# arielmission-space/PAOS

Hardware: AMD Instinct MI355X
Metric: wavefronts/sec (4096^2 c128, 20-surface chain) + achieved HBM GB/s (higher is better)
Workload: dtype c128 (f64); 1 GPU; SYN20 20-surface chain (SURVEY 8d: 43 2-D FFTs per wavefront as the reference runs it), 4096x4096 fp64, walked 512-wavelength sweep, 32 wavefronts/GPU/step, PSFs stay in HBM; separable pass programs + ptp identities ([24] passes/wavefront, parity 1e-15..2e-14 vs oracle); grid=4096, batch_per_gpu=32, parallelism=wavefront-sharded x1, transport=none (single process), ranks_seen=1, launcher=none

## Files before the change

include/paos_hip.h:

```cpp
#ifndef PAOS_HIP_H
#define PAOS_HIP_H

#ifdef __cplusplus
extern "C" {
#endif

typedef struct paos_ctx paos_ctx;

enum { PAOS_OK = 0, PAOS_EINVAL = 1, PAOS_EHIP = 2, PAOS_EUNSUPPORTED = 3 };
enum { PAOS_F64 = 0, PAOS_F32 = 1 };
enum { PAOS_SHAPE_ELLIPSE = 0, PAOS_SHAPE_RECT = 1 };
enum { PAOS_KERNEL_PASS_ROWS = 0, PAOS_KERNEL_PASS_COLS = 1, PAOS_KERNEL_PASS_ANY = 2 };
enum { PAOS_PW_SIGN = 1, PAOS_PW_QPHASE_CENTRED = 2, PAOS_PW_QPHASE_NATURAL = 3, PAOS_PW_SCALE = 4,
       PAOS_PW_MASK = 5 };
enum { PAOS_PWF_MUL2PI = 1,
       PAOS_PWF_X_ONLY = 2, PAOS_PWF_Y_ONLY = 4 };
enum { PAOS_MAX_PW = 6 };
enum { PAOS_NORM_SLOTS = 64 };
enum { PAOS_WHAT_FIELD = 0, PAOS_WHAT_AMPLITUDE = 1, PAOS_WHAT_PHASE = 2, PAOS_WHAT_INTENSITY = 3 };

enum { PAOS_PHASE_STRIDE = 5 };
enum { PAOS_APERTURE_STRIDE = 8 };
enum { PAOS_ZERNIKE_HEAD = 8 };

typedef struct { int kind, flags, block; } paos_pw_op;
typedef struct {
  int axis;
  int fft1, fft2;
  int n_pre, n_mid, n_post;
  paos_pw_op pre[PAOS_MAX_PW], mid[PAOS_MAX_PW], post[PAOS_MAX_PW];
} paos_pass;

typedef struct {
  const double* live_rows;
  int rows_stale;
  int final_intensity;
  int* power_ticket;
  const double* live_cols;
} paos_program_opts;

int paos_ctx_create(int device, int n, int batch, int precision, paos_ctx** out);
int paos_ctx_destroy(paos_ctx* ctx);
const char* paos_last_error(const paos_ctx* ctx);
int paos_sync(paos_ctx* ctx);
const char* paos_build_info(void);
const char* paos_source_hash(void);
void* paos_stream(paos_ctx* ctx);

int paos_profile_begin(paos_ctx* ctx, int kernel_kind, int max_launches);
int paos_profile_end(paos_ctx* ctx, int* launches, double* total_ms);
int paos_profile_end_split(paos_ctx* ctx, int* launches, double* total_ms, int* pruned_launches, double* pruned_ms);
int paos_profile_end_launches(paos_ctx* ctx, int capacity, double* ms_out, int* tag_out, int* count);
int paos_profile_planned_bytes(paos_ctx* ctx, int capacity, double* bytes_out, int* count);
int paos_profile_line_transforms(paos_ctx* ctx, int capacity, double* lines_out, int* count);

int paos_fill(paos_ctx* ctx, double re, double im);
int paos_start(paos_ctx* ctx, double re, double im, int shape, const double* aperture, const double* stop);
int paos_start_rows(paos_ctx* ctx, double re, double im, int shape, const double* aperture, const double* stop,
                    const double* write_rows);
int paos_zero_outside_rows(paos_ctx* ctx, const double* live_rows);
int paos_start_box(paos_ctx* ctx, double re, double im, int shape, const double* aperture, const double* stop,
                   const double* write_rows, const double* write_cols);
int paos_start_zernike_box(paos_ctx* ctx, double re, double im, int shape, const double* aperture, const double* stop,
                           const double* write_rows, const double* write_cols, int nmax, int kdim, const double* table,
                           const double* params, int param_stride, int* power_ticket);
int paos_zero_outside_box(paos_ctx* ctx, const double* live_rows, const double* live_cols);
int paos_import(paos_ctx* ctx, int item, const void* host_c128);
int paos_export(paos_ctx* ctx, int item, int what, void* host_out);

int paos_psf_keep(paos_ctx* ctx);
int paos_psf_keep_power(paos_ctx* ctx, int* ticket);
int paos_psf_fetch(paos_ctx* ctx, int item, double* host_out);
int paos_host_alloc(unsigned long long bytes, void** out);
int paos_host_free(void* p);
int paos_export_pinned(paos_ctx* ctx, int item, int what, void* pinned_out);

int paos_aperture(paos_ctx* ctx, int shape, const double* params);
int paos_aperture_render(paos_ctx* ctx, int shape, const double* params1, double* host_mask);
int paos_make_stop(paos_ctx* ctx, const double* enable);
int paos_stop_scale_last_power(paos_ctx* ctx, const double* enable);
int paos_stop_defer_last_power(paos_ctx* ctx, const double* enable);
int paos_norm2(paos_ctx* ctx, double* host_out);
int paos_norm2_enqueue(paos_ctx* ctx, int* ticket);
int paos_norm2_enqueue_rows(paos_ctx* ctx, const double* live_rows, int* ticket);
int paos_norm2_enqueue_rows_like(paos_ctx* ctx, const double* live_rows, const double* same_as, int* ticket);
int paos_norm2_enqueue_box(paos_ctx* ctx, const double* live_rows, const double* live_cols, const double* same_as, int* ticket);
int paos_norm2_fetch(paos_ctx* ctx, int ticket, double* host_out);
int paos_norm2_release(paos_ctx* ctx, int ticket);
int paos_psf_metrics(paos_ctx* ctx, int nr, const double* radii_px, double cx_px, double cy_px,
                     double* host_out);
int paos_phase(paos_ctx* ctx, const double* params, int mul2pi);
int paos_phase_map(paos_ctx* ctx, int item, const double* host_wfe, double wl);
int paos_phase_map_items(paos_ctx* ctx, const double* host_wfe, unsigned long long key, int n_items, const double* items,
                         const double* wl);
int paos_psd_screen(paos_ctx* ctx, const double* host_noise, const double* host_rough, const double* params,
                    unsigned long long key, double* host_out);
int paos_ptp(paos_ctx* ctx, const double* params);
int paos_stw(paos_ctx* ctx, const double* params, int inverse);
int paos_wts(paos_ctx* ctx, const double* params, int inverse);
int paos_focus_begin(paos_ctx* ctx);
int paos_focus_plane(paos_ctx* ctx, const double* params);
int paos_focus_end(paos_ctx* ctx);
enum { PAOS_OTF_MTF = 0, PAOS_OTF_COMPLEX = 1 };
int paos_otf_compute(paos_ctx* ctx);
int paos_otf_fetch(paos_ctx* ctx, int item, int what, void* host_out);
int paos_otf_cuts(paos_ctx* ctx, double* host_out);
int paos_blur_table(int n, double d, double sigma, double pixel, double* t);
enum { PAOS_BLUR_ITEM = 6 };
int paos_blur_apply(paos_ctx* ctx, const double* per_item);
enum { PAOS_EE_GIVEN = 0, PAOS_EE_CENTROID = 1, PAOS_EE_PEAK = 2 };
enum { PAOS_EE_ITEM = 4 };
enum { PAOS_EE_SUMMARY = 9 };
int paos_ee_compute(paos_ctx* ctx, int bins, int square, int centre_mode, const double* per_item);
int paos_ee_fetch(paos_ctx* ctx, double* summary, double* curves);
int paos_zoom_weights(int n, int s, double frac, double* w, int* carry);
enum { PAOS_ZOOM_PSF = 0, PAOS_ZOOM_FIELD = 1 };
int paos_zoom_compute(paos_ctx* ctx, int m, int s, const double* centres, int want_field);
int paos_zoom_tiles(int n, int batch, int m, int* pt_y, int* pt_x);
int paos_zoom_fetch(paos_ctx* ctx, int item, int what, void* host_out);
int paos_run_passes(paos_ctx* ctx, const paos_pass* passes, int n_passes, const double* blocks,
                    int n_blocks);
int paos_copy_yardstick(paos_ctx* ctx, int reps, double* ms_per_launch, double* bytes_per_launch);
int paos_record_set_stats(paos_ctx* ctx, unsigned long long* found, unsigned long long* rendered);
int paos_central_half_stats(paos_ctx* ctx, unsigned long long* central, unsigned long long* plain);
int paos_frugal_built(int precision, int n, const int* record);
int paos_pass_builds(paos_ctx* ctx, int* records, int capacity, int* count);
int paos_deferred_stop_stats(paos_ctx* ctx, unsigned long long* rode, unsigned long long* settled);
int paos_ctx_set_pruning(paos_ctx* ctx, int on);
int paos_run_passes_live(paos_ctx* ctx, const paos_pass* passes, int n_passes, const double* blocks,
                         int n_blocks, const double* live_rows);
int paos_run_program(paos_ctx* ctx, const paos_pass* passes, int n_passes, const double* blocks, int n_blocks,
                     const paos_program_opts* opts);
int paos_zernike(paos_ctx* ctx, int nmax, int kdim, const double* table, const double* params,
                 int param_stride, double* host_wfe);
int paos_zernike_like(paos_ctx* ctx, int nmax, int kdim, const double* table, const double* params,
                      int param_stride, const double* same_as, double* host_wfe);


int paos_pupil_aperture(paos_ctx* ctx, int shape, const double* params);
int paos_pupil_upload(paos_ctx* ctx, int item, const double* host_weights);
int paos_zernike_gram(paos_ctx* ctx, int nmax, int kdim, const double* table, const double* params,
                      int param_stride, int K, const double* poly, int use_pupil, double* host_out);
int paos_zernike_pupil(paos_ctx* ctx, int nmax, int kdim, const double* table, const double* params,
                       int param_stride, double* host_wfe);

enum { PAOS_WF_UNIFORM = 0, PAOS_WF_INTENSITY = 1 };
enum { PAOS_WF_SUMMARY = 10 };
int paos_wavefront_fit(paos_ctx* ctx, int nmax, int kdim, const double* table, const double* params, int param_stride,
                       int K, const double* poly, int weight_mode, int use_pupil, const double* min_intensity);
int paos_wavefront_fetch(paos_ctx* ctx, double* summary, double* sums);

enum { PAOS_DETECTOR_GEOM = 6 };
enum { PAOS_DETECTOR_ITEM = 3 };
enum { PAOS_DETECTOR_SCRATCH_MIB = 512 };
int paos_detector_begin(paos_ctx* ctx, const double* geom);
int paos_detector_add(paos_ctx* ctx, const double* per_item);
int paos_detector_images(paos_ctx* ctx, const double* per_item, double* host_out);
int paos_detector_fetch(paos_ctx* ctx, double* host_out);
enum { PAOS_DETECTOR_PLACED_ITEM = 5 };
int paos_detector_add_placed(paos_ctx* ctx, const double* per_item);
int paos_detector_images_placed(paos_ctx* ctx, const double* per_item, double* host_out);

#ifdef __cplusplus
}
#endif
#endif
```

paos_amd/_lib.py:

```python
import ctypes
import os
import threading
import weakref

import numpy as np

_HERE = os.path.dirname(os.path.abspath(__file__))
LIB_PATH = os.environ.get("PAOS_LIB") or os.path.join(_HERE, "libpaoship.so")

PAOS_F64, PAOS_F32 = 0, 1
SHAPE_ELLIPSE, SHAPE_RECT = 0, 1
WHAT_FIELD, WHAT_AMPLITUDE, WHAT_PHASE, WHAT_INTENSITY = 0, 1, 2, 3
KERNEL_PASS_ROWS, KERNEL_PASS_COLS, KERNEL_PASS_ANY = 0, 1, 2
PW_SIGN, PW_QPHASE_CENTRED, PW_QPHASE_NATURAL, PW_SCALE, PW_MASK = 1, 2, 3, 4, 5
PWF_MUL2PI = 1
PWF_X_ONLY, PWF_Y_ONLY = 2, 4
MAX_PW = 6
OTF_MTF, OTF_COMPLEX = 0, 1
EE_GIVEN, EE_CENTROID, EE_PEAK = 0, 1, 2
EE_ITEM, EE_SUMMARY, EE_MAX_BINS = 4, 9, 1024
WF_UNIFORM, WF_INTENSITY = 0, 1
WF_SUMMARY, WF_MAX_TERMS = 10, 63
ZOOM_PSF, ZOOM_FIELD = 0, 1
ZOOM_MAX_TABLES = 256
NORM_SLOTS = 64


class PwOp(ctypes.Structure):
    _fields_ = [("kind", ctypes.c_int), ("flags", ctypes.c_int), ("block", ctypes.c_int)]


class ProgramOpts(ctypes.Structure):
    _fields_ = [("live_rows", ctypes.POINTER(ctypes.c_double)), ("rows_stale", ctypes.c_int),
                ("final_intensity", ctypes.c_int), ("power_ticket", ctypes.POINTER(ctypes.c_int)),
                ("live_cols", ctypes.POINTER(ctypes.c_double))]


class Pass(ctypes.Structure):
    _fields_ = [("axis", ctypes.c_int), ("fft1", ctypes.c_int), ("fft2", ctypes.c_int),
                ("n_pre", ctypes.c_int), ("n_mid", ctypes.c_int), ("n_post", ctypes.c_int),
                ("pre", PwOp * MAX_PW), ("mid", PwOp * MAX_PW), ("post", PwOp * MAX_PW)]

PHASE_STRIDE = 5
APERTURE_STRIDE = 8
ZERNIKE_HEAD = 8

_c_ctx = ctypes.c_void_p
_dbl_p = ctypes.POINTER(ctypes.c_double)
SYMBOLS = {
    "paos_ctx_create": (ctypes.c_int, [ctypes.c_int, ctypes.c_int, ctypes.c_int, ctypes.c_int, ctypes.POINTER(_c_ctx)]),
    "paos_ctx_destroy": (ctypes.c_int, [_c_ctx]),
    "paos_last_error": (ctypes.c_char_p, [_c_ctx]),
    "paos_sync": (ctypes.c_int, [_c_ctx]),
    "paos_build_info": (ctypes.c_char_p, []),
    "paos_stream": (ctypes.c_void_p, [_c_ctx]),
    "paos_profile_begin": (ctypes.c_int, [_c_ctx, ctypes.c_int, ctypes.c_int]),
    "paos_profile_end": (ctypes.c_int, [_c_ctx, ctypes.POINTER(ctypes.c_int), _dbl_p]),
    "paos_profile_end_split": (ctypes.c_int, [_c_ctx, ctypes.POINTER(ctypes.c_int), _dbl_p, ctypes.POINTER(ctypes.c_int), _dbl_p]),
    "paos_source_hash": (ctypes.c_char_p, []),
    "paos_profile_planned_bytes": (ctypes.c_int, [_c_ctx, ctypes.c_int, _dbl_p, ctypes.POINTER(ctypes.c_int)]),
    "paos_profile_line_transforms": (ctypes.c_int, [_c_ctx, ctypes.c_int, _dbl_p, ctypes.POINTER(ctypes.c_int)]),
    "paos_profile_end_launches": (ctypes.c_int, [_c_ctx, ctypes.c_int, _dbl_p, ctypes.POINTER(ctypes.c_int),
                                                 ctypes.POINTER(ctypes.c_int)]),
    "paos_fill": (ctypes.c_int, [_c_ctx, ctypes.c_double, ctypes.c_double]),
    "paos_import": (ctypes.c_int, [_c_ctx, ctypes.c_int, ctypes.c_void_p]),
    "paos_export": (ctypes.c_int, [_c_ctx, ctypes.c_int, ctypes.c_int, ctypes.c_void_p]),
    "paos_aperture": (ctypes.c_int, [_c_ctx, ctypes.c_int, _dbl_p]),
    "paos_aperture_render": (ctypes.c_int, [_c_ctx, ctypes.c_int, _dbl_p, _dbl_p]),
    "paos_make_stop": (ctypes.c_int, [_c_ctx, _dbl_p]),
    "paos_stop_scale_last_power": (ctypes.c_int, [_c_ctx, _dbl_p]),
    "paos_stop_defer_last_power": (ctypes.c_int, [_c_ctx, _dbl_p]),
    "paos_norm2": (ctypes.c_int, [_c_ctx, _dbl_p]),
    "paos_norm2_enqueue": (ctypes.c_int, [_c_ctx, ctypes.POINTER(ctypes.c_int)]),
    "paos_norm2_fetch": (ctypes.c_int, [_c_ctx, ctypes.c_int, _dbl_p]),
    "paos_norm2_release": (ctypes.c_int, [_c_ctx, ctypes.c_int]),
    "paos_psf_metrics": (ctypes.c_int, [_c_ctx, ctypes.c_int, _dbl_p, ctypes.c_double, ctypes.c_double, _dbl_p]),
    "paos_phase": (ctypes.c_int, [_c_ctx, _dbl_p, ctypes.c_int]),
    "paos_phase_map": (ctypes.c_int, [_c_ctx, ctypes.c_int, _dbl_p, ctypes.c_double]),
    "paos_ptp": (ctypes.c_int, [_c_ctx, _dbl_p]),
    "paos_stw": (ctypes.c_int, [_c_ctx, _dbl_p, ctypes.c_int]),
    "paos_wts": (ctypes.c_int, [_c_ctx, _dbl_p, ctypes.c_int]),
    "paos_focus_begin": (ctypes.c_int, [_c_ctx]),
    "paos_focus_plane": (ctypes.c_int, [_c_ctx, _dbl_p]),
    "paos_focus_end": (ctypes.c_int, [_c_ctx]),
    "paos_otf_compute": (ctypes.c_int, [_c_ctx]),
    "paos_otf_fetch": (ctypes.c_int, [_c_ctx, ctypes.c_int, ctypes.c_int, ctypes.c_void_p]),
    "paos_otf_cuts": (ctypes.c_int, [_c_ctx, _dbl_p]),
    "paos_blur_table": (ctypes.c_int, [ctypes.c_int, ctypes.c_double, ctypes.c_double, ctypes.c_double, _dbl_p]),
    "paos_blur_apply": (ctypes.c_int, [_c_ctx, _dbl_p]),
    "paos_ee_compute": (ctypes.c_int, [_c_ctx, ctypes.c_int, ctypes.c_int, ctypes.c_int, _dbl_p]),
    "paos_ee_fetch": (ctypes.c_int, [_c_ctx, _dbl_p, _dbl_p]),
    "paos_wavefront_fit": (ctypes.c_int, [_c_ctx, ctypes.c_int, ctypes.c_int, _dbl_p, _dbl_p, ctypes.c_int, ctypes.c_int, _dbl_p,
                                          ctypes.c_int, ctypes.c_int, _dbl_p]),
    "paos_wavefront_fetch": (ctypes.c_int, [_c_ctx, _dbl_p, _dbl_p]),
    "paos_zoom_weights": (ctypes.c_int, [ctypes.c_int, ctypes.c_int, ctypes.c_double, _dbl_p, ctypes.POINTER(ctypes.c_int)]),
    "paos_zoom_compute": (ctypes.c_int, [_c_ctx, ctypes.c_int, ctypes.c_int, _dbl_p, ctypes.c_int]),
    "paos_zoom_fetch": (ctypes.c_int, [_c_ctx, ctypes.c_int, ctypes.c_int, ctypes.c_void_p]),
    "paos_zoom_tiles": (ctypes.c_int, [ctypes.c_int, ctypes.c_int, ctypes.c_int, ctypes.POINTER(ctypes.c_int),
                                       ctypes.POINTER(ctypes.c_int)]),
    "paos_run_passes": (ctypes.c_int, [_c_ctx, ctypes.POINTER(Pass), ctypes.c_int, _dbl_p, ctypes.c_int]),
    "paos_copy_yardstick": (ctypes.c_int, [_c_ctx, ctypes.c_int, _dbl_p, _dbl_p]),
    "paos_record_set_stats": (ctypes.c_int, [_c_ctx, ctypes.POINTER(ctypes.c_ulonglong), ctypes.POINTER(ctypes.c_ulonglong)]),
    "paos_central_half_stats": (ctypes.c_int, [_c_ctx, ctypes.POINTER(ctypes.c_ulonglong), ctypes.POINTER(ctypes.c_ulonglong)]),
    "paos_frugal_built": (ctypes.c_int, [ctypes.c_int, ctypes.c_int, ctypes.POINTER(ctypes.c_int)]),
    "paos_pass_builds": (ctypes.c_int, [_c_ctx, ctypes.POINTER(ctypes.c_int), ctypes.c_int, ctypes.POINTER(ctypes.c_int)]),
    "paos_deferred_stop_stats": (ctypes.c_int, [_c_ctx, ctypes.POINTER(ctypes.c_ulonglong), ctypes.POINTER(ctypes.c_ulonglong)]),
    "paos_ctx_set_pruning": (ctypes.c_int, [_c_ctx, ctypes.c_int]),
    "paos_run_passes_live": (ctypes.c_int, [_c_ctx, ctypes.POINTER(Pass), ctypes.c_int, _dbl_p, ctypes.c_int, _dbl_p]),
    "paos_zernike": (ctypes.c_int, [_c_ctx, ctypes.c_int, ctypes.c_int, _dbl_p, _dbl_p, ctypes.c_int, _dbl_p]),
    "paos_psf_keep": (ctypes.c_int, [_c_ctx]),
    "paos_psf_keep_power": (ctypes.c_int, [_c_ctx, ctypes.POINTER(ctypes.c_int)]),
    "paos_psf_fetch": (ctypes.c_int, [_c_ctx, ctypes.c_int, _dbl_p]),
    "paos_host_alloc": (ctypes.c_int, [ctypes.c_ulonglong, ctypes.POINTER(ctypes.c_void_p)]),
    "paos_host_free": (ctypes.c_int, [ctypes.c_void_p]),
    "paos_export_pinned": (ctypes.c_int, [_c_ctx, ctypes.c_int, ctypes.c_int, ctypes.c_void_p]),
    "paos_start": (ctypes.c_int, [_c_ctx, ctypes.c_double, ctypes.c_double, ctypes.c_int, _dbl_p, _dbl_p]),
    "paos_pupil_aperture": (ctypes.c_int, [_c_ctx, ctypes.c_int, _dbl_p]),
    "paos_pupil_upload": (ctypes.c_int, [_c_ctx, ctypes.c_int, _dbl_p]),
    "paos_zernike_like": (ctypes.c_int, [_c_ctx, ctypes.c_int, ctypes.c_int, _dbl_p, _dbl_p, ctypes.c_int, _dbl_p, _dbl_p]),
    "paos_zernike_gram": (ctypes.c_int, [_c_ctx, ctypes.c_int, ctypes.c_int, _dbl_p, _dbl_p, ctypes.c_int,
                                         ctypes.c_int, _dbl_p, ctypes.c_int, _dbl_p]),
    "paos_zernike_pupil": (ctypes.c_int, [_c_ctx, ctypes.c_int, ctypes.c_int, _dbl_p, _dbl_p, ctypes.c_int, _dbl_p]),
    "paos_start_rows": (ctypes.c_int, [_c_ctx, ctypes.c_double, ctypes.c_double, ctypes.c_int, _dbl_p, _dbl_p, _dbl_p]),
    "paos_zero_outside_rows": (ctypes.c_int, [_c_ctx, _dbl_p]),
    "paos_phase_map_items": (ctypes.c_int, [_c_ctx, _dbl_p, ctypes.c_ulonglong, ctypes.c_int, _dbl_p, _dbl_p]),
    "paos_psd_screen": (ctypes.c_int, [_c_ctx, _dbl_p, _dbl_p, _dbl_p, ctypes.c_ulonglong, _dbl_p]),
    "paos_start_box": (ctypes.c_int, [_c_ctx, ctypes.c_double, ctypes.c_double, ctypes.c_int, _dbl_p, _dbl_p, _dbl_p, _dbl_p]),
    "paos_start_zernike_box": (ctypes.c_int, [_c_ctx, ctypes.c_double, ctypes.c_double, ctypes.c_int, _dbl_p, _dbl_p, _dbl_p, _dbl_p,
                                              ctypes.c_int, ctypes.c_int, _dbl_p, _dbl_p, ctypes.c_int, ctypes.POINTER(ctypes.c_int)]),
    "paos_zero_outside_box": (ctypes.c_int, [_c_ctx, _dbl_p, _dbl_p]),
    "paos_norm2_enqueue_box": (ctypes.c_int, [_c_ctx, _dbl_p, _dbl_p, _dbl_p, ctypes.POINTER(ctypes.c_int)]),
    "paos_norm2_enqueue_rows": (ctypes.c_int, [_c_ctx, _dbl_p, ctypes.POINTER(ctypes.c_int)]),
    "paos_norm2_enqueue_rows_like": (ctypes.c_int, [_c_ctx, _dbl_p, _dbl_p, ctypes.POINTER(ctypes.c_int)]),
    "paos_run_program": (ctypes.c_int, [_c_ctx, ctypes.POINTER(Pass), ctypes.c_int, _dbl_p, ctypes.c_int,
                                        ctypes.POINTER(ProgramOpts)]),
    "paos_detector_begin": (ctypes.c_int, [_c_ctx, _dbl_p]),
    "paos_detector_add": (ctypes.c_int, [_c_ctx, _dbl_p]),
    "paos_detector_images": (ctypes.c_int, [_c_ctx, _dbl_p, _dbl_p]),
    "paos_detector_fetch": (ctypes.c_int, [_c_ctx, _dbl_p]),
    "paos_detector_add_placed": (ctypes.c_int, [_c_ctx, _dbl_p]),
    "paos_detector_images_placed": (ctypes.c_int, [_c_ctx, _dbl_p, _dbl_p]),
}

_lib = None


class PaosHipError(RuntimeError):
    pass


def load():
    global _lib
    if _lib is not None:
        return _lib
    if not os.path.exists(LIB_PATH):
        raise PaosHipError(
            f"{LIB_PATH} not found: build it with `make` or "
            "`python -c 'import __graft_entry__ as g; g.build()'` (there is no CPU fallback)"
        )
    lib = ctypes.CDLL(LIB_PATH)
    if os.environ.get("PAOS_LIB"):
        import sys

        print(f"paos_amd: using the library variant {LIB_PATH} (PAOS_LIB)", file=sys.stderr)
    for name, (res, args) in SYMBOLS.items():
        fn = getattr(lib, name)
        fn.restype = res
        fn.argtypes = args
    _lib = lib
    return lib


def _dptr(arr):
    return arr.ctypes.data_as(_dbl_p)


def as_blocks(blocks, batch, stride):
    arr = np.ascontiguousarray(blocks, dtype=np.float64)
    if arr.shape != (batch, stride):
        raise ValueError(f"expected parameter blocks of shape {(batch, stride)}, got {arr.shape}")
    return arr


BUILD_FIELDS = ("axis", "kpre", "kmid", "nfft", "store", "tab", "fuse", "one_line", "central")


def frugal_built(precision, n, record):
    if len(record) != len(BUILD_FIELDS):
        raise ValueError("a build record has nine fields")
    rec = (ctypes.c_int * 9)(*[int(v) for v in record])
    code = {"fp64": PAOS_F64, "fp32": PAOS_F32}.get(precision, -1)
    rc = load().paos_frugal_built(code, int(n), rec)
    if rc < 0:
        raise ValueError(f"no family of pass-kernel builds for {precision} at n = {n}")
    return bool(rc)


def zoom_check(size, oversample, n):
    if isinstance(size, bool) or not isinstance(size, (int, np.integer)) or size < 16 or size > 1024 or size % 16:
        raise ValueError(f"a zoomed window's size must be an integer multiple of 16 in 16 .. 1024, got {size!r}")
    if isinstance(oversample, bool) or not isinstance(oversample, (int, np.integer)) or not 1 <= oversample <= 64:
        raise ValueError(f"a zoomed window's oversampling must be an integer in 1 .. 64, got {oversample!r}")
    if size > oversample * n:
        raise ValueError(f"a zoomed window of {size} samples at oversampling {oversample} is wider than the {n}-pixel grid")


def zoom_tiles(n, batch, size):
    pty, ptx = ctypes.c_int(0), ctypes.c_int(0)
    if load().paos_zoom_tiles(int(n), int(batch), int(size), ctypes.byref(pty), ctypes.byref(ptx)) != 0:
        raise ValueError(f"paos_zoom_tiles refused n={n!r}, batch={batch!r}, size={size!r}")
    return pty.value, ptx.value


def blur_table(n, d, sigma, pixel=0.0):
    if isinstance(n, bool) or not isinstance(n, (int, np.integer)) or n < 2:
        raise ValueError(f"paos_blur_table refused n={n!r}")
    out = np.empty(int(n) // 2 + 1, dtype=np.float64)
    if load().paos_blur_table(int(n), float(d), float(sigma), float(pixel), _dptr(out)) != 0:
        raise ValueError(f"paos_blur_table refused n={n!r}, d={d!r}, sigma={sigma!r}, pixel={pixel!r}")
    return out


def zoom_centres(centres, batch, n):
    try:
        ctr = np.ascontiguousarray(centres, dtype=np.float64)
    except (TypeError, ValueError):
        raise ValueError("zoomed-window centres must be a (batch, 2) array of pixel positions (x, y)") from None
    if ctr.shape != (batch, 2):
        raise ValueError(f"zoomed-window centres must have shape ({batch}, 2), got {ctr.shape}")
    if not np.all(np.isfinite(ctr)) or np.any(ctr < 0.0) or np.any(ctr >= n):
        raise ValueError(f"zoomed-window centres must be finite and lie in [0, {n})")
    if np.unique(ctr - np.floor(ctr)).size > ZOOM_MAX_TABLES:
        raise ValueError(f"the centres of one call may have at most {ZOOM_MAX_TABLES} distinct fractional parts")
    return ctr


PINNED_MIN_BYTES = 4 << 20
PINNED_MAX_BYTES = 32 << 20
PINNED_LIVE_BYTES = int(os.environ.get("PAOS_PINNED_BYTES", 8 << 30))
PINNED_POOL_BYTES = 2 << 30
_pin_lock = threading.Lock()
_pin_free = {}
_pin_live = 0
_pin_pooled = 0


def _pin_release(address, nbytes):
    global _pin_live, _pin_pooled
    with _pin_lock:
        _pin_live -= nbytes
        if _pin_pooled + nbytes <= PINNED_POOL_BYTES:
            _pin_free.setdefault(nbytes, []).append(address)
            _pin_pooled += nbytes
            return
    try:
        load().paos_host_free(ctypes.c_void_p(address))
    except Exception:
        pass


def pinned_empty(shape, dtype):
    global _pin_live, _pin_pooled
    nbytes = int(np.prod(shape)) * np.dtype(dtype).itemsize
    if nbytes <= PINNED_MIN_BYTES:
        return None
    address = None
    with _pin_lock:
        if _pin_live + nbytes > PINNED_LIVE_BYTES:
            return None
        stack = _pin_free.get(nbytes)
        if stack:
            address = stack.pop()
            _pin_pooled -= nbytes
        elif nbytes > PINNED_MAX_BYTES:
            return None
        _pin_live += nbytes
    if address is None:
        ptr = ctypes.c_void_p()
        if load().paos_host_alloc(nbytes, ctypes.byref(ptr)) != 0 or not ptr.value:
            with _pin_lock:
                _pin_live -= nbytes
            return None
        address = ptr.value
    buf = (ctypes.c_char * nbytes).from_address(address)
    weakref.finalize(buf, _pin_release, address, nbytes)
    return np.frombuffer(buf, dtype=dtype).reshape(shape)


def release_pinned_pool():
    global _pin_pooled
    with _pin_lock:
        items = [(a, n) for n, lst in _pin_free.items() for a in lst]
        _pin_free.clear()
        _pin_pooled = 0
    for address, _ in items:
        load().paos_host_free(ctypes.c_void_p(address))


_HIP_TOUCHED = [False]


def hip_initialised():
    return _HIP_TOUCHED[0]


class DeviceFields:

    def __init__(self, n, batch=1, precision="fp64", device=0):
        self._lib = load()
        _HIP_TOUCHED[0] = True
        self._ctx = _c_ctx()
        self.detector = None
        self.n, self.batch = int(n), int(batch)
        if precision not in ("fp64", "fp32"):
            raise ValueError("precision must be 'fp64' or 'fp32'")
        self.precision = precision
        rc = self._lib.paos_ctx_create(int(device), self.n, self.batch,
                                       PAOS_F64 if precision == "fp64" else PAOS_F32,
                                       ctypes.byref(self._ctx))
        if rc != 0:
            msg = self._lib.paos_last_error(None).decode()
            self._ctx = _c_ctx()
            raise PaosHipError(f"paos_ctx_create failed ({rc}): {msg}")

    def _check(self, rc, what):
        if rc != 0:
            raise PaosHipError(f"{what} failed ({rc}): {self._lib.paos_last_error(self._ctx).decode()}")

    def close(self):
        if getattr(self, "_ctx", None) and self._ctx.value:
            self._lib.paos_ctx_destroy(self._ctx)
            self._ctx = _c_ctx()

    def __del__(self):
        try:
            self.close()
        except Exception:
            pass

    def sync(self):
        self._check(self._lib.paos_sync(self._ctx), "paos_sync")

    @property
    def stream(self):
        return self._lib.paos_stream(self._ctx)

    def build_info(self):
        return self._lib.paos_build_info().decode()

    def profile_begin(self, kernel_kind, max_launches=4096):
        self._check(self._lib.paos_profile_begin(self._ctx, int(kernel_kind), int(max_launches)),
                    "paos_profile_begin")

    def profile_end(self):
        n, ms = ctypes.c_int(0), ctypes.c_double(0.0)
        self._check(self._lib.paos_profile_end(self._ctx, ctypes.byref(n), ctypes.byref(ms)),
                    "paos_profile_end")
        return n.value, ms.value

    def profile_end_split(self):
        n, ms, pn, pms = ctypes.c_int(0), ctypes.c_double(0.0), ctypes.c_int(0), ctypes.c_double(0.0)
        self._check(self._lib.paos_profile_end_split(self._ctx, ctypes.byref(n), ctypes.byref(ms), ctypes.byref(pn),
                                                     ctypes.byref(pms)), "paos_profile_end_split")
        return n.value, ms.value, pn.value, pms.value

    def profile_planned_bytes(self, capacity=1 << 16):
        out = np.empty(capacity, dtype=np.float64)
        n = ctypes.c_int(0)
        self._check(self._lib.paos_profile_planned_bytes(self._ctx, int(capacity), _dptr(out), ctypes.byref(n)),
                    "paos_profile_planned_bytes")
        return out[:n.value].copy()

    def profile_line_transforms(self, capacity=1 << 16):
        out = np.empty(capacity, dtype=np.float64)
        n = ctypes.c_int(0)
        self._check(self._lib.paos_profile_line_transforms(self._ctx, int(capacity), _dptr(out), ctypes.byref(n)),
                    "paos_profile_line_transforms")
        return out[:n.value].copy()

    def profile_end_launches(self, capacity=1 << 16):
        ms = np.empty(capacity, dtype=np.float64)
        tags = np.empty(capacity, dtype=np.int32)
        n = ctypes.c_int(0)
        self._check(self._lib.paos_profile_end_launches(self._ctx, int(capacity), _dptr(ms),
                                                        tags.ctypes.data_as(ctypes.POINTER(ctypes.c_int)), ctypes.byref(n)),
                    "paos_profile_end_launches")
        return ms[:n.value].copy(), tags[:n.value].copy()

    def fill(self, value=1.0 + 0.0j):
        value = complex(value)
        self._check(self._lib.paos_fill(self._ctx, value.real, value.imag), "paos_fill")

    def upload(self, item, field):
        arr = np.ascontiguousarray(field, dtype=np.complex128)
        if arr.shape != (self.n, self.n):
            raise ValueError(f"field must have shape {(self.n, self.n)}")
        self._check(self._lib.paos_import(self._ctx, int(item), arr.ctypes.data_as(ctypes.c_void_p)),
                    "paos_import")

    def download(self, item=0, what=WHAT_FIELD):
        dtype = np.complex128 if what == WHAT_FIELD else np.float64
        out = pinned_empty((self.n, self.n), dtype)
        if out is not None:
            self._check(self._lib.paos_export_pinned(self._ctx, int(item), int(what),
                                                     out.ctypes.data_as(ctypes.c_void_p)), "paos_export_pinned")
            return out
# ... 457 lines not shown
```

paos_amd/csrc/context.hip:

```cpp
#include "host.h"

#include <cmath>
#include <complex>
#include <cstdio>
#include <cstring>
#include <mutex>
#include <set>
#include <utility>

namespace {

thread_local std::string g_err;

}

int fail(paos_ctx* c, int code, const std::string& msg) {
  if (c) c->err = msg;
  g_err = msg;
  return code;
}

namespace {

bool dump_arena() {
  static const bool dump = env_is("PAOS_DUMP_PASSES", '1');
  return dump;
}

int arena_commit(paos_ctx* c) {
  Arena& a = c->arena;
  size_t first = 0, count = 0;
  if (!a.lay.take(&first, &count)) return PAOS_OK;
  const size_t at = (size_t)a.cur * a.lay.cap + first;
  HIPCHK(c, hipMemcpyAsync(a.dev + at, a.host + at, count * sizeof(double), hipMemcpyHostToDevice, c->stream));
  return PAOS_OK;
}

int arena_switch(paos_ctx* c) {
  Arena& a = c->arena;
  if (int rc = arena_commit(c)) return rc;
  if (a.left >= 0) {
    HIPCHK(c, hipEventRecord(a.fence[a.left], c->stream));
    a.fenced[a.left] = true;
  }
  a.left = a.cur;
  const int next = (a.cur + 1) % kArenaSlabs;
  if (a.used[next]) {
    if (a.fenced[next]) HIPCHK(c, hipEventSynchronize(a.fence[next]));
    else HIPCHK(c, hipStreamSynchronize(c->stream));
  }
  a.fenced[next] = false;
  a.used[next] = true;
  a.cur = next;
  a.lay.rewind();
  if (dump_arena()) std::fprintf(stderr, "arena switch to slab %d\n", next);
  return PAOS_OK;
}

}

int launch_failed(paos_ctx* c, const char* call, hipError_t e, const char* file, int line) {
  return fail(c, PAOS_EHIP, std::string(call) + ": " + hipGetErrorString(e) + " (" + file + ":" + std::to_string(line) + ")");
}

int arena_reserve(paos_ctx* c, size_t total) {
  Arena& a = c->arena;
  switch (a.lay.room(total)) {
    case ARENA_FITS: return PAOS_OK;
    case ARENA_SWITCH: return arena_switch(c);
    case ARENA_GROW: break;
  }
  if (int rc = arena_commit(c)) return rc;
  HIPCHK(c, hipStreamSynchronize(c->stream));
  const size_t cap = a.lay.grown(total);
  double *h = nullptr, *d = nullptr;
  HIPCHK(c, hipHostMalloc(&h, kArenaSlabs * cap * sizeof(double)));
  if (hipMalloc(&d, kArenaSlabs * cap * sizeof(double)) != hipSuccess) {
    (void)hipHostFree(h);
    return fail(c, PAOS_EHIP, "hipMalloc(arena growth)");
  }
  (void)hipHostFree(a.host);
  (void)hipFree(a.dev);
  if (dump_arena()) std::fprintf(stderr, "arena grow to %zu doubles per slab\n", cap);
  a.host = h; a.dev = d; a.lay.cap = cap; a.lay.rewind(); a.cur = 0; a.left = -1;
  for (int k = 0; k < kArenaSlabs; ++k) a.fenced[k] = a.used[k] = false;
  a.used[0] = true;
  return PAOS_OK;
}

int ArenaBatch::begin(size_t total) {
  if (st_.closed || st_.reserved) return fail(c_, PAOS_EINVAL, "a parameter batch is begun once, before its first block");
  const int rc = arena_reserve(c_, total);
  if (rc == PAOS_OK) st_.reserved = true;
  return rc;
}

int ArenaBatch::add(const double* src, size_t count, const double** dev) {
  Arena& a = c_->arena;
  if (!st_.may_add()) return fail(c_, PAOS_EINVAL, "parameter block added to a batch that has been committed");
  if (count > a.lay.cap) return fail(c_, PAOS_EINVAL, "parameter block larger than the arena");
  if (!a.lay.fits(count)) {
    if (!st_.may_switch()) return fail(c_, PAOS_EINVAL, "a parameter batch outgrew the room it reserved");
    if (int rc = arena_switch(c_)) return rc;
  }
  const size_t at = (size_t)a.cur * a.lay.cap + a.lay.place(count);
  std::memcpy(a.host + at, src, count * sizeof(double));
  *dev = a.dev + at;
  return PAOS_OK;
}

int ArenaBatch::commit() {
  st_.closed = true;
  return arena_commit(c_);
}

int arena_push(paos_ctx* c, const double* src, size_t count, const double** dev) {
  ArenaBatch one(c);
  if (int rc = one.add(src, count, dev)) return rc;
  return one.commit();
}

int arena_settled(paos_ctx* c, int rc) {
  if (!c) return rc;
  const bool pending = c->arena.lay.pending();
  c->arena.lay.drop();
  if (rc == PAOS_OK && pending)
    return fail(c, PAOS_EHIP, "parameter blocks were added but never copied to the device: the call's launches read stale parameters");
  return rc;
}

constexpr size_t kBounceBytes = size_t(4) << 20;
int copy_to_host(paos_ctx* c, void* host, const void* dev, size_t bytes) {
  if (bytes > kBounceBytes) {
    HIPCHK(c, hipMemcpyAsync(host, dev, bytes, hipMemcpyDeviceToHost, c->stream));
    HIPCHK(c, hipStreamSynchronize(c->stream));
    return PAOS_OK;
  }
  for (int i = 0; i < 2; ++i)
    if (!c->bounce[i]) {
      HIPCHK(c, hipHostMalloc(&c->bounce[i], kBounceBytes));
      HIPCHK(c, hipEventCreateWithFlags(&c->bounce_ev[i], hipEventDisableTiming));
    }
  const size_t chunks = (bytes + kBounceBytes - 1) / kBounceBytes;
  auto len = [&](size_t k) { return k + 1 < chunks ? kBounceBytes : bytes - k * kBounceBytes; };
  for (size_t k = 0; k <= chunks; ++k) {
    if (k < chunks) {
      HIPCHK(c, hipMemcpyAsync(c->bounce[k & 1], (const char*)dev + k * kBounceBytes, len(k), hipMemcpyDeviceToHost, c->stream));
      HIPCHK(c, hipEventRecord(c->bounce_ev[k & 1], c->stream));
    }
    if (k > 0) {
      HIPCHK(c, hipEventSynchronize(c->bounce_ev[(k - 1) & 1]));
      std::memcpy((char*)host + (k - 1) * kBounceBytes, c->bounce[(k - 1) & 1], len(k - 1));
    }
  }
  HIPCHK(c, hipStreamSynchronize(c->stream));
  return PAOS_OK;
}

bool timed_launch_begin(paos_ctx* c, int kind) {
  const bool timed = (c->prof_kind == kind || c->prof_kind == PAOS_KERNEL_PASS_ANY) && (c->prof_used + 2 <= c->prof_events.size());
  return timed && hipEventRecord(c->prof_events[c->prof_used], c->stream) == hipSuccess;
}
hipError_t timed_launch_end(paos_ctx* c, int tag) {
  const hipError_t e = hipEventRecord(c->prof_events[c->prof_used + 1], c->stream);
  if (e != hipSuccess) return e;
  c->prof_tags.resize(c->prof_used / 2, 0);
  c->prof_tags.push_back(tag);
  c->prof_bytes.resize(c->prof_tags.size() - 1, 0.0);
  c->prof_bytes.push_back(c->prof_next_bytes);
  c->prof_lines.resize(c->prof_tags.size() - 1, 0.0);
  c->prof_lines.push_back(c->prof_next_lines);
  c->prof_used += 2;
  return hipSuccess;
}

int next_norm_slot(paos_ctx* c) {
  for (int k = 0; k < kNormSlots; ++k) {
    const int slot = (c->norm_slot + k) % kNormSlots;
    if (!c->norm_busy[slot]) { c->norm_slot = slot; return slot; }
  }
  return c->norm_slot;
}

int opt_in_lds(paos_ctx* c, const void* kern, size_t lds) {
  static std::mutex mu;
  static std::set<std::pair<int, const void*>> configured;
  std::lock_guard<std::mutex> lock(mu);
  const std::pair<int, const void*> key(c->device, kern);
  if (configured.count(key)) return PAOS_OK;
  HIPCHK(c, hipFuncSetAttribute(kern, hipFuncAttributeMaxDynamicSharedMemorySize, (int)lds));
  configured.insert(key);
  return PAOS_OK;
}

int check_mask_overflow(paos_ctx* c) {
  if (!c->mask_overflow) return PAOS_OK;
  int n = 0;
  HIPCHK(c, hipMemcpy(&n, c->mask_overflow, sizeof(int), hipMemcpyDeviceToHost));
  if (n != 0) {
    (void)hipMemset(c->mask_overflow, 0, sizeof(int));
    for (auto& ms : c->mask_sets) ms.key.clear();
    return fail(c, PAOS_EUNSUPPORTED, "aperture line records overflowed (partial run longer than kMaskW): results are invalid");
  }
  return PAOS_OK;
}

int check_rows(paos_ctx* c, const double* rows) {
  for (int i = 0; i < c->batch; ++i)
    if (!(rows[2 * i] >= 0.0) || !(rows[2 * i + 1] <= (double)c->n) || !(rows[2 * i] <= rows[2 * i + 1]))
      return fail(c, PAOS_EINVAL, "row range must satisfy 0 <= lo <= hi <= n");
  return PAOS_OK;
}

std::vector<double> rounded_cols(const paos_ctx* c, const double* cols) {
  std::vector<double> out((size_t)2 * c->batch);
  for (int i = 0; i < c->batch; ++i) {
    int l = (int)cols[2 * i], h = (int)cols[2 * i + 1];
    l = l < 0 ? 0 : (l / c->br) * c->br;
    h = ((h + c->br - 1) / c->br) * c->br;
    if (h > c->n) h = c->n;
    out[2 * i] = l; out[2 * i + 1] = h;
  }
  return out;
}

namespace {

template <typename T>
std::vector<std::complex<T>> twiddles(int n) {
  std::vector<std::complex<T>> tw(n);
  const long double two_pi = 6.283185307179586476925286766559005768L;
  for (int m = 0; m < n; ++m) {
    const long double a = two_pi * (long double)m / (long double)n;
    tw[m] = std::complex<T>((T)cosl(a), (T)-sinl(a));
  }
  return tw;
}


int profile_end(paos_ctx* c, int* launches, double* total_ms, int* pruned_launches, double* pruned_ms) {
  if (c) (void)hipSetDevice(c->device);
  if (!c || !launches || !total_ms) return fail(c, PAOS_EINVAL, "null argument");
  HIPCHK(c, hipStreamSynchronize(c->stream));
  double sum = 0.0, psum = 0.0;
  int pcount = 0;
  for (size_t i = 0; i + 1 < c->prof_used; i += 2) {
    float ms = 0.f;
    HIPCHK(c, hipEventElapsedTime(&ms, c->prof_events[i], c->prof_events[i + 1]));
    sum += ms;
    if (i / 2 < c->prof_tags.size() && c->prof_tags[i / 2]) { psum += ms; ++pcount; }
  }
  *launches = (int)(c->prof_used / 2);
  *total_ms = sum;
  if (pruned_launches) *pruned_launches = pcount;
  if (pruned_ms) *pruned_ms = psum;
  c->prof_kind = -1;
  c->prof_used = 0;
  return PAOS_OK;
}

}

extern "C" {

const char* paos_last_error(const paos_ctx* ctx) { return ctx ? ctx->err.c_str() : g_err.c_str(); }

const char* paos_build_info(void) {
  static const std::string info = std::string("libpaoship gfx950 layout=") + std::to_string(BR) + "(c64 at N>=2048: " + std::to_string(PAOS_F32_BR) + ")x(" +
                                  std::to_string(Lay<double>::BC) + "|" + std::to_string(Lay<float>::BC) +
                                  ") pad_blocks=" + std::to_string(PAOS_PAD_BLOCKS);
  return info.c_str();
}

void* paos_stream(paos_ctx* ctx) { return ctx ? (void*)ctx->stream : nullptr; }

int paos_ctx_create(int device, int n, int batch, int precision, paos_ctx** out) {
  if (!out) return fail(nullptr, PAOS_EINVAL, "out is null");
  *out = nullptr;
  if (n < 64 || n > 4096 || (n & (n - 1))) return fail(nullptr, PAOS_EUNSUPPORTED, "grid size must be a power of two in 64..4096");
  if (batch < 1) return fail(nullptr, PAOS_EINVAL, "batch must be >= 1");
  if (precision != PAOS_F64 && precision != PAOS_F32) return fail(nullptr, PAOS_EINVAL, "precision must be PAOS_F64 or PAOS_F32");
  int ndev = 0;
  if (hipGetDeviceCount(&ndev) != hipSuccess || ndev == 0)
    return fail(nullptr, PAOS_EHIP, "no HIP device available: libpaoship has no CPU fallback");
  if (device < 0 || device >= ndev) return fail(nullptr, PAOS_EINVAL, "device index out of range");
  paos_ctx* c = new paos_ctx();
  c->device = device; c->n = n; c->batch = batch; c->precision = precision;
  const int bc = precision == PAOS_F64 ? Lay<double>::BC : Lay<float>::BC;
  c->br = (precision == PAOS_F32 && n >= 2048) ? PAOS_F32_BR : PAOS_BR;
  c->pitch = (unsigned)n * c->br + (unsigned)PAOS_PAD_BLOCKS * c->br * bc;
  c->item_stride = c->pitch * (unsigned)(n / c->br);
  const size_t eb = elem_bytes(c);
  auto bail = [&](hipError_t e, const char* what) {
    std::string msg = std::string(what) + ": " + hipGetErrorString(e);
    paos_ctx_destroy(c);
    return fail(nullptr, PAOS_EHIP, msg);
  };
  hipError_t e;
  if ((e = hipSetDevice(device)) != hipSuccess) return bail(e, "hipSetDevice");
  if ((e = hipStreamCreateWithFlags(&c->stream, hipStreamNonBlocking)) != hipSuccess) return bail(e, "hipStreamCreate");
  if (const char* pad = getenv("PAOS_LDS_PAD")) c->lds_pad = (size_t)std::max(0, std::atoi(pad));
  if (env_is("PAOS_CENTRAL_HALF", '0')) c->central_half = false;
  if (env_is("PAOS_CENTRAL_HALF", '1')) c->central_half = true;
  if ((e = hipMalloc(&c->dyn_scale, (size_t)batch * sizeof(double))) != hipSuccess) return bail(e, "hipMalloc(dyn_scale)");
  {
    std::vector<double> ones((size_t)batch, 1.0);
    if ((e = hipMemcpy(c->dyn_scale, ones.data(), ones.size() * sizeof(double), hipMemcpyHostToDevice)) != hipSuccess) return bail(e, "hipMemcpy(dyn_scale)");
  }
  if ((e = hipMalloc(&c->field, (size_t)c->item_stride * batch * eb)) != hipSuccess) return bail(e, "hipMalloc(field)");
  if ((e = hipMemsetAsync(c->field, 0, (size_t)c->item_stride * batch * eb, c->stream)) != hipSuccess) return bail(e, "hipMemset(field)");
  if ((e = hipMalloc(&c->tw, (size_t)n * eb)) != hipSuccess) return bail(e, "hipMalloc(tw)");
  if ((e = hipMalloc(&c->staging, (size_t)n * n * 16)) != hipSuccess) return bail(e, "hipMalloc(staging)");
  c->nparts = 1024;
  if ((e = hipMalloc(&c->partial, (size_t)batch * c->nparts * sizeof(double))) != hipSuccess) return bail(e, "hipMalloc(partial)");
  if ((e = hipMalloc(&c->norm2, (size_t)batch * sizeof(double))) != hipSuccess) return bail(e, "hipMalloc(norm2)");
  if ((e = hipHostMalloc(&c->norm2_host, (size_t)kNormSlots * batch * sizeof(double))) != hipSuccess) return bail(e, "hipHostMalloc(norm2)");
  c->arena.lay.cap = (size_t)1 << 18;
  if (c->arena.lay.cap < (size_t)batch * 2048) c->arena.lay.cap = (size_t)batch * 2048;
  if (const char* cap = getenv("PAOS_ARENA_DOUBLES")) c->arena.lay.cap = arena_rounded((size_t)std::max(1LL, std::atoll(cap)));
  if ((e = hipHostMalloc(&c->arena.host, kArenaSlabs * c->arena.lay.cap * sizeof(double))) != hipSuccess) return bail(e, "hipHostMalloc(arena)");
  if ((e = hipMalloc(&c->arena.dev, kArenaSlabs * c->arena.lay.cap * sizeof(double))) != hipSuccess) return bail(e, "hipMalloc(arena)");
  for (int k = 0; k < kArenaSlabs; ++k)
    if ((e = hipEventCreateWithFlags(&c->arena.fence[k], hipEventDisableTiming)) != hipSuccess) return bail(e, "hipEventCreate(arena fence)");
  c->arena.used[0] = true;
  e = dispatch_layout(c, [&](auto t, auto) {
    auto tw = twiddles<decltype(t)>(n);
    return hipMemcpy(c->tw, tw.data(), (size_t)n * eb, hipMemcpyHostToDevice);
  });
  if (e != hipSuccess) return bail(e, "hipMemcpy(tw)");
  *out = c;
  return PAOS_OK;
}

int paos_profile_begin(paos_ctx* c, int kernel_kind, int max_launches) {
  if (c) (void)hipSetDevice(c->device);
  if (!c || max_launches < 0) return fail(c, PAOS_EINVAL, "bad profile request");
  HIPCHK(c, hipStreamSynchronize(c->stream));
  while (c->prof_events.size() < (size_t)2 * max_launches) {
    hipEvent_t e;
    HIPCHK(c, hipEventCreate(&e));
    c->prof_events.push_back(e);
  }
  c->prof_kind = kernel_kind;
  c->prof_used = 0;
  c->prof_tags.clear();
  c->prof_bytes.clear();
  c->prof_lines.clear();
  return PAOS_OK;
}

int paos_profile_end_launches(paos_ctx* c, int capacity, double* ms_out, int* tag_out, int* count) {
  if (c) (void)hipSetDevice(c->device);
  if (!c || !ms_out || !tag_out || !count || capacity < 0) return fail(c, PAOS_EINVAL, "null argument");
  HIPCHK(c, hipStreamSynchronize(c->stream));
  const int n = (int)(c->prof_used / 2);
  if (n > capacity) return fail(c, PAOS_EINVAL, "more launches were timed than the caller's arrays hold");
  for (int i = 0; i < n; ++i) {
    float ms = 0.f;
    HIPCHK(c, hipEventElapsedTime(&ms, c->prof_events[2 * i], c->prof_events[2 * i + 1]));
    ms_out[i] = ms;
    tag_out[i] = (size_t)i < c->prof_tags.size() ? c->prof_tags[i] : 0;
  }
  *count = n;
  c->prof_kind = -1;
  c->prof_used = 0;
  return PAOS_OK;
}

int paos_profile_planned_bytes(paos_ctx* c, int capacity, double* bytes_out, int* count) {
  if (!c || !bytes_out || !count || capacity < 0) return fail(c, PAOS_EINVAL, "null argument");
  const int n = (int)(c->prof_used / 2);
  if (n > capacity) return fail(c, PAOS_EINVAL, "more launches were timed than the caller's array holds");
  for (int i = 0; i < n; ++i) bytes_out[i] = (size_t)i < c->prof_bytes.size() ? c->prof_bytes[i] : 0.0;
  *count = n;
  return PAOS_OK;
}

int paos_profile_line_transforms(paos_ctx* c, int capacity, double* lines_out, int* count) {
  if (!c || !lines_out || !count || capacity < 0) return fail(c, PAOS_EINVAL, "bad profile request");
  const int n = (int)(c->prof_used / 2);
  if (n > capacity) return fail(c, PAOS_EINVAL, "profile buffer too small");
  for (int i = 0; i < n; ++i) lines_out[i] = (size_t)i < c->prof_lines.size() ? c->prof_lines[i] : 0.0;
  *count = n;
  return PAOS_OK;
}

int paos_profile_end(paos_ctx* c, int* launches, double* total_ms) {
  return profile_end(c, launches, total_ms, nullptr, nullptr);
}

int paos_profile_end_split(paos_ctx* c, int* launches, double* total_ms, int* pruned_launches, double* pruned_ms) {
  if (!pruned_launches || !pruned_ms) return fail(c, PAOS_EINVAL, "null argument");
  return profile_end(c, launches, total_ms, pruned_launches, pruned_ms);
}

int paos_ctx_destroy(paos_ctx* c) {
  if (!c) return PAOS_OK;
  (void)hipSetDevice(c->device);
  if (c->stream) (void)hipStreamSynchronize(c->stream);
  for (hipEvent_t e : c->prof_events) (void)hipEventDestroy(e);
  if (c->field) (void)hipFree(c->field);
  if (c->tw) (void)hipFree(c->tw);
  if (c->staging) (void)hipFree(c->staging);
  if (c->tables) (void)hipFree(c->tables);
  if (c->mask) (void)hipFree(c->mask);
  if (c->metric_partial) (void)hipFree(c->metric_partial);
  if (c->metric_out) (void)hipFree(c->metric_out);
  if (c->metric_host) (void)hipHostFree(c->metric_host);
  for (auto& ms : c->mask_sets) {
    if (ms.lines) (void)hipFree(ms.lines);
    if (ms.vals) (void)hipFree(ms.vals);
  }
  if (c->mask_overflow) (void)hipFree(c->mask_overflow);
  if (c->partial) (void)hipFree(c->partial);
  if (c->norm2) (void)hipFree(c->norm2);
  if (c->norm2_host) (void)hipHostFree(c->norm2_host);
  if (c->psf) (void)hipFree(c->psf);
  if (c->focus_spec) (void)hipFree(c->focus_spec);
  if (c->otf_spec) (void)hipFree(c->otf_spec);
  if (c->otf_cuts) (void)hipFree(c->otf_cuts);
  if (c->zoom_t) (void)hipFree(c->zoom_t);
  if (c->zoom_psf) (void)hipFree(c->zoom_psf);
  if (c->zoom_field) (void)hipFree(c->zoom_field);
  if (c->zoom_tabs) (void)hipFree(c->zoom_tabs);
  if (c->map_dev) (void)hipFree(c->map_dev);
  if (c->psd_scratch) (void)hipFree(c->psd_scratch);
  if (c->start_norm2) (void)hipFree(c->start_norm2);
  if (c->start_partial) (void)hipFree(c->start_partial);
  if (c->psd_bad) (void)hipFree(c->psd_bad);
  if (c->pow_partial) (void)hipFree(c->pow_partial);
  if (c->dyn_scale) (void)hipFree(c->dyn_scale);
  if (c->ptab) (void)hipFree(c->ptab);
  if (c->psf_partial) (void)hipFree(c->psf_partial);
  if (c->det_img) (void)hipFree(c->det_img);
  if (c->det_rows) (void)hipFree(c->det_rows);
  if (c->det_out) (void)hipFree(c->det_out);
  if (c->ee_buf) (void)hipFree(c->ee_buf);
  if (c->wf_buf) (void)hipFree(c->wf_buf);
  for (int i = 0; i < 2; ++i) {
    if (c->bounce[i]) (void)hipHostFree(c->bounce[i]);
    if (c->bounce_ev[i]) (void)hipEventDestroy(c->bounce_ev[i]);
  }
  if (c->arena.host) (void)hipHostFree(c->arena.host);
  if (c->arena.dev) (void)hipFree(c->arena.dev);
  for (int k = 0; k < kArenaSlabs; ++k)
    if (c->arena.fence[k]) (void)hipEventDestroy(c->arena.fence[k]);
  if (c->stream) (void)hipStreamDestroy(c->stream);
  delete c;
  return PAOS_OK;
}

int paos_sync(paos_ctx* c) {
  if (c) (void)hipSetDevice(c->device);
  if (!c) return fail(c, PAOS_EINVAL, "null context");
  HIPCHK(c, hipStreamSynchronize(c->stream));
  return check_mask_overflow(c);
}

int paos_host_alloc(unsigned long long bytes, void** out) {
  if (!out || bytes == 0) return fail(nullptr, PAOS_EINVAL, "null argument");
  *out = nullptr;
  const hipError_t e = hipHostMalloc(out, (size_t)bytes);
  if (e != hipSuccess) {
    *out = nullptr;
    return fail(nullptr, PAOS_EHIP, std::string("hipHostMalloc: ") + hipGetErrorString(e));
  }
  return PAOS_OK;
}

int paos_host_free(void* p) {
  if (!p) return PAOS_OK;
  const hipError_t e = hipHostFree(p);
  if (e != hipSuccess) return fail(nullptr, PAOS_EHIP, std::string("hipHostFree: ") + hipGetErrorString(e));
  return PAOS_OK;
}

int paos_norm2_fetch(paos_ctx* c, int ticket, double* host_out) {
  if (c) (void)hipSetDevice(c->device);
  if (!c || !host_out || ticket < 0 || ticket >= kNormSlots) return fail(c, PAOS_EINVAL, "bad ticket");
  if (!c->norm_busy[ticket]) return fail(c, PAOS_EINVAL, "ticket is not outstanding (already fetched, or never issued)");
  HIPCHK(c, hipStreamSynchronize(c->stream));
  c->norm_busy[ticket] = false;
  std::memcpy(host_out, c->norm2_host + (size_t)ticket * c->batch, (size_t)c->batch * sizeof(double));
  return check_mask_overflow(c);
}

int paos_norm2_release(paos_ctx* c, int ticket) {
  if (!c || ticket < 0 || ticket >= kNormSlots) return fail(c, PAOS_EINVAL, "bad ticket");
  c->norm_busy[ticket] = false;
  return PAOS_OK;
}

int paos_record_set_stats(paos_ctx* c, unsigned long long* found, unsigned long long* rendered) {
  if (!c || !found || !rendered) return fail(c, PAOS_EINVAL, "bad record-set request");
  *found = c->mask_hits;
  *rendered = c->mask_rendered;
  return PAOS_OK;
}

int paos_central_half_stats(paos_ctx* c, unsigned long long* central, unsigned long long* plain) {
  if (!c || !central || !plain) return fail(c, PAOS_EINVAL, "bad central-half request");
  *central = c->central_launches;
  *plain = c->plain_launches;
  return PAOS_OK;
}

int paos_deferred_stop_stats(paos_ctx* c, unsigned long long* rode, unsigned long long* settled) {
  if (!c || !rode || !settled) return fail(c, PAOS_EINVAL, "bad deferred-stop request");
  *rode = c->deferred_rode;
  *settled = c->deferred_settled;
  return PAOS_OK;
}

int paos_ctx_set_pruning(paos_ctx* c, int on) {
  if (!c) return fail(c, PAOS_EINVAL, "null context");
  c->prune = on != 0;
  return PAOS_OK;
}

}
```

paos_amd/csrc/fft_core.h:

```cpp
#pragma once
#include <hip/hip_runtime.h>

namespace paos {

template <typename T>
struct cx {
  T x, y;
};

template <typename T>
__device__ __forceinline__ cx<T> cadd(cx<T> a, cx<T> b) { return {a.x + b.x, a.y + b.y}; }
template <typename T>
__device__ __forceinline__ cx<T> csub(cx<T> a, cx<T> b) { return {a.x - b.x, a.y - b.y}; }
template <typename T>
__device__ __forceinline__ cx<T> cmul(cx<T> a, cx<T> b) {
  return {fma(a.x, b.x, -(a.y * b.y)), fma(a.x, b.y, a.y * b.x)};
}
template <typename T>
__device__ __forceinline__ cx<T> cconj(cx<T> a) { return {a.x, -a.y}; }
template <typename T>
__device__ __forceinline__ cx<T> sub_ib(cx<T> a, cx<T> b) { return {a.x + b.y, a.y - b.x}; }
template <typename T>
__device__ __forceinline__ cx<T> add_ib(cx<T> a, cx<T> b) { return {a.x - b.y, a.y + b.x}; }
template <typename T>
__device__ __forceinline__ cx<T> fma_real(T c, cx<T> b, cx<T> a) { return {fma(c, b.x, a.x), fma(c, b.y, a.y)}; }
template <typename T>
__device__ __forceinline__ cx<T> rot_tau(cx<T> b, T tau) { return {fma(-tau, b.y, b.x), fma(tau, b.x, b.y)}; }
template <typename T>
__device__ __forceinline__ cx<T> fma_mic(T c, cx<T> b, cx<T> a) { return {fma(c, b.y, a.x), fma(-c, b.x, a.y)}; }
template <typename T>
__device__ __forceinline__ cx<T> fma_pic(T c, cx<T> b, cx<T> a) { return {fma(-c, b.y, a.x), fma(c, b.x, a.y)}; }
template <typename T>
__device__ __forceinline__ cx<T> cmul_const(cx<T> v, T c, T s) { return {fma(v.x, c, -(v.y * s)), fma(v.x, s, v.y * c)}; }
template <typename T>
__device__ __forceinline__ cx<T> scale2(cx<T> v, T p, T q) { return {v.x * p, v.y * q}; }

typedef float f2 __attribute__((ext_vector_type(2)));
__device__ __forceinline__ f2 pk(cx<float> a) { return f2{a.x, a.y}; }
__device__ __forceinline__ cx<float> unpk(f2 v) { return {v.x, v.y}; }
__device__ __forceinline__ cx<float> cadd(cx<float> a, cx<float> b) { return unpk(pk(a) + pk(b)); }
__device__ __forceinline__ cx<float> csub(cx<float> a, cx<float> b) { return unpk(pk(a) - pk(b)); }
__device__ __forceinline__ cx<float> cmul(cx<float> a, cx<float> b) {
  f2 t, r;
  const f2 av = pk(a), bv = pk(b);
  asm("v_pk_mul_f32 %0, %1, %2 op_sel_hi:[0,1]" : "=v"(t) : "v"(av), "v"(bv));
  asm("v_pk_fma_f32 %0, %1, %2, %3 op_sel:[1,1,0] op_sel_hi:[1,0,1] neg_lo:[1,0,0]"
      : "=v"(r) : "v"(av), "v"(bv), "v"(t));
  return unpk(r);
}
__device__ __forceinline__ cx<float> cmul_after_trans(cx<float> a, cx<float> b) {
  f2 t, r;
  const f2 av = pk(a), bv = pk(b);
  asm("s_nop 0\n\tv_pk_mul_f32 %0, %1, %2 op_sel_hi:[0,1]" : "=v"(t) : "v"(av), "v"(bv));
  asm("v_pk_fma_f32 %0, %1, %2, %3 op_sel:[1,1,0] op_sel_hi:[1,0,1] neg_lo:[1,0,0]" : "=v"(r) : "v"(av), "v"(bv), "v"(t));
  return unpk(r);
}
__device__ __forceinline__ cx<float> sub_ib(cx<float> a, cx<float> b) {
  f2 r;
  asm("v_pk_add_f32 %0, %1, %2 op_sel:[0,1] op_sel_hi:[1,0] neg_hi:[0,1]" : "=v"(r) : "v"(pk(a)), "v"(pk(b)));
  return unpk(r);
}
__device__ __forceinline__ cx<float> add_ib(cx<float> a, cx<float> b) {
  f2 r;
  asm("v_pk_add_f32 %0, %1, %2 op_sel:[0,1] op_sel_hi:[1,0] neg_lo:[0,1]" : "=v"(r) : "v"(pk(a)), "v"(pk(b)));
  return unpk(r);
}
__device__ __forceinline__ cx<float> fma_real(float c, cx<float> b, cx<float> a) {
  return unpk(__builtin_elementwise_fma(f2{c, c}, pk(b), pk(a)));
}
__device__ __forceinline__ cx<float> rot_tau(cx<float> b, float tau) {
  const f2 bv = pk(b);
  return unpk(__builtin_elementwise_fma(bv.yx, f2{-tau, tau}, bv));
}
__device__ __forceinline__ cx<float> fma_mic(float c, cx<float> b, cx<float> a) {
  return unpk(__builtin_elementwise_fma(pk(b).yx, f2{c, -c}, pk(a)));
}
__device__ __forceinline__ cx<float> fma_pic(float c, cx<float> b, cx<float> a) {
  return unpk(__builtin_elementwise_fma(pk(b).yx, f2{-c, c}, pk(a)));
}
__device__ __forceinline__ cx<float> cmul_const(cx<float> v, float c, float s) {
  const f2 vv = pk(v);
  return unpk(__builtin_elementwise_fma(vv.yy, f2{-s, c}, vv.xx * f2{c, s}));
}
__device__ __forceinline__ cx<float> scale2(cx<float> v, float p, float q) { return unpk(pk(v) * f2{p, q}); }

__device__ __forceinline__ void sincos_fast(double a, double* sn, double* cs) {
  const double kMagic = 6755399441055744.0;
  const double nb = fma(a, 0.63661977236758134308, kMagic);
  const unsigned q = (unsigned)__double2loint(nb);
  const double n = nb - kMagic;
  double r = fma(-n, 1.57079632673412561417e+00, a);
  r = fma(-n, 6.07710050630396597660e-11, r);
  r = fma(-n, 2.02226624879595063154e-21, r);
  const double z = r * r;
  double ps = fma(z, 1.58969099521155010221e-10, -2.50507602534068634195e-08);
  ps = fma(z, ps, 2.75573137070700676789e-06);
  ps = fma(z, ps, -1.98412698298579493134e-04);
  ps = fma(z, ps, 8.33333333332248946124e-03);
  ps = fma(z, ps, -1.66666666666666324348e-01);
  const double s = fma(r * z, ps, r);
  double pc = fma(z, -1.13596475577881948265e-11, 2.08757232129817482790e-09);
  pc = fma(z, pc, -2.75573143513906633035e-07);
  pc = fma(z, pc, 2.48015872894767294178e-05);
  pc = fma(z, pc, -1.38888888888741095749e-03);
  pc = fma(z, pc, 4.16666666666666019037e-02);
  const double c = fma(z * z, pc, fma(z, -0.5, 1.0));
  const bool odd = (q & 1u) != 0;
  const double s1 = odd ? c : s;
  const double c1 = odd ? s : c;
  const int sflip = (int)((q & 2u) << 30), cflip = (int)(((q + 1u) & 2u) << 30);
  *sn = __hiloint2double(__double2hiint(s1) ^ sflip, __double2loint(s1));
  *cs = __hiloint2double(__double2hiint(c1) ^ cflip, __double2loint(c1));
}

__device__ constexpr double kCos32[9] = {
    1.0,
    0.98078528040323044913,
    0.92387953251128675613,
    0.83146961230254523708,
    0.70710678118654752440,
    0.55557023301960222474,
    0.38268343236508977173,
    0.19509032201612826785,
    0.0};

__host__ __device__ constexpr double cos32(int m) {
  m &= 31;
  if (m > 16) m = 32 - m;
  return (m > 8) ? -kCos32[16 - m] : kCos32[m];
}
__host__ __device__ constexpr double sin32(int m) { return cos32(m - 8); }

template <int R, int DIR, typename T>
__device__ __forceinline__ cx<T> mulw(cx<T> v, int m) {
  const int m32 = (m * (32 / R)) & 31;
  if (m32 == 0) return v;
  if (m32 == 16) return {-v.x, -v.y};
  if (m32 == 8) return (DIR > 0) ? cx<T>{v.y, -v.x} : cx<T>{-v.y, v.x};
  if (m32 == 24) return (DIR > 0) ? cx<T>{-v.y, v.x} : cx<T>{v.y, -v.x};
  const T c = (T)cos32(m32);
  const T s = (T)((DIR > 0) ? -sin32(m32) : sin32(m32));
  return cmul_const(v, c, s);
}

template <int M16, int DIR>
struct W16 {
  static constexpr int m32 = (M16 * 2) & 31;
  static constexpr bool quarter = m32 == 8 || m32 == 24;
  static constexpr bool times_minus_i = (m32 == 8) == (DIR > 0);
  static constexpr double c = cos32(m32);
  static constexpr double s = (DIR > 0) ? -sin32(m32) : sin32(m32);
  static constexpr double tau = quarter ? 0.0 : s / c;
};
template <typename T>
__device__ __forceinline__ cx<T> lf_u(cx<T> b, double tau) { return rot_tau(b, (T)tau); }
template <int K1, int DIR, typename T>
__device__ __forceinline__ void lf_twiddled_dft4(const cx<T>* b, cx<T>* out) {
  using W1 = W16<K1, DIR>;
  using W2 = W16<2 * K1, DIR>;
  using W3 = W16<3 * K1, DIR>;
  static_assert(!W1::quarter && !W3::quarter, "K1 and 3 K1 are never multiples of 4 here");
  cx<T> t0, t1;
  if constexpr (W2::quarter) {
    const cx<T> wb = W2::times_minus_i ? cx<T>{b[2].y, -b[2].x} : cx<T>{-b[2].y, b[2].x};
    t0 = cadd(b[0], wb);
    t1 = csub(b[0], wb);
  } else {
    const cx<T> u2 = lf_u(b[2], W2::tau);
    t0 = fma_real((T)W2::c, u2, b[0]);
    t1 = fma_real((T)-W2::c, u2, b[0]);
  }
  const cx<T> u1 = lf_u(b[1], W1::tau), u3 = lf_u(b[3], W3::tau);
  constexpr double rho = W3::c / W1::c;
  const cx<T> t2 = fma_real((T)rho, u3, u1);
  const cx<T> t3 = fma_real((T)-rho, u3, u1);
  constexpr T c1 = (T)W1::c;
  out[0] = fma_real(c1, t2, t0);
  out[2] = fma_real(-c1, t2, t0);
  if constexpr (DIR > 0) {
    out[1] = fma_mic(c1, t3, t1);
    out[3] = fma_pic(c1, t3, t1);
  } else {
    out[1] = fma_pic(c1, t3, t1);
    out[3] = fma_mic(c1, t3, t1);
  }
}

template <int R, int DIR, typename T>
__device__ __forceinline__ void dft(cx<T>* v);

template <int DIR, typename T>
__device__ __forceinline__ void dft16_lf(cx<T>* v) {
  cx<T> y[16];
#pragma unroll
  for (int n2 = 0; n2 < 4; ++n2) {
    cx<T> a[4] = {v[n2], v[4 + n2], v[8 + n2], v[12 + n2]};
    dft<4, DIR>(a);
#pragma unroll
    for (int k1 = 0; k1 < 4; ++k1) y[k1 * 4 + n2] = a[k1];
  }
  cx<T> o[4];
  {
    cx<T> b[4] = {y[0], y[1], y[2], y[3]};
    dft<4, DIR>(b);
#pragma unroll
    for (int k2 = 0; k2 < 4; ++k2) v[4 * k2] = b[k2];
  }
  lf_twiddled_dft4<1, DIR>(y + 4, o);
#pragma unroll
  for (int k2 = 0; k2 < 4; ++k2) v[1 + 4 * k2] = o[k2];
  lf_twiddled_dft4<2, DIR>(y + 8, o);
#pragma unroll
  for (int k2 = 0; k2 < 4; ++k2) v[2 + 4 * k2] = o[k2];
  lf_twiddled_dft4<3, DIR>(y + 12, o);
#pragma unroll
  for (int k2 = 0; k2 < 4; ++k2) v[3 + 4 * k2] = o[k2];
}

template <int DIR, typename T>
__device__ __forceinline__ void dft16_lf_central(cx<T>* v) {
  static_assert(DIR > 0, "the pass kernel runs forward transforms only");
  cx<T> y[16];
#pragma unroll
  for (int n2 = 0; n2 < 4; ++n2) {
    const cx<T> a = v[4 + n2], b = v[8 + n2];
    const cx<T> nb = {-b.x, -b.y};
    y[0 * 4 + n2] = cadd(b, a);
    y[1 * 4 + n2] = sub_ib(nb, a);
    y[2 * 4 + n2] = csub(b, a);
    y[3 * 4 + n2] = add_ib(nb, a);
  }
  cx<T> o[4];
  {
    cx<T> b[4] = {y[0], y[1], y[2], y[3]};
    dft<4, DIR>(b);
#pragma unroll
    for (int k2 = 0; k2 < 4; ++k2) v[4 * k2] = b[k2];
  }
  lf_twiddled_dft4<1, DIR>(y + 4, o);
#pragma unroll
  for (int k2 = 0; k2 < 4; ++k2) v[1 + 4 * k2] = o[k2];
  lf_twiddled_dft4<2, DIR>(y + 8, o);
#pragma unroll
  for (int k2 = 0; k2 < 4; ++k2) v[2 + 4 * k2] = o[k2];
  lf_twiddled_dft4<3, DIR>(y + 12, o);
#pragma unroll
  for (int k2 = 0; k2 < 4; ++k2) v[3 + 4 * k2] = o[k2];
}

template <int R, int DIR, typename T>
__device__ __forceinline__ void dft(cx<T>* v) {
  if constexpr (R == 16) {
    dft16_lf<DIR>(v);
  } else if constexpr (R == 2) {
    cx<T> a = v[0], b = v[1];
    v[0] = cadd(a, b);
    v[1] = csub(a, b);
  } else if constexpr (R == 4) {
    cx<T> t0 = cadd(v[0], v[2]), t1 = csub(v[0], v[2]);
    cx<T> t2 = cadd(v[1], v[3]), t3 = csub(v[1], v[3]);
    v[0] = cadd(t0, t2);
    v[2] = csub(t0, t2);
    if constexpr (DIR > 0) {
      v[1] = sub_ib(t1, t3);
      v[3] = add_ib(t1, t3);
    } else {
      v[1] = add_ib(t1, t3);
      v[3] = sub_ib(t1, t3);
    }
  } else if constexpr (R > 4) {
    constexpr int A = 4, B = R / 4;
    cx<T> y[R];
#pragma unroll
    for (int n2 = 0; n2 < B; ++n2) {
      cx<T> a[A];
#pragma unroll
      for (int n1 = 0; n1 < A; ++n1) a[n1] = v[B * n1 + n2];
      dft<A, DIR>(a);
#pragma unroll
      for (int k1 = 0; k1 < A; ++k1) y[k1 * B + n2] = mulw<R, DIR>(a[k1], n2 * k1);
    }
#pragma unroll
    for (int k1 = 0; k1 < A; ++k1) {
      cx<T> b[B];
#pragma unroll
      for (int n2 = 0; n2 < B; ++n2) b[n2] = y[k1 * B + n2];
      dft<B, DIR>(b);
#pragma unroll
      for (int k2 = 0; k2 < B; ++k2) v[k1 + A * k2] = b[k2];
    }
  }
}

__device__ __forceinline__ constexpr int lds_pad(int i) { return i + (i >> 4); }
template <int N>
constexpr int lds_line_slots() { return N + (N >> 4); }

template <int N, int E, int NS>
struct StageInfo {
  static constexpr int REM = N / NS;
  static constexpr int R = (REM >= E) ? E : REM;
  static constexpr int TPT = E / R;
  static constexpr bool LAST = (NS * R == N);
};

template <int N, int E, int NS = 1>
constexpr int last_radix() {
  if constexpr (StageInfo<N, E, NS>::LAST) return StageInfo<N, E, NS>::R;
  else return last_radix<N, E, NS * StageInfo<N, E, NS>::R>();
}

template <int N, int E>
__device__ __forceinline__ constexpr int outslot(int k) {
  constexpr int RL = last_radix<N, E>();
  constexpr int TPTL = E / RL;
  return (k / RL) + (k % RL) * TPTL;
}

template <int R, typename T>
__device__ __forceinline__ void apply_twiddle_powers(cx<T>* v, cx<T> w1) {
  v[1] = cmul(v[1], w1);
  if constexpr (R > 2) {
    const cx<T> w2 = cmul(w1, w1);
    const cx<T> w3 = cmul(w2, w1);
    v[2] = cmul(v[2], w2);
    v[3] = cmul(v[3], w3);
    if constexpr (R > 4) {
      const cx<T> w4 = cmul(w2, w2);
      cx<T> base = w4;
#pragma unroll
      for (int a = 1; a < R / 4; ++a) {
        v[4 * a] = cmul(v[4 * a], base);
        v[4 * a + 1] = cmul(v[4 * a + 1], cmul(base, w1));
        v[4 * a + 2] = cmul(v[4 * a + 2], cmul(base, w2));
        v[4 * a + 3] = cmul(v[4 * a + 3], cmul(base, w3));
        if (a + 1 < R / 4) base = cmul(base, w4);
      }
    }
  }
}

template <int R, typename T>
__device__ __forceinline__ void apply_twiddle_chain(cx<T>* v, cx<T> w1) {
  cx<T> w = w1;
#pragma unroll
  for (int r = 1; r < R; ++r) {
    v[r] = cmul(v[r], w);
    if (r + 1 < R) w = cmul(w, w1);
  }
}

#define PAOS_FENCE() do { if constexpr (FR != 0) __builtin_amdgcn_sched_barrier(0); } while (0)
template <typename T, int N, int E, int DIR, bool SPLIT, int NS = 1, int FR = 0, int CH = 0>
__device__ __forceinline__ void fft_stages(cx<T>* v, void* lds, int t,
                                           const cx<T>* __restrict__ tw, const cx<double>* circle = nullptr,
                                           const cx<T>* w1_last = nullptr) {
  using S = StageInfo<N, E, NS>;
  constexpr int TL = N / E;
  constexpr int R = S::R;
  constexpr int TPT = S::TPT;

#pragma unroll
  for (int s = 0; s < TPT; ++s) {
    if constexpr (NS > 1) {
      const int j = t + s * TL;
      const int k = j & (NS - 1);
      if constexpr (FR != 0 && sizeof(T) == 8 && NS * R == 256) {
        cx<double> wa = circle[k], wb = circle[2 * k];
#pragma unroll
        for (int r = 1; r < R; ++r) {
          const cx<double> w = wa;
          wa = wb;
          if (r + 2 < R) wb = circle[k * (r + 2)];
          v[s * R + r] = cmul(v[s * R + r], cx<T>{(T)w.x, (T)(DIR > 0 ? -w.y : w.y)});
          PAOS_FENCE();
        }
      } else {
        cx<T> w1 = (w1_last != nullptr && NS * R == N) ? w1_last[s] : tw[k * (N / (NS * R))];
        if constexpr (DIR < 0) w1.y = -w1.y;
        if constexpr (FR != 0) apply_twiddle_chain<R>(v + s * R, w1);
        else apply_twiddle_powers<R>(v + s * R, w1);
      }
      PAOS_FENCE();
    }
    if constexpr (CH != 0 && NS == 1) {
      static_assert(R == 16 && TPT == 1, "central-half first stage: one 16-point butterfly per thread");
      dft16_lf_central<DIR>(v);
    } else {
      dft<R, DIR>(v + s * R);
    }
    PAOS_FENCE();
  }

  if constexpr (!S::LAST) {
    using SN = StageInfo<N, E, NS * R>;
    constexpr int R2 = SN::R;
    constexpr int TPT2 = SN::TPT;
    constexpr bool LIN_R = (TL % 16 == 0) && ((N / R2) % 16 == 0);
    int wb[TPT];
#pragma unroll
    for (int s = 0; s < TPT; ++s) {
      const int j = t + s * TL;
      wb[s] = lds_pad((j / NS) * (NS * R) + (j & (NS - 1)));
    }
    const int rb = lds_pad(t);
    auto ridx = [&](int s, int r) -> int {
      const int off = s * TL + r * (N / R2);
      return LIN_R ? rb + lds_pad(off) : lds_pad(t + off);
    };
    if constexpr (!SPLIT) {
      cx<T>* l = reinterpret_cast<cx<T>*>(lds);
#pragma unroll
      for (int s = 0; s < TPT; ++s)
#pragma unroll
        for (int r = 0; r < R; ++r) l[wb[s] + lds_pad(r * NS)] = v[s * R + r];
      __syncthreads();
#pragma unroll
      for (int s = 0; s < TPT2; ++s)
#pragma unroll
        for (int r = 0; r < R2; ++r) v[s * R2 + r] = l[ridx(s, r)];
      if constexpr (!SN::LAST) __syncthreads();
    } else {
      T* l = reinterpret_cast<T*>(lds);
#pragma unroll
      for (int part = 0; part < 2; ++part) {
#pragma unroll
        for (int s = 0; s < TPT; ++s)
#pragma unroll
          for (int r = 0; r < R; ++r) l[wb[s] + lds_pad(r * NS)] = part ? v[s * R + r].y : v[s * R + r].x;
        __syncthreads();
#pragma unroll
        for (int s = 0; s < TPT2; ++s)
#pragma unroll
          for (int r = 0; r < R2; ++r) {
            const T val = l[ridx(s, r)];
            if (part) v[s * R2 + r].y = val; else v[s * R2 + r].x = val;
          }
        if (part == 0 || !SN::LAST) __syncthreads();
      }
    }
    PAOS_FENCE();
    fft_stages<T, N, E, DIR, SPLIT, NS * R, FR, 0>(v, lds, t, tw, circle, w1_last);
  }
}

template <int N, int E, typename T>
__device__ __forceinline__ void unpermute_slots(cx<T>* v) {
  cx<T> tmp[E];
#pragma unroll
  for (int k = 0; k < E; ++k) tmp[outslot<N, E>(k)] = v[k];
#pragma unroll
  for (int k = 0; k < E; ++k) v[k] = tmp[k];
}

template <int BR, int BC>
__device__ __host__ __forceinline__ constexpr size_t layout_index(int row, int col, size_t pitch) {
  return (size_t)(row / BR) * pitch + (size_t)(col / BC) * (BR * BC) + (row % BR) * BC + (col % BC);
}

}
```

paos_amd/csrc/frugal_d1024.hip:

```cpp
#include "frugal_launch.h"

template <>
int frugal_family<double, 1024>(paos_ctx* c, const FrugalBuild& b, const FrugalArgs& a) { return frugal_dispatch<double, 1024>(c, b, a); }
```

paos_amd/csrc/frugal_d2048.hip:

```cpp
#include "frugal_launch.h"

template <>
int frugal_family<double, 2048>(paos_ctx* c, const FrugalBuild& b, const FrugalArgs& a) { return frugal_dispatch<double, 2048>(c, b, a); }
```

paos_amd/csrc/frugal_d4096.hip:

```cpp
#include "frugal_launch.h"

template <>
int frugal_family<double, 4096>(paos_ctx* c, const FrugalBuild& b, const FrugalArgs& a) { return frugal_dispatch<double, 4096>(c, b, a); }
```

paos_amd/csrc/frugal_f2048.hip:

```cpp
#include "frugal_launch.h"

template <>
int frugal_family<float, 2048>(paos_ctx* c, const FrugalBuild& b, const FrugalArgs& a) { return frugal_dispatch<float, 2048>(c, b, a); }
```

paos_amd/csrc/frugal_f4096.hip:

```cpp
#include "frugal_launch.h"

template <>
int frugal_family<float, 4096>(paos_ctx* c, const FrugalBuild& b, const FrugalArgs& a) { return frugal_dispatch<float, 4096>(c, b, a); }
```

paos_amd/csrc/frugal_launch.h:

```cpp
#pragma once
#include "host.h"
#include "pass_records.h"


inline int frugal_not_built(paos_ctx* c, const FrugalBuild& b) {
  if (b.tab && b.fuse) {
    if (b.kpre != 1 || b.kmid != 1) return fail(c, PAOS_EINVAL, "no fused build of this pass shape");
    if (b.nfft < 2) return fail(c, PAOS_EINVAL, "a fused chain starts with a two-transform pass");
    if (b.fuse > 4) return fail(c, PAOS_EINVAL, "a launch runs at most three passes");
  }
  if (b.tab && !(b.kpre <= 1 && b.kmid <= 1 && b.kpre + b.kmid > 0)) return fail(c, PAOS_EINVAL, "no table build of this pass shape");
  if (b.store == 1 && !b.tab) return fail(c, PAOS_EUNSUPPORTED, "no PSF-storing build of this pass shape");
  if (b.store == 2 && !b.tab) return fail(c, PAOS_EUNSUPPORTED, "no power-summing build of this pass shape");
  return fail(c, PAOS_EINVAL, "no build of this pass shape");
}

template <typename T, int N, int AXIS, int KPRE, int KMID, int STORE = 0, int LONG = 0, int ONE = 0, int LINES_ = 0, int TILES_ = 0>
struct FrugalGeometry {
  using C = FftCfg<T, N>;
  static constexpr bool kLatencyBound = PAOS_LONG_ONE_LINE != 0 && (LONG != 0 || ONE != 0) && STORE == 0 && sizeof(T) == 8;
  static constexpr bool kOneLine = kLatencyBound && N == 4096;
  static constexpr int OCC = (kLatencyBound && N == 2048) ? 1 : 0;
  static constexpr int LINES = LINES_ != 0 ? LINES_ : (kOneLine ? 1 : (AXIS == 0 ? C::FR_ROW_LINES : C::COL_LINES));
  static constexpr int TILES = TILES_ != 0 ? TILES_ : (AXIS == 0 ? C::ROW_TILES : C::COL_TILES);
  static constexpr bool SPLIT = sizeof(T) == 8 || LINES > 2;
  static constexpr int GROUPS = N / LINES / TILES, THREADS = TILES * LINES * N / C::E;
  static constexpr size_t LDS = frugal_lds_bytes<T, N, LINES, TILES, SPLIT, KPRE, KMID, C::E, STORE, OCC>();
  static constexpr unsigned ALIGN = (LINES == 1 && AXIS == 0) ? 32 : 16;
};

namespace {

template <typename T, int N, int AXIS, int KPRE, int KMID, int NFFT, int STORE, int TAB, int LONG, int ONE, int CH>
int frugal_launch(paos_ctx* c, const FrugalArgs& args) {
  using C = FftCfg<T, N>;
  using G = FrugalGeometry<T, N, AXIS, KPRE, KMID, STORE, LONG, ONE>;
  FrugalArgs a = args;
  unsigned groups = G::GROUPS;
  a.wg0 = 0;
  static_assert(G::GROUPS % G::ALIGN == 0, "TileMap renumbers tiles inside aligned groups of workgroups");
  if (a.live_hi > a.live_lo) {
    const unsigned per = G::LINES * G::TILES;
    a.wg0 = (a.live_lo / per) / G::ALIGN * G::ALIGN;
    unsigned end = ((a.live_hi + per - 1) / per + G::ALIGN - 1) / G::ALIGN * G::ALIGN;
    if (end > groups) end = groups;
    groups = end - a.wg0;
  }
  const dim3 grid(groups, c->batch), block(G::THREADS);
  constexpr size_t kMaxPad = 8192;
  const size_t lds = G::LDS + (c->lds_pad < kMaxPad ? c->lds_pad : kMaxPad);
  auto kern = frugal_pass_kernel<T, N, C::E, G::LINES, G::TILES, AXIS, C::BR, C::BC, G::SPLIT, KPRE, KMID, NFFT, STORE, TAB, LONG, G::OCC, CH>;
  ++(CH != 0 ? c->central_launches : c->plain_launches);
  return TIMED_LAUNCH(c, kern, grid, block, lds, G::LDS + kMaxPad, AXIS == 0 ? PAOS_KERNEL_PASS_ROWS : PAOS_KERNEL_PASS_COLS,
                      c->prof_next_tag, PAOS_FRUGAL_PASS(a));
}

constexpr int kFrugalFieldMax[] = {1, kFrugalMaxPre, kFrugalMaxMid, 2, 2, 1, 4, 1, 1};
template <typename T, int N, int X, int... V>
int frugal_unfold(paos_ctx* c, const FrugalBuild& b, const FrugalArgs& a) {
  constexpr int I = sizeof...(V), kFields = sizeof(kFrugalFieldMax) / sizeof(int);
  static_assert(kFields == kBuildFields, "one maximum per field");
  int field[kBuildFields];
  build_to_ints(b, field);
  if (field[I] != X) {
    if constexpr (X < kFrugalFieldMax[I]) return frugal_unfold<T, N, X + 1, V...>(c, b, a);
    else return frugal_not_built(c, b);
  } else if constexpr (I + 1 < kFields) {
    return frugal_unfold<T, N, 0, V..., X>(c, b, a);
  } else if constexpr (frugal_built<T, N>(FrugalBuild{V..., X})) {
    return frugal_launch<T, N, V..., X>(c, a);
  } else {
    return frugal_not_built(c, b);
  }
}
template <typename T, int N>
int frugal_dispatch(paos_ctx* c, const FrugalBuild& b, const FrugalArgs& a) {
  return frugal_unfold<T, N, 0>(c, b, a);
}

}
```

paos_amd/csrc/frugal_pass.h:

```cpp
#pragma once
#include "fft_kernels.h"
#include "pass_records.h"

#ifndef PAOS_FENCE_EVERY
#define PAOS_FENCE_EVERY 2
#endif

namespace paos {


template <int N, int E>
constexpr int twiddle_lds_entries() { return E <= 16 ? 256 : (N / 4 < 1024 ? N / 4 : 1024); }

#ifndef PAOS_STAMPS
#define PAOS_STAMPS 0
#endif
constexpr int kStampSlots = 12;

struct FrugalArgs {
  void* field;
  const void* tw;
  const FrugalItem* items;
  unsigned pitch, item_stride;
  double* psf;
  double* psf_partial;
  double* pow_partial;
  const double* dyn_scale;
#if PAOS_STAMPS
  unsigned long long* stamps;
#endif
  unsigned live_lo = 0, live_hi = 0, wg0 = 0;
};
#if PAOS_STAMPS
#define PAOS_STAMP(i)                                                                              \
  do {                                                                                             \
    if (threadIdx.x == 0)                                                                          \
      a.stamps[((size_t)blockIdx.y * gridDim.x + blockIdx.x) * kStampSlots + (i)] = __builtin_amdgcn_s_memtime(); \
  } while (0)
#define PAOS_STAMP_WAIT_VM() asm volatile("s_waitcnt vmcnt(0)" ::: "memory")
#else
#define PAOS_STAMP(i) do { } while (0)
#define PAOS_STAMP_WAIT_VM() do { } while (0)
#endif

constexpr int kCircleLds = 256;
template <bool TAIL = false>
__device__ __forceinline__ void sincos_tab(double a, const cx<double>* circle, double* sn, double* cs, double tail = 0.0) {
  const double kMagic = 6755399441055744.0;
  const double nb = fma(a, 40.743665431525205956834243423363677, kMagic);
  const unsigned j = (unsigned)__double2loint(nb) & (unsigned)(kCircleLds - 1);
  const double n = nb - kMagic;
  double r = fma(-n, 2.45436926061702596754894014318e-02, a);
  r = fma(-n, 9.56755311833869697380e-19, r);
  if constexpr (TAIL) r = __dadd_rn(r, tail);
  const cx<double> c = circle[j];
  const double z = r * r;
  const double ps = fma(z, 8.33333333333333333333e-03, -1.66666666666666666667e-01);
  const double s1 = fma(r * z, ps, r);
  double pc = fma(z, -1.38888888888888888889e-03, 4.16666666666666666667e-02);
  pc = fma(z, pc, -0.5);
  const double c1 = fma(z, pc, 1.0);
  *cs = fma(c.x, c1, -(c.y * s1));
  *sn = fma(c.y, c1, c.x * s1);
}

template <typename T>
__device__ __forceinline__ T flip_sign(T x, unsigned mask_hi) {
  if constexpr (sizeof(T) == 8)
    return __hiloint2double(__double2hiint(x) ^ (int)mask_hi, __double2loint(x));
  else
    return __uint_as_float(__float_as_uint(x) ^ mask_hi);
}

#ifndef PAOS_ROW_PRE
#define PAOS_ROW_PRE 2
#endif
#ifndef PAOS_COL_PRE
#define PAOS_COL_PRE 2
#endif
#ifndef PAOS_TABLE_FENCE
#define PAOS_TABLE_FENCE 8
#endif

__device__ __forceinline__ void lds_barrier() { asm volatile("s_waitcnt lgkmcnt(0)\n\ts_barrier" ::: "memory"); }

template <int K>
__device__ __forceinline__ cx<double> slot_factor(const double* g, const double* step, const double* across2,
                                                  const double* coefq, const double* m2, const cx<double>* circle) {
  cx<double> p = {1.0, 0.0};
  if constexpr (K == 2) {
    const double x0 = __dmul_rn(g[0], step[0]);
    const double q0 = __dmul_rn(m2[0], __dmul_rn(coefq[0], __dadd_rn(__dmul_rn(x0, x0), across2[0])));
    const double x1 = __dmul_rn(g[1], step[1]);
    const double q1 = __dmul_rn(m2[1], __dmul_rn(coefq[1], __dadd_rn(__dmul_rn(x1, x1), across2[1])));
    const double a = __dadd_rn(q0, q1);
    const double bb = __dsub_rn(a, q0);
    const double e = __dadd_rn(__dsub_rn(q0, __dsub_rn(a, bb)), __dsub_rn(q1, bb));
    double sn, cs;
    sincos_tab<true>(a, circle, &sn, &cs, e);
    return cx<double>{cs, sn};
  }
#pragma unroll
  for (int j = 0; j < K; ++j) {
    const double x = __dmul_rn(g[j], step[j]);
    const double s = __dadd_rn(__dmul_rn(x, x), across2[j]);
    const double q = __dmul_rn(m2[j], __dmul_rn(coefq[j], s));
    double sn, cs;
    sincos_tab(q, circle, &sn, &cs);
    p = j == 0 ? cx<double>{cs, sn} : cx<double>{fma(p.x, cs, -(p.y * sn)), fma(p.x, sn, p.y * cs)};
  }
  return p;
}

__device__ __forceinline__ float turn_fraction(double q) {
  const double k = rint(q * 0.15915494309189535);
  double r = fma(-k, 6.283185307179586, q);
  r = fma(-k, 2.4492935982947064e-16, r);
  return (float)(r * 0.15915494309189535);
}
template <int K>
__device__ __forceinline__ cx<float> slot_factor32(const double* g, const double* step, const double* across2,
                                                   const double* coefq, const double* m2) {
  cx<float> p = {1.0f, 0.0f};
  if constexpr (K == 2) {
    const double x0 = __dmul_rn(g[0], step[0]);
    const double q0 = __dmul_rn(m2[0], __dmul_rn(coefq[0], __dadd_rn(__dmul_rn(x0, x0), across2[0])));
    const double x1 = __dmul_rn(g[1], step[1]);
    const double q1 = __dmul_rn(m2[1], __dmul_rn(coefq[1], __dadd_rn(__dmul_rn(x1, x1), across2[1])));
    const double a = __dadd_rn(q0, q1);
    const double bb = __dsub_rn(a, q0);
    const double e = __dadd_rn(__dsub_rn(q0, __dsub_rn(a, bb)), __dsub_rn(q1, bb));
    const float frac = turn_fraction(a) + (float)(e * 0.15915494309189535);
    return cx<float>{__builtin_amdgcn_cosf(frac), __builtin_amdgcn_sinf(frac)};
  }
#pragma unroll
  for (int j = 0; j < K; ++j) {
    const double x = __dmul_rn(g[j], step[j]);
    const double q = __dmul_rn(m2[j], __dmul_rn(coefq[j], __dadd_rn(__dmul_rn(x, x), across2[j])));
    const float frac = turn_fraction(q);
    const float snf = __builtin_amdgcn_sinf(frac), csf = __builtin_amdgcn_cosf(frac);
    p = j == 0 ? cx<float>{csf, snf} : cmul_after_trans(p, cx<float>{csf, snf});
  }
  return p;
}

template <typename T, int N, int E, int K, typename Map, int PLAIN = 0, bool SHARE = false, int RECS = 0, int TAB = 0, int CH = 0>
__device__ __forceinline__ void frugal_slot(cx<T>* v, const FrugalSlot& sl, const FrugalPhase* ph,
                                            const Map& m, const cx<double>* circle, bool conj_in, bool conj_out, int tpos,
                                            void* area = nullptr, bool area_busy = false, const MaskLine* recs = nullptr,
                                            int lbase = 0, double extra_scale = 1.0) {
  if constexpr (PLAIN == 1) {
    static_assert(K == 0, "a plain slot has no phases");
    const unsigned mask = (conj_out != conj_in) ? 0x80000000u : 0u;
#pragma unroll
    for (int k = 0; k < E; ++k) v[k].y = flip_sign(v[k].y, mask);
    return;
  }
  if constexpr (PLAIN == 2) {
    static_assert(K == 0, "a plain slot has no phases");
    const unsigned mask = (conj_out != conj_in) ? 0x80000000u : 0u;
    const unsigned none = (sl.sign_on != 0.0) ? 0x80000000u : 0u;
#pragma unroll
    for (int k = 0; k < E; ++k) {
      v[k].x = flip_sign(v[k].x, none);
      v[k].y = flip_sign(v[k].y, mask);
      if ((k + 1) % PAOS_FENCE_EVERY == 0) __builtin_amdgcn_sched_barrier(0);
    }
    return;
  }
  constexpr int TL = N / E;
  static_assert(TL % 2 == 0, "the checkerboard sign is constant along a thread's elements");
  static_assert(CH == 0 || (K > 0 && TAB != 0 && sizeof(T) == 8 && E % 4 == 0), "central-half slots: complex128 table slots");
  constexpr int kFirst = CH != 0 ? E / 4 : 0, kEnd = CH != 0 ? 3 * E / 4 : E;
  const double sc = __dmul_rn(sl.scale, extra_scale);
  const int line = Map::kAxis == 0 ? m.row(0) : m.col(0);
  if (sl.mask_on != 0.0) {
    MaskLine ml;
    if constexpr (RECS > 0) {
      ml = recs[0];
#pragma unroll
      for (int j = 1; j < RECS; ++j)
        if (line - lbase == j) ml = recs[j];
    } else if constexpr (RECS < 0) {
      ml = recs[line - lbase];
    } else {
      ml = sl.lines[line];
    }
    constexpr int R = (kMaskW + TL - 1) / TL;
    const char* vb = reinterpret_cast<const char*>(sl.vals);
    const unsigned vlo = (unsigned)line * (unsigned)(2 * kMaskW * sizeof(double));
    auto val = [&](int idx) { return *reinterpret_cast<const double*>(vb + (vlo + (unsigned)idx * (unsigned)sizeof(double))); };
    const int ka = (int)((unsigned)(ml.p0 - tpos + TL - 1) / (unsigned)TL);
    const int kb = (int)((unsigned)(ml.p2 - tpos + TL - 1) / (unsigned)TL);
    double wa[R], wb[R];
    int sel_a[R], sel_b[R];
#pragma unroll
    for (int j = 0; j < R; ++j) {
      const int pa = tpos + (ka + j) * TL, pb = tpos + (kb + j) * TL;
      const bool hit_a = ka + j < E && pa < ml.p1, hit_b = kb + j < E && pb < ml.p3;
      wa[j] = val(hit_a ? pa - ml.p0 : 0);
      wb[j] = val(hit_b ? kMaskW + pb - ml.p2 : kMaskW);
      sel_a[j] = hit_a ? ka + j : -1;
      sel_b[j] = hit_b ? kb + j : -1;
    }
    const double w_in = __dmul_rn(sl.w_in, ml.lm), w_out = __dmul_rn(sl.w_out, ml.lm);
#pragma unroll
    for (int j = 0; j < R; ++j) { wa[j] = __dmul_rn(wa[j], ml.lm); wb[j] = __dmul_rn(wb[j], ml.lm); }
#pragma unroll
    for (int k = kFirst; k < kEnd; ++k) {
      const int pos = tpos + k * TL;
      double w = (pos >= ml.p1 && pos < ml.p2) ? w_in : w_out;
#pragma unroll
      for (int j = 0; j < R; ++j) {
        w = (k == sel_a[j]) ? wa[j] : w;
        w = (k == sel_b[j]) ? wb[j] : w;
      }
      if constexpr (sizeof(T) == 4) {
        const float wf = (float)w;
        v[k] = {(T)(v[k].x * wf), (T)(v[k].y * wf)};
      } else {
        v[k] = {(T)__dmul_rn((double)v[k].x, w), (T)__dmul_rn((double)v[k].y, w)};
      }
      if ((k + 1) % PAOS_FENCE_EVERY == 0) __builtin_amdgcn_sched_barrier(0);
    }
    __builtin_amdgcn_sched_barrier(0);
  }
  const int parity = sl.sign_on == 1.0 ? line + tpos : (sl.sign_on == 2.0 ? tpos : line);
  const double f = (sl.sign_on != 0.0 && (parity & 1)) ? -sc : sc;
  const double fy = (conj_out != conj_in) ? -f : f;
  const int qflip = conj_in ? (int)0x80000000 : 0;
  constexpr int KK = K > 0 ? K : 1;
  double across2[KK], step[KK], g_lo[KK], g_hi[KK], coefq[KK];
#pragma unroll
  for (int j = 0; j < K; ++j) {
    coefq[j] = __hiloint2double(__double2hiint(ph[j].coef) ^ qflip, __double2loint(ph[j].coef));
    const bool nat = ph[j].natural != 0.0;
    const int ga = nat ? ((line < N / 2) ? line : line - N) : line - N / 2;
    const double a = (double)ga * (Map::kAxis == 0 ? ph[j].sy : ph[j].sx);
    across2[j] = __dmul_rn(a, a);
    step[j] = Map::kAxis == 0 ? ph[j].sx : ph[j].sy;
    g_lo[j] = (double)(nat ? tpos : tpos - N / 2);
    g_hi[j] = (double)(nat ? tpos - N : tpos - N / 2);
  }
  const int mt = tpos == 0 ? 0 : TL - tpos;
  const int mbase = (tpos == 0 ? TL : 0) + mt;
  if constexpr (sizeof(T) == 4) {
    double m2s32[KK];
#pragma unroll
    for (int j = 0; j < K; ++j) m2s32[j] = ph[j].m2;
    const float ff = (float)f, ffy = (float)fy;
    auto factor32 = [&](int k) __attribute__((always_inline)) {
      double gk[KK];
#pragma unroll
      for (int j = 0; j < K; ++j) gk[j] = (k < E / 2 ? g_lo[j] : g_hi[j]) + (double)(k * TL);
      return slot_factor32<K>(gk, step, across2, coefq, m2s32);
    };
    if constexpr (K > 0 && TAB != 0) {
      static_assert(!SHARE, "a table slot does not stand for a barrier");
      const cx<float>* tb = reinterpret_cast<const cx<float>*>(sl.table) + tpos;
#pragma unroll
      for (int k = 0; k < E; ++k) {
        const cx<float> zs = scale2(cmul(cx<float>{(float)v[k].x, (float)v[k].y}, tb[k * TL]), ff, ffy);
        v[k] = {(T)zs.x, (T)zs.y};
        if ((k + 1) % PAOS_TABLE_FENCE == 0) __builtin_amdgcn_sched_barrier(0);
      }
      return;
    }
    if constexpr (SHARE && K > 0) {
      cx<float>* fac = reinterpret_cast<cx<float>*>(area);
      if (area_busy) lds_barrier();
#pragma unroll
      for (int k = 0; k < E / 2; ++k) {
        const cx<float> p = factor32(k);
        fac[k * TL + tpos] = p;
        constexpr bool kFresh = K <= 2;
        const cx<float> zs = scale2(kFresh ? cmul_after_trans(cx<float>{(float)v[k].x, (float)v[k].y}, p)
                                           : cmul(cx<float>{(float)v[k].x, (float)v[k].y}, p), ff, ffy);
        v[k] = {(T)zs.x, (T)zs.y};
        if ((k + 1) % PAOS_FENCE_EVERY == 0) __builtin_amdgcn_sched_barrier(0);
      }
      if (tpos == 0) fac[(E / 2) * TL] = factor32(E / 2);
      lds_barrier();
#pragma unroll
      for (int k = E / 2; k < E; ++k) {
        const cx<float> p = fac[(E - 1 - k) * TL + mbase];
        const cx<float> zs = scale2(cmul(cx<float>{(float)v[k].x, (float)v[k].y}, p), ff, ffy);
        v[k] = {(T)zs.x, (T)zs.y};
      }
      lds_barrier();
      return;
    }
#pragma unroll
    for (int k = 0; k < E; ++k) {
      cx<float> z = {(float)v[k].x, (float)v[k].y};
      if constexpr (K > 0) z = cmul_after_trans(z, factor32(k));
      const cx<float> zs = scale2(z, ff, ffy);
      v[k] = {(T)zs.x, (T)zs.y};
      if ((k + 1) % PAOS_FENCE_EVERY == 0) __builtin_amdgcn_sched_barrier(0);
    }
    return;
  }
  double m2s[KK];
#pragma unroll
  for (int j = 0; j < K; ++j) m2s[j] = ph[j].m2;
  auto factor = [&](int k) __attribute__((always_inline)) {
    double gk[KK];
#pragma unroll
    for (int j = 0; j < K; ++j) gk[j] = (k < E / 2 ? g_lo[j] : g_hi[j]) + (double)(k * TL);
    return slot_factor<K>(gk, step, across2, coefq, m2s, circle);
  };
  auto apply = [&](int k, cx<double> p) __attribute__((always_inline)) {
    const cx<double> vd = {(double)v[k].x, (double)v[k].y};
    v[k] = {(T)(fma(vd.x, p.x, -(vd.y * p.y)) * f), (T)(fma(vd.x, p.y, vd.y * p.x) * fy)};
  };
  if constexpr (K > 0 && TAB != 0) {
    static_assert(!SHARE, "a table slot does not stand for a barrier");
    const cx<double>* tb = sl.table + tpos;
    constexpr int kFence = Map::kLinesPerWorkgroup == 1 ? 4 : PAOS_TABLE_FENCE;
#pragma unroll
    for (int k = kFirst; k < kEnd; ++k) {
      apply(k, tb[k * TL]);
      if ((k - kFirst + 1) % kFence == 0) __builtin_amdgcn_sched_barrier(0);
    }
    return;
  }
  if constexpr (SHARE && K > 0) {
    cx<double>* fac = reinterpret_cast<cx<double>*>(area);
    if (area_busy) lds_barrier();
#pragma unroll
    for (int k = 0; k < E / 2; ++k) {
      const cx<double> p = factor(k);
      fac[k * TL + tpos] = p;
      apply(k, p);
      if ((k + 1) % PAOS_FENCE_EVERY == 0) __builtin_amdgcn_sched_barrier(0);
    }
    if (tpos == 0) fac[(E / 2) * TL] = factor(E / 2);
    lds_barrier();
#pragma unroll
    for (int k = E / 2; k < E; ++k) {
      apply(k, fac[(E - 1 - k) * TL + mbase]);
      if ((k + 1) % PAOS_FENCE_EVERY == 0) __builtin_amdgcn_sched_barrier(0);
    }
    lds_barrier();
    return;
  }
#pragma unroll
  for (int k = 0; k < E; ++k) {
    if constexpr (K > 0) apply(k, factor(k));
    else v[k] = {(T)((double)v[k].x * f), (T)((double)v[k].y * fy)};
    if ((k + 1) % PAOS_FENCE_EVERY == 0) __builtin_amdgcn_sched_barrier(0);
  }
}

struct PhaseTableArgs {
  const FrugalItem* items;
  const cx<double>* tw;
  const PhaseSlotDesc* desc;
  int n;
  int f32;
};
template <int UNIT = 0>
__global__ void __launch_bounds__(256) phase_table_kernel(PhaseTableArgs a) {
  __shared__ cx<double> circle[kCircleLds];
  if (!a.f32) {
    const cx<double> w = a.tw[threadIdx.x * (a.n / kCircleLds)];
    circle[threadIdx.x] = {w.x, -w.y};
  }
  __syncthreads();
  const PhaseSlotDesc d = a.desc[blockIdx.z];
  const FrugalItem& it = a.items[d.item_base + blockIdx.y];
  const bool mid = d.mid != 0;
  const FrugalSlot& sl = mid ? it.mid : it.pre;
  if (it.active == 0.0 || sl.table == nullptr) return;
  const FrugalPhase* ph = mid ? it.mid_ph : it.pre_ph;
  const int K = d.k;
  const int qflip = (mid && it.fft1_on != 0.0 && it.fft1_inv != 0.0) ? (int)0x80000000 : 0;
  const int pos = blockIdx.x * blockDim.x + threadIdx.x;
  double g[kFrugalMaxMid], step[kFrugalMaxMid], across2[kFrugalMaxMid], coefq[kFrugalMaxMid], m2[kFrugalMaxMid];
#pragma unroll
  for (int j = 0; j < kFrugalMaxMid; ++j) {
    const FrugalPhase& q = ph[j < K ? j : 0];
    g[j] = (double)(q.natural != 0.0 ? (pos < a.n / 2 ? pos : pos - a.n) : pos - a.n / 2);
    step[j] = d.axis == 0 ? q.sx : q.sy;
    across2[j] = 0.0;
    coefq[j] = __hiloint2double(__double2hiint(q.coef) ^ qflip, __double2loint(q.coef));
    m2[j] = q.m2;
  }
  if (a.f32) {
    cx<float> pf = {1.0f, 0.0f};
    if (K <= 0) {}
    else if (K == 1) pf = slot_factor32<1>(g, step, across2, coefq, m2);
    else if (K == 2) pf = slot_factor32<2>(g, step, across2, coefq, m2);
    else pf = slot_factor32<3>(g, step, across2, coefq, m2);
    reinterpret_cast<cx<float>*>(const_cast<cx<double>*>(sl.table))[pos] = pf;
    return;
  }
  cx<double> p = {1.0, 0.0};
  if (K <= 0) {}
  else if (K == 1) p = slot_factor<1>(g, step, across2, coefq, m2, circle);
  else if (K == 2) p = slot_factor<2>(g, step, across2, coefq, m2, circle);
  else p = slot_factor<3>(g, step, across2, coefq, m2, circle);
  const_cast<cx<double>*>(sl.table)[pos] = p;
}

template <bool NT, typename T>
__device__ __forceinline__ cx<T> stream_load(const cx<T>* p) {
  typedef T vec2 __attribute__((ext_vector_type(2)));
  if constexpr (NT) {
    const vec2 t = __builtin_nontemporal_load(reinterpret_cast<const vec2*>(p));
    return {t.x, t.y};
  } else {
    return *p;
  }
}
template <bool NT, typename T>
__device__ __forceinline__ void stream_store(cx<T>* p, cx<T> v) {
  typedef T vec2 __attribute__((ext_vector_type(2)));
  if constexpr (NT) __builtin_nontemporal_store(vec2{v.x, v.y}, reinterpret_cast<vec2*>(p));
  else *p = v;
}

template <typename T, int N, int E, bool SPLIT, bool FLIP = true, int CH = 0>
__device__ __forceinline__ void frugal_fft(cx<T>* v, void* lds, int t, const cx<T>* tw, const cx<double>* circle,
                                           double inv, const cx<T>* w1_last = nullptr) {
  fft_stages<T, N, E, +1, SPLIT, 1, 1, CH>(v, lds, t, tw, circle, w1_last);
  unpermute_slots<N, E>(v);
  if constexpr (FLIP) {
    const unsigned mask = inv != 0.0 ? 0x80000000u : 0u;
#pragma unroll
    for (int k = 0; k < E; ++k) v[k].y = flip_sign(v[k].y, mask);
  }
  __builtin_amdgcn_sched_barrier(0);
}

constexpr size_t kStoreScratch = 16 * sizeof(double);
template <int LINES, int TILES, int KPRE>
constexpr int frugal_record_mode() {
  return (TILES * LINES == 2 && KPRE == 0) ? 2 : (TILES * LINES <= 16 ? 1 : 0);
}
template <typename T, int N, int E, int LINES, int TILES, int OCC = 0>
constexpr bool frugal_tw_in_regs() {
  return sizeof(T) == 8 && E == 16 && ((N == 4096 && TILES * LINES == 1) || (N == 2048 && OCC != 0 && TILES * LINES == 2) ||
                                       (N == 1024 && OCC != 0 && TILES * LINES == 4));
}
template <typename T, int N, int LINES, int TILES, bool SPLIT, int KPRE, int KMID, int E = 16, int STORE = 0, int OCC = 0>
constexpr size_t frugal_lds_bytes() {
  return (size_t)TILES * LINES * line_lds_bytes<T, N, SPLIT, LINES>() +
         (frugal_tw_in_regs<T, N, E, LINES, TILES, OCC>() ? 0 : twiddle_lds_entries<N, E>() * sizeof(cx<T>)) +
         (sizeof(T) == 8 ? kCircleLds * sizeof(cx<double>) : 0) + kStoreScratch +
         (frugal_record_mode<LINES, TILES, KPRE>() == 1 ? (size_t)TILES * LINES * sizeof(MaskLine) : 0);
}

#ifndef PAOS_MINW_SMALL
#define PAOS_MINW_SMALL 3
#endif
#ifndef PAOS_F32_MINW
#define PAOS_F32_MINW 4
#endif
template <typename T, int N, int THREADS, int OCC = 0>
constexpr int frugal_min_waves() {
  if (OCC != 0) return 4;
  if (sizeof(T) == 4 && THREADS >= 1024) return 8;
  if (sizeof(T) == 4 && THREADS >= 512) return PAOS_F32_MINW;
  if (sizeof(T) == 8 && N == 4096 && THREADS == 256) return 4;
  return THREADS >= 512 ? 4 : PAOS_MINW_SMALL;
}

template <int THREADS>
__device__ __forceinline__ void tile_power_out(double acc, double* scratch, double* out) {
#pragma unroll
  for (int off = 32; off > 0; off >>= 1) acc += __shfl_down(acc, off, 64);
  if ((threadIdx.x & 63) == 0) scratch[threadIdx.x >> 6] = acc;
  __syncthreads();
  if (threadIdx.x == 0) {
    double s = 0.0;
#pragma unroll
    for (int w = 0; w < THREADS / 64; ++w) s += scratch[w];
    *out = s;
  }
}

#if PAOS_STAMPS
#define PAOS_FRUGAL_PARAMS const FrugalItem *k_items, void *k_field, unsigned k_pitch, unsigned k_item_stride, unsigned k_wg0, \
                           const void *k_tw, double *k_psf, double *k_psf_partial, double *k_pow_partial, const double *k_dyn_scale, \
                           unsigned long long *k_stamps
#define PAOS_FRUGAL_PASS(a) (a).items, (a).field, (a).pitch, (a).item_stride, (a).wg0, (a).tw, (a).psf, (a).psf_partial, (a).pow_partial, (a).dyn_scale, (a).stamps
#else
#define PAOS_FRUGAL_PARAMS const FrugalItem *k_items, void *k_field, unsigned k_pitch, unsigned k_item_stride, unsigned k_wg0, \
                           const void *k_tw, double *k_psf, double *k_psf_partial, double *k_pow_partial, const double *k_dyn_scale
#define PAOS_FRUGAL_PASS(a) (a).items, (a).field, (a).pitch, (a).item_stride, (a).wg0, (a).tw, (a).psf, (a).psf_partial, (a).pow_partial, (a).dyn_scale
#endif
template <typename T, int N, int E, int LINES, int TILES, int AXIS, int BR, int BC, bool SPLIT,
          int KPRE, int KMID, int NFFT, int STORE = 0, int TAB = 0, int LONG = 0, int OCC = 0, int CH = 0>
__global__ void __launch_bounds__(TILES* LINES* N / E, (frugal_min_waves<T, N, TILES * LINES * N / E, OCC>()))
    frugal_pass_kernel(PAOS_FRUGAL_PARAMS) {
  static_assert(LONG == 0 || (TAB != 0 && NFFT == 2 && KPRE == 1 && KMID == 1), "LONG builds: see above");
  static_assert(CH == 0 || (sizeof(T) == 8 && N == 4096 && E == 16 && TAB != 0 && KPRE == 1 && NFFT <= 2), "CH builds: see above");
  FrugalArgs a;
  a.items = k_items; a.field = k_field; a.pitch = k_pitch; a.item_stride = k_item_stride; a.wg0 = k_wg0;
  a.tw = k_tw; a.psf = k_psf; a.psf_partial = k_psf_partial; a.pow_partial = k_pow_partial; a.dyn_scale = k_dyn_scale; a.live_lo = a.live_hi = 0;
#if PAOS_STAMPS
  a.stamps = k_stamps;
#endif
  const int item = blockIdx.y;
  typedef const __attribute__((address_space(4))) FrugalItem* ConstItemPtr;
  const FrugalItem& it = *(const FrugalItem*)((ConstItemPtr)a.items + item);
  constexpr int kThreads = TILES * LINES * N / E;
  constexpr int kTwiddleLds = twiddle_lds_entries<N, E>();
  constexpr int kTwIt = (kTwiddleLds + kThreads - 1) / kThreads;
  constexpr int kClIt = sizeof(T) == 8 ? (kCircleLds + kThreads - 1) / kThreads : 1;
  constexpr int kExtra = (LONG + 1) / 2;
  const FrugalItem& it_last = LONG == 0 ? it : *(const FrugalItem*)((ConstItemPtr)a.items + item + kExtra * gridDim.y);
  const double h_active = it.active, h_line_lo = it.line_lo, h_line_hi = it.line_hi, h_line_fill = it_last.line_fill,
               h_pos_lo = it.pos_lo, h_pos_hi = it.pos_hi, h_spos_lo = it_last.spos_lo, h_spos_hi = it_last.spos_hi;
  const double h_mask_on = it.mid.mask_on;
  const MaskLine* const h_lines = it.mid.lines;
  const double h_dyn = *((const __attribute__((address_space(4))) double*)a.dyn_scale + item);
  if constexpr (frugal_record_mode<LINES, TILES, KPRE>() != 0)
    asm volatile("" ::"s"(h_active), "s"(h_line_lo), "s"(h_line_hi), "s"(h_line_fill), "s"(h_pos_lo), "s"(h_pos_hi), "s"(h_spos_lo),
                 "s"(h_spos_hi), "s"(h_mask_on), "s"(h_lines), "s"(h_dyn));
  else
    asm volatile("" ::"s"(h_active), "s"(h_line_lo), "s"(h_line_hi), "s"(h_line_fill), "s"(h_pos_lo), "s"(h_pos_hi), "s"(h_spos_lo),
                 "s"(h_spos_hi), "s"(h_dyn));
  if (h_active == 0.0) return;
  extern __shared__ __attribute__((aligned(16))) unsigned char smem[];
  constexpr bool kBlockIsLine = BR * BC * sizeof(cx<T>) >= 128;
  constexpr int COLSIB = (kBlockIsLine ? 1 : (int)(128 / (BR * BC * sizeof(cx<T>)))) * (AXIS == 1 && LINES < BC ? BC / LINES : 1);
  const unsigned wg = blockIdx.x + a.wg0;
  const TileMap<N, E, LINES, TILES, AXIS, BR, BC, 1, COLSIB> m(wg, threadIdx.x, a.pitch);
  cx<T>* f = reinterpret_cast<cx<T>*>(a.field) + (size_t)item * a.item_stride;
  constexpr bool NT = kBlockIsLine && ((AXIS == 1 && LINES >= BC) || (AXIS == 0 && LINES == BR));
  const int l0 = TILES == 1 ? (AXIS == 0 ? m.row0 : m.col0) : (int)wg * (TILES * LINES);
  {
    if (l0 + TILES * LINES <= (int)h_line_lo || l0 >= (int)h_line_hi) {
      if constexpr (STORE == 1) {
        if (h_line_fill == 0.0) return;
        if (l0 + TILES * LINES <= (int)h_spos_lo || l0 >= (int)h_spos_hi) return;
        double* ps = a.psf + (size_t)item * a.item_stride;
#pragma unroll
        for (int k = 0; k < E; ++k) ps[m.base + (unsigned)k * m.stride] = 0.0;
        if (threadIdx.x == 0) a.psf_partial[(size_t)item * (N / LINES / TILES) + wg] = 0.0;
        return;
      }
      if (h_line_fill != 0.0) {
#pragma unroll
        for (int k = 0; k < E; ++k)
          stream_store<NT>(reinterpret_cast<cx<T>*>(reinterpret_cast<char*>(f) + (m.base + (unsigned)k * m.stride) * (unsigned)sizeof(cx<T>)),
                           cx<T>{(T)0, (T)0});
      }
      return;
    }
  }
  void* lds = smem + (size_t)m.lds_line * line_lds_bytes<T, N, SPLIT, LINES>();
  cx<T>* tw_lds = reinterpret_cast<cx<T>*>(smem + (size_t)TILES * LINES * line_lds_bytes<T, N, SPLIT, LINES>());
  constexpr bool kTwRegs = frugal_tw_in_regs<T, N, E, LINES, TILES, OCC>();
  const cx<T>* tw = kTwRegs ? reinterpret_cast<const cx<T>*>(a.tw) : tw_lds;
  cx<double>* cl = reinterpret_cast<cx<double>*>(tw_lds + (kTwRegs ? 0 : kTwiddleLds));
  const cx<double>* circle = sizeof(T) == 8 ? cl : nullptr;
#if PAOS_STAMPS
  if (threadIdx.x == 0) {
    unsigned long long* st = a.stamps + ((size_t)blockIdx.y * gridDim.x + blockIdx.x) * kStampSlots;
    st[8] = __builtin_amdgcn_s_memrealtime();
    st[9] = ((unsigned long long)__builtin_amdgcn_s_getreg((31 << 11) | 20) << 32) | __builtin_amdgcn_s_getreg((31 << 11) | 4);
  }
#endif
  PAOS_STAMP(0);

  const char* fb = reinterpret_cast<const char*>(f);
  const unsigned boff = m.base * (unsigned)sizeof(cx<T>);
  const size_t bstride = (size_t)(m.stride * (unsigned)sizeof(cx<T>));
  auto at = [&](int k) {
    const unsigned long long u = (unsigned long long)(fb + (size_t)k * bstride);
    const unsigned lo = (unsigned)__builtin_amdgcn_readfirstlane((int)(unsigned)u);
    const unsigned hi = (unsigned)__builtin_amdgcn_readfirstlane((int)(unsigned)(u >> 32));
    typedef __attribute__((address_space(1))) char* GlobalBytes;
    unsigned bo = boff;
    asm volatile("" : "+v"(bo));
    return (cx<T>*)((GlobalBytes)(((unsigned long long)hi << 32) | lo) + bo);
  };
  constexpr int kRecMode = frugal_record_mode<LINES, TILES, KPRE>();
  constexpr int kRecs = kRecMode == 2 ? 2 : 0;
  MaskLine mrec[kRecs > 0 ? kRecs : 1] = {};
  const int lbase = __builtin_amdgcn_readfirstlane(l0);
  if constexpr (kRecs > 0) {
    if (h_mask_on != 0.0) {
#pragma unroll
      for (int j = 0; j < kRecs; ++j) mrec[j] = h_lines[lbase + j];
    }
  }
  constexpr int kPlainPre = KPRE != 0 ? 0 : (AXIS == 1 ? PAOS_COL_PRE : PAOS_ROW_PRE);
  cx<T> v[E];
  const int plo = (int)h_pos_lo, phi = (int)h_pos_hi;
  if constexpr (CH != 0) {
#pragma unroll
    for (int k = 0; k < E; ++k) v[k] = cx<T>{(T)0, (T)0};
#pragma unroll
    for (int k = E / 4; k < 3 * E / 4; ++k) {
      const int pos = m.t + k * (N / E);
      if (pos >= plo && pos < phi) v[k] = stream_load<NT>(at(k));
    }
  } else if (plo <= 0 && phi >= N) {
#pragma unroll
    for (int k = 0; k < E; ++k) v[k] = stream_load<NT>(at(k));
  } else {
#pragma unroll
    for (int k = 0; k < E; ++k) {
      const int pos = m.t + k * (N / E);
      v[k] = cx<T>{(T)0, (T)0};
      if (pos >= plo && pos < phi) v[k] = stream_load<NT>(at(k));
    }
  }
  __builtin_amdgcn_sched_barrier(0);
  cx<T> tw_fetch[kTwIt], cl_fetch[kClIt];
  constexpr int kRecDwords = kRecMode == 1 ? TILES * LINES * (int)(sizeof(MaskLine) / 4) : 0;
  static_assert(kRecDwords <= 128, "the record area is filled by the first 128 threads");
  const bool stage_recs = kRecMode == 1 && h_mask_on != 0.0;
  unsigned rec_fetch = 0;
  if constexpr (kRecMode == 1) {
    if (stage_recs && (int)threadIdx.x < kRecDwords) rec_fetch = reinterpret_cast<const unsigned*>(h_lines + lbase)[threadIdx.x];
  }
  constexpr int kLastTpt = E / last_radix<N, E>();
  cx<T> w1_keep[kLastTpt];
#pragma unroll
  for (int q = 0; q < kLastTpt; ++q) w1_keep[q] = cx<T>{(T)1, (T)0};
  if constexpr (kTwRegs) {
#pragma unroll
    for (int q = 0; q < kLastTpt; ++q) w1_keep[q] = reinterpret_cast<const cx<T>*>(a.tw)[m.t + q * (N / E)];
  }
  const cx<T>* const w1_last = kTwRegs ? w1_keep : nullptr;
#pragma unroll
  for (int j = 0; j < kTwIt; ++j) {
    const int i = (int)threadIdx.x + j * kThreads;
    tw_fetch[j] = cx<T>{(T)0, (T)0};
    if (!kTwRegs && i < kTwiddleLds) tw_fetch[j] = reinterpret_cast<const cx<T>*>(a.tw)[i];
  }
  if constexpr (sizeof(T) == 8) {
#pragma unroll
    for (int j = 0; j < kClIt; ++j) {
      const int i = (int)threadIdx.x + j * kThreads;
      cl_fetch[j] = cx<T>{(T)0, (T)0};
      if (i < kCircleLds) cl_fetch[j] = reinterpret_cast<const cx<T>*>(a.tw)[i * (N / kCircleLds)];
    }
  }
#pragma unroll
  for (int j = 0; j < kTwIt; ++j) {
    const int i = (int)threadIdx.x + j * kThreads;
    if (!kTwRegs && i < kTwiddleLds) tw_lds[i] = tw_fetch[j];
  }
  if constexpr (sizeof(T) == 8) {
#pragma unroll
    for (int j = 0; j < kClIt; ++j) {
      const int i = (int)threadIdx.x + j * kThreads;
      if (i < kCircleLds) cl[i] = {(double)cl_fetch[j].x, -(double)cl_fetch[j].y};
    }
  }
  MaskLine* rec_lds = reinterpret_cast<MaskLine*>(smem + frugal_lds_bytes<T, N, LINES, TILES, SPLIT, KPRE, KMID, E, 0, OCC>() -
                                                  (kRecMode == 1 ? (size_t)TILES * LINES * sizeof(MaskLine) : 0));
  if constexpr (kRecMode == 1) {
    if (stage_recs && (int)threadIdx.x < kRecDwords) reinterpret_cast<unsigned*>(rec_lds)[threadIdx.x] = rec_fetch;
  }
  asm volatile("s_waitcnt lgkmcnt(0)\n\ts_barrier" ::: "memory");
  PAOS_STAMP_WAIT_VM();
  PAOS_STAMP(1);

  const bool ran1 = it.fft1_on != 0.0;
  const bool ran2 = NFFT == 2 && it.fft2_on != 0.0;
  const bool inv1 = ran1 && it.fft1_inv != 0.0;
  constexpr bool kShare = TAB == 0;
  frugal_slot<T, N, E, KPRE, decltype(m), kPlainPre, kShare && KMID == 0, 0, TAB, CH>(v, it.pre, it.pre_ph, m, circle, false, inv1, m.t, lds, false);
  PAOS_STAMP(2);
  if (ran1) frugal_fft<T, N, E, SPLIT, false, CH>(v, lds, m.t, tw, circle, it.fft1_inv, w1_last);
  PAOS_STAMP(3);
  constexpr bool kShareMid = kShare && KPRE == 0 && KMID < 3;
  frugal_slot<T, N, E, KMID, decltype(m), 0, kShareMid, (kRecMode == 1 ? -1 : kRecs), TAB>(
      v, it.mid, it.mid_ph, m, circle, inv1, ran2 && it.fft2_inv != 0.0, m.t, lds, ran1, kRecMode == 1 ? rec_lds : mrec, lbase, h_dyn);
  PAOS_STAMP(4);
  if constexpr (NFFT == 2) {
    if (ran2) {
      if (ran1 && !(kShareMid && KMID > 0)) __syncthreads();
      frugal_fft<T, N, E, SPLIT>(v, lds, m.t, tw, circle, it.fft2_inv, w1_last);
    }
  }
  if constexpr (LONG != 0) {
    bool busy = ran1 || ran2;
#define PAOS_EXTRA_PASS(ix, kTwo)                                                                                                    \
  {                                                                                                                                  \
    const bool ran3 = (ix).fft1_on != 0.0;                                                                                           \
    const bool ran4 = (kTwo) && (ix).fft2_on != 0.0;                                                                                 \
    const bool inv3 = ran3 && (ix).fft1_inv != 0.0;                                                                                  \
    frugal_slot<T, N, E, 1, decltype(m), 0, false, 0, TAB>(v, (ix).pre, (ix).pre_ph, m, circle, false, inv3, m.t, lds, false);       \
    if (ran3) {                                                                                                                      \
      if (busy) __syncthreads();                                                                                                     \
      frugal_fft<T, N, E, SPLIT, false>(v, lds, m.t, tw, circle, (ix).fft1_inv, w1_last);                                            \
      busy = true;                                                                                                                   \
    }                                                                                                                                \
    frugal_slot<T, N, E, 1, decltype(m), 0, false, 0, TAB>(v, (ix).mid, (ix).mid_ph, m, circle, inv3, ran4 && (ix).fft2_inv != 0.0,  \
                                                           m.t, lds, ran3);                                                          \
    if constexpr (kTwo) {                                                                                                            \
      if (ran4) {                                                                                                                    \
        if (busy) __syncthreads();                                                                                                   \
        frugal_fft<T, N, E, SPLIT>(v, lds, m.t, tw, circle, (ix).fft2_inv, w1_last);                                                 \
        busy = true;                                                                                                                 \
      }                                                                                                                              \
    }                                                                                                                                \
  }
    const FrugalItem& it2 = *(const FrugalItem*)((ConstItemPtr)a.items + item + gridDim.y);
    if constexpr (LONG == 1) PAOS_EXTRA_PASS(it2, false)
    else PAOS_EXTRA_PASS(it2, true)
    if constexpr (LONG == 3) PAOS_EXTRA_PASS(it_last, false)
    if constexpr (LONG == 4) PAOS_EXTRA_PASS(it_last, true)
#undef PAOS_EXTRA_PASS
  }
  PAOS_STAMP(5);
  [[maybe_unused]] double* const scratch = reinterpret_cast<double*>(
      smem + frugal_lds_bytes<T, N, LINES, TILES, SPLIT, KPRE, KMID, E, 0, OCC>() - kStoreScratch - (kRecMode == 1 ? (size_t)TILES * LINES * sizeof(MaskLine) : 0));
  if constexpr (STORE == 1) {
    double* ps = a.psf + (size_t)item * a.item_stride;
    double acc = 0.0;
#pragma unroll
    for (int k = 0; k < E; ++k) {
      const double x = (double)v[k].x, y = (double)v[k].y;
      const double w = __dadd_rn(__dmul_rn(x, x), __dmul_rn(y, y));
      ps[m.base + (unsigned)k * m.stride] = w;
      acc += w;
    }
    tile_power_out<TILES * LINES * N / E>(acc, scratch, a.psf_partial + (size_t)item * (N / LINES / TILES) + wg);
    return;
  }
  const int slo = (int)h_spos_lo, shi = (int)h_spos_hi;
  if (slo <= 0 && shi >= N) {
#pragma unroll
    for (int k = 0; k < E; ++k) stream_store<NT>(at(k), v[k]);
  } else {
#pragma unroll
    for (int k = 0; k < E; ++k) {
      const int pos = m.t + k * (N / E);
      if (pos >= slo && pos < shi) stream_store<NT>(at(k), v[k]);
    }
  }
  if constexpr (STORE == 2) {
    double acc = 0.0;
#pragma unroll
    for (int k = 0; k < E; ++k) {
      const double x = (double)v[k].x, y = (double)v[k].y;
      acc += __dadd_rn(__dmul_rn(x, x), __dmul_rn(y, y));
    }
    tile_power_out<TILES * LINES * N / E>(acc, scratch, a.pow_partial + (size_t)item * (N / LINES / TILES) + wg);
  }
  PAOS_STAMP(6);
  PAOS_STAMP_WAIT_VM();
  PAOS_STAMP(7);
#if PAOS_STAMPS
  if (threadIdx.x == 0)
    a.stamps[((size_t)blockIdx.y * gridDim.x + blockIdx.x) * kStampSlots + 10] = __builtin_amdgcn_s_memrealtime();
#endif
}

}
```

paos_amd/csrc/host.h:

```cpp
#pragma once
#include "../../include/paos_hip.h"

#include <hip/hip_runtime.h>

#include <cstdlib>
#include <string>
#include <type_traits>
#include <vector>

#include "arena_layout.h"
#include "frugal_pass.h"
#include "pass_records.h"

using namespace paos;

#ifndef PAOS_BR
#define PAOS_BR 4
#endif
#ifndef PAOS_PAD_BLOCKS
#define PAOS_PAD_BLOCKS 3
#endif
inline constexpr int BR = PAOS_BR;
#ifndef PAOS_F32_BR
#define PAOS_F32_BR 8
#endif
template <typename T, int N>
constexpr int block_rows() { return (sizeof(T) == 4 && N >= 2048) ? PAOS_F32_BR : PAOS_BR; }
inline constexpr int kNormSlots = PAOS_NORM_SLOTS;
template <typename T>
struct Lay {
  static constexpr int BC = 2;
};

constexpr int kArenaSlabs = 4;
struct Arena {
  double* host = nullptr;
  double* dev = nullptr;
  ArenaLayout lay;
  int cur = 0;
  int left = -1;
  hipEvent_t fence[kArenaSlabs] = {};
  bool fenced[kArenaSlabs] = {};
  bool used[kArenaSlabs] = {};
};

struct paos_ctx {
  int device = 0, n = 0, batch = 0, precision = 0;
  int br = PAOS_BR;
  unsigned pitch = 0, item_stride = 0;
  hipStream_t stream = nullptr;
  double* psf = nullptr;
  void* focus_spec = nullptr;
  bool focus_open = false;
  void* otf_spec = nullptr;
  bool otf_computed = false, otf_valid = false;
  double* otf_cuts = nullptr;
  std::vector<double> blur_tabs, blur_key;
  cx<double>* zoom_t = nullptr;
  double* zoom_psf = nullptr;
  cx<double>* zoom_field = nullptr;
  int zoom_m = 0;
  bool zoom_done = false, zoom_has_field = false;
  double* zoom_tabs = nullptr;
  int zoom_s = 0, zoom_cap = 0;
  std::vector<double> zoom_fracs;
  std::vector<std::vector<int>> zoom_carry;
  double* map_dev = nullptr;
  unsigned long long map_key = 0;
  double map_max = 0.0;
  std::vector<double> start_key;
  double* start_norm2 = nullptr;
  std::vector<double> start_partial_key;
  double* start_partial = nullptr;
  cx<double>* psd_scratch = nullptr;
  int* psd_bad = nullptr;
  double* psf_partial = nullptr;
  int psf_nparts = 0;
  double* pow_partial = nullptr;
  int pow_nparts = 0;
  cx<double>* ptab = nullptr;
  int ptab_slots = 0;
  double* dyn_scale = nullptr;
  bool dyn_pending = false;
  unsigned long long deferred_rode = 0, deferred_settled = 0;
  bool norm2_of_field = false;
  int psf_zero_axis = -1;
  std::vector<double> psf_zero_lo, psf_zero_hi;
  bool det_set = false;
  int det_nx = 0, det_ny = 0;
  double det_geom[4] = {};
  double* det_img = nullptr;
  double* det_rows = nullptr;
  size_t det_rows_bytes = 0;
  double* det_out = nullptr;
  size_t det_out_bytes = 0;
  double* ee_buf = nullptr;
  size_t ee_bytes = 0;
  int ee_bins = 0, ee_curves = 0;
  bool ee_computed = false, ee_valid = false;
  double* wf_buf = nullptr;
  size_t wf_bytes = 0;
  int wf_pairs = 0;
  bool wf_fitted = false;
  void* bounce[2] = {nullptr, nullptr};
  hipEvent_t bounce_ev[2] = {nullptr, nullptr};
  void* field = nullptr;
  void* tw = nullptr;
  void* staging = nullptr;
  cx<double>* tables = nullptr;
  double* mask = nullptr;
  double* metric_partial = nullptr;
  double* metric_out = nullptr;
  double* metric_host = nullptr;
  struct MaskSet {
    MaskLine* lines = nullptr;
    double* vals = nullptr;
    std::vector<double> key;
    unsigned long long used = 0;
    int line_lo = 0, line_hi = 0;
  };
  static constexpr int kMaskSets = 8;
  MaskSet mask_sets[kMaskSets];
  unsigned long long mask_clock = 0;
  unsigned long long mask_hits = 0, mask_rendered = 0;
  size_t lds_pad = 0;
  bool central_half = true;
  unsigned long long central_launches = 0, plain_launches = 0;
  std::vector<int> pass_builds;
  int* mask_overflow = nullptr;
  double* partial = nullptr;
  double* norm2 = nullptr;
  double* norm2_host = nullptr;
  bool prune = true;
  int norm_slot = 0;
  bool norm_busy[64] = {};
  int nparts = 0;
  Arena arena;
  std::string err;
  int prof_kind = -1;
  std::vector<hipEvent_t> prof_events;
  std::vector<int> prof_tags;
  int prof_next_tag = 0;
  double prof_next_bytes = 0.0;
  std::vector<double> prof_bytes;
  double prof_next_lines = 0.0;
  std::vector<double> prof_lines;
  size_t prof_used = 0;
};

#pragma GCC visibility push(hidden)

int fail(paos_ctx* c, int code, const std::string& msg);

#define HIPCHK(c, call)                                                                     \
  do {                                                                                      \
    hipError_t e_ = (call);                                                                 \
    if (e_ != hipSuccess)                                                                   \
      return fail((c), PAOS_EHIP,                                                           \
                  std::string(#call) + ": " + hipGetErrorString(e_) + " (" __FILE__ ":" +   \
                      std::to_string(__LINE__) + ")");                                      \
  } while (0)

inline size_t elem_bytes(const paos_ctx* c) { return c->precision == PAOS_F64 ? 16 : 8; }

inline bool env_is(const char* name, char ch) {
  const char* e = getenv(name);
  return e && e[0] == ch;
}

template <typename T, int N>
struct FftCfg {
  static constexpr int BC = Lay<T>::BC;
  static constexpr int BR = block_rows<T, N>();
  static constexpr int E = 16;
  static constexpr int ROW_LINES = (N >= 2048) ? PAOS_BR / 2 : PAOS_BR;
  static constexpr int FR_ROW_LINES = (N >= 2048) ? BR / 2 : BR;
  static constexpr int COL_LINES = BC;
  static constexpr int ROW_THREADS = ROW_LINES * N / E, COL_THREADS = COL_LINES * N / E;
  static constexpr int ROW_TILES = (ROW_THREADS >= 128) ? 1 : 128 / ROW_THREADS;
  static constexpr int COL_TILES = (COL_THREADS >= 128) ? 1 : 128 / COL_THREADS;
  static constexpr bool ROW_SPLIT = (size_t)ROW_LINES * ROW_TILES * line_lds_bytes<T, N, false>() > 144 * 1024;
  static constexpr bool COL_SPLIT = (size_t)COL_LINES * COL_TILES * line_lds_bytes<T, N, false>() > 144 * 1024;
  static constexpr int MINW = 1;
};
inline int frugal_tile_lines(const paos_ctx* c, int axis) { return axis == 0 ? (c->n >= 2048 ? c->br / 2 : c->br) : 2; }

int arena_reserve(paos_ctx* c, size_t total);
int arena_push(paos_ctx* c, const double* src, size_t count, const double** dev);
class ArenaBatch {
 public:
  explicit ArenaBatch(paos_ctx* c) : c_(c) {}
  int begin(size_t total);
  int add(const double* src, size_t count, const double** dev);
  int commit();

 private:
  paos_ctx* c_;
  ArenaBatchState st_;
};
int arena_settled(paos_ctx* c, int rc);
int copy_to_host(paos_ctx* c, void* host, const void* dev, size_t bytes);
int next_norm_slot(paos_ctx* c);
int check_mask_overflow(paos_ctx* c);
int check_rows(paos_ctx* c, const double* rows);
std::vector<double> rounded_cols(const paos_ctx* c, const double* cols);
int opt_in_lds(paos_ctx* c, const void* kern, size_t lds);
bool timed_launch_begin(paos_ctx* c, int kind);
hipError_t timed_launch_end(paos_ctx* c, int tag);

int launch_failed(paos_ctx* c, const char* call, hipError_t e, const char* file, int line);
#define TIMED_LAUNCH(c, ...) timed_launch(__FILE__, __LINE__, (c), __VA_ARGS__)
template <typename Kern, typename... Args>
int timed_launch(const char* file, int line, paos_ctx* c, Kern kern, dim3 grid, dim3 block, size_t lds, size_t lds_opt_in, int kind,
                 int tag, Args... args) {
  if (lds_opt_in) {
    int rc = opt_in_lds(c, (const void*)kern, lds_opt_in);
    if (rc) return rc;
  }
  const bool timed = timed_launch_begin(c, kind);
  hipLaunchKernelGGL(kern, grid, block, lds, c->stream, args...);
  hipError_t e = hipGetLastError();
  if (e != hipSuccess) return launch_failed(c, "hipGetLastError()", e, file, line);
  if (timed && (e = timed_launch_end(c, tag)) != hipSuccess) return launch_failed(c, "timed_launch_end(c, tag)", e, file, line);
  return PAOS_OK;
}
inline size_t generic_lds_opt_in(size_t lds) { return lds > 48 * 1024 ? lds : 0; }

template <typename F>
int dispatch_n(paos_ctx* c, F&& f) {
  switch (c->n) {
#define PAOS_N_CASE(N) case N: return f(std::integral_constant<int, N>{})
    PAOS_N_CASE(64);
    PAOS_N_CASE(128);
    PAOS_N_CASE(256);
    PAOS_N_CASE(512);
    PAOS_N_CASE(1024);
    PAOS_N_CASE(2048);
    PAOS_N_CASE(4096);
#undef PAOS_N_CASE
  }
  return fail(c, PAOS_EUNSUPPORTED, "grid size must be a power of two in 64..4096");
}

template <typename F>
auto dispatch_block_rows(const paos_ctx* c, F&& f) {
  if (c->br == PAOS_F32_BR) return f(std::integral_constant<int, PAOS_F32_BR>{});
  return f(std::integral_constant<int, PAOS_BR>{});
}
template <typename F>
auto dispatch_layout(const paos_ctx* c, F&& f) {
  if (c->precision == PAOS_F64) return f(double{}, std::integral_constant<int, PAOS_BR>{});
  return dispatch_block_rows(c, [&](auto br) { return f(float{}, br); });
}
template <int A, int B, typename F>
auto dispatch_either(bool first, F&& f) {
  if (first) return f(std::integral_constant<int, A>{});
  return f(std::integral_constant<int, B>{});
}

int run_passes(paos_ctx* c, const paos_pass* passes, int n_passes, const double* blocks, int n_blocks,
               const double* entry_rows = nullptr, bool entry_stale = false, int* final_ticket = nullptr, int final_mode = 1,
               const double* entry_cols = nullptr);
int mask_render_mode();
bool mask_rect_blocks();

int generic_pass(paos_ctx* c, int axis, const PassArgs& a, int feat);

template <typename T, int N>
int frugal_family(paos_ctx* c, const FrugalBuild& b, const FrugalArgs& a);

int settle_scale(paos_ctx* c, bool field_is_overwritten = false);
int dyn_scale_reset(paos_ctx* c);
int zero_outside_rows(paos_ctx* c, const double* live_rows);
int zero_outside_box(paos_ctx* c, const double* live_rows, const double* live_cols);
int power_ring_full(paos_ctx* c);
int take_power_ticket(paos_ctx* c, const double* partial, int nparts, const double* source, int* ticket);
int psf_keep_power_impl(paos_ctx* c, int* ticket);
struct MaskRender {
  const double *params, *shared;
  int set, axis, line0, line_end, shapes;
};
constexpr int kMaskRenders = 8;
int render_mask_records(paos_ctx* c, const MaskRender* jobs, int count);
int render_mask_weights(paos_ctx* c, const double* ap);
int pointwise_pass(paos_ctx* c, const PassArgs& a);

#define SETTLE_SCALE(c) do { if (c) { (c)->norm2_of_field = false; if ((c)->dyn_pending) { int rc_ = settle_scale(c); if (rc_) return rc_; } } } while (0)
#define DROP_SCALE(c) do { if (c) { (c)->norm2_of_field = false; if ((c)->dyn_pending) { int rc_ = settle_scale(c, true); if (rc_) return rc_; } } } while (0)

#pragma GCC visibility pop
```

paos_amd/csrc/pass_program.h:

```cpp
#pragma once
#include "../../include/paos_hip.h"

#include <cmath>
#include <cstddef>
#include <cstring>
#include <vector>

#include "pass_records.h"

#pragma GCC visibility push(hidden)

using namespace paos;

struct PlanDims {
  int n, batch, br;
  int precision;
  int central_half;
};
struct PlanSwitches {
  bool line_tables = true;
  bool fuse_pairs = true;
  bool compact_grid = true;
  bool env_prune = true;
  bool stage_program = true;
  bool batched_records = true;
  bool psf_zero_reuse = true;
  bool ctx_prune = true;
};

struct OpList {
  const paos_pw_op* ops;
  int count;
};
inline OpList op_list(const paos_pass& p, int l) {
  return l == 0 ? OpList{p.pre, p.n_pre} : (l == 1 ? OpList{p.mid, p.n_mid} : OpList{p.post, p.n_post});
}
inline bool is_phase(const paos_pw_op& op) { return op.kind == PAOS_PW_QPHASE_CENTRED || op.kind == PAOS_PW_QPHASE_NATURAL; }

enum PhaseCheck { PHASES_OK = 0, PHASE_BLOCK_OUT_OF_RANGE, PHASE_TOO_LARGE };
inline PhaseCheck check_phase_args(const PlanDims& d, const paos_pass* passes, int n_passes, const double* blocks, int n_blocks) {
  for (int i = 0; i < n_passes; ++i)
    for (int l = 0; l < 3; ++l) {
      const OpList ol = op_list(passes[i], l);
      for (int o = 0; o < ol.count && o < PAOS_MAX_PW; ++o) {
        const paos_pw_op& op = ol.ops[o];
        if (!is_phase(op)) continue;
        if (op.block < 0 || op.block >= n_blocks) return PHASE_BLOCK_OUT_OF_RANGE;
        for (int it = 0; it < d.batch; ++it) {
          const double* p = blocks + ((size_t)op.block * d.batch + it) * FP_STRIDE;
          if (p[FP_ENABLE] == 0.0) continue;
          const double hx = 0.5 * d.n * p[FP_SX], hy = 0.5 * d.n * p[FP_SY];
          double arg = std::fabs(p[FP_COEF]) * (hx * hx + hy * hy);
          if (op.flags & PAOS_PWF_MUL2PI) arg *= 6.283185307179586;
          if (!(arg < kMaxPhaseArg)) return PHASE_TOO_LARGE;
        }
      }
    }
  return PHASES_OK;
}

inline bool lower_frugal(const PlanDims& d, const paos_pass& p, const double* blocks , LoweredPass& lp) {
  std::vector<FrugalItem>& items = lp.items;
  int &kpre = lp.kpre, &kmid = lp.kmid, &nfft = lp.nfft, &mask_block = lp.mask_block, &mask_slot = lp.mask_slot;
  std::vector<double>& mask_shared = lp.mask_shared;
  std::vector<int>& mask_rep = lp.mask_rep;
  if (p.axis != 0 && p.axis != 1) return false;
  if (p.fft1 < 0 || p.n_post != 0) return false;
  const OpList lists[2] = {op_list(p, 0), op_list(p, 1)};
  int k[2] = {0, 0};
  mask_block = -1; mask_slot = -1;
  for (int l = 0; l < 2; ++l)
    for (int o = 0; o < lists[l].count; ++o) {
      const int kind = lists[l].ops[o].kind;
      if (is_phase(lists[l].ops[o])) {
        ++k[l];
        for (int it = 0; it < d.batch; ++it) {
          const double* q = blocks + ((size_t)lists[l].ops[o].block * d.batch + it) * FP_STRIDE;
          if (q[FP_ENABLE] != 0.0 && std::fabs(q[FP_SGN]) != 1.0) return false;
        }
      }
      else if (kind == PAOS_PW_MASK) {
        if (mask_block >= 0) return false;
        mask_block = lists[l].ops[o].block; mask_slot = l;
      } else if (kind != PAOS_PW_SIGN && kind != PAOS_PW_SCALE) return false;
    }
  if (k[0] > kFrugalMaxPre || k[1] > kFrugalMaxMid) return false;
  if (mask_block >= 0) {
    for (int it = 0; it < d.batch; ++it) {
      const double* q = blocks + ((size_t)mask_block * d.batch + it) * FP_STRIDE;
      const double* q2 = blocks + ((size_t)(mask_block + 1) * d.batch + it) * FP_STRIDE;
      if (q[0] == 0.0) continue;
      const double a = q[3], b = q[4], theta = q2[0], obsc = q2[1], subpix = q2[2], shape = q2[3];
      if (theta != 0.0 || !(a > 0.0) || !(b > 0.0)) return false;
      if (shape == PAOS_SHAPE_ELLIPSE) {
        const double along = p.axis == 0 ? a : b, across = p.axis == 0 ? b : a;
        if (!(across >= 2.0) || 2.0 * along * std::sqrt(3.0 / across) + 8.0 > kMaskW) return false;
      } else {
        const int sp = (int)subpix;
        if (obsc != 0.0 || sp <= 0 || (sp & (sp - 1)) != 0) return false;
      }
    }
  }
  kpre = k[0]; kmid = k[1]; nfft = p.fft2 >= 0 ? 2 : 1;
  items.assign(d.batch, FrugalItem{});
  mask_shared.assign(d.batch, 0.0);
  mask_rep.assign(d.batch, -1);
  auto blk = [&](int b, int it) { return blocks + ((size_t)b * d.batch + it) * FP_STRIDE; };
  for (int it = 0; it < d.batch; ++it) {
    FrugalItem& fi = items[it];
    const double* c1 = blk(p.fft1, it);
    fi.fft1_on = c1[FC_ENABLE] != 0.0; fi.fft1_inv = c1[FC_INVERSE] != 0.0;
    if (p.fft2 >= 0) { const double* c2 = blk(p.fft2, it); fi.fft2_on = c2[FC_ENABLE] != 0.0; fi.fft2_inv = c2[FC_INVERSE] != 0.0; }
    bool active = fi.fft1_on != 0.0 || fi.fft2_on != 0.0;
    FrugalSlot* slots[2] = {&fi.pre, &fi.mid};
    FrugalPhase* phases[2] = {fi.pre_ph, fi.mid_ph};
    int sign_bits[2] = {0, 0};
    for (int l = 0; l < 2; ++l) {
      slots[l]->sign_on = 0.0; slots[l]->scale = 1.0;
      sign_bits[l] = 0;
      slots[l]->mask_on = 0.0; slots[l]->w_in = 1.0; slots[l]->w_out = 0.0;
      slots[l]->lines = nullptr; slots[l]->vals = nullptr;
      int j = 0;
      for (int o = 0; o < lists[l].count; ++o) {
        const paos_pw_op& op = lists[l].ops[o];
        const double* q = blk(op.block, it);
        const bool on = q[FP_ENABLE] != 0.0;
        active = active || on;
        if (op.kind == PAOS_PW_MASK) {
          const double* q2 = blk(op.block + 1, it);
          slots[l]->mask_on = on ? 1.0 : 0.0;
          const bool obsc = q2[1] != 0.0 && q2[3] == PAOS_SHAPE_ELLIPSE;
          slots[l]->w_in = obsc ? 0.0 : 1.0; slots[l]->w_out = obsc ? 1.0 : 0.0;
          int rep = it;
          for (int j = 0; j < it; ++j)
            if (!std::memcmp(blk(op.block, j), q, FP_STRIDE * sizeof(double)) &&
                !std::memcmp(blk(op.block + 1, j), q2, FP_STRIDE * sizeof(double))) { rep = j; break; }
          mask_shared[it] = rep != it ? 1.0 : 0.0;
          mask_rep[it] = rep;
        } else if (op.kind == PAOS_PW_SIGN) {
          if (on) {
            const bool x_only = op.flags & PAOS_PWF_X_ONLY, y_only = op.flags & PAOS_PWF_Y_ONLY;
            const int along = p.axis == 0 ? (y_only ? 0 : 1) : (x_only ? 0 : 1);
            const int across = p.axis == 0 ? (x_only ? 0 : 1) : (y_only ? 0 : 1);
            sign_bits[l] ^= along | (across << 1);
          }
        }
        else if (op.kind == PAOS_PW_SCALE) { if (on) slots[l]->scale *= q[FP_COEF]; }
        else {
          FrugalPhase& ph = phases[l][j++];
          ph.natural = op.kind == PAOS_PW_QPHASE_NATURAL ? 1.0 : 0.0;
          if (on) { ph.sx = q[FP_SX]; ph.sy = q[FP_SY]; ph.coef = q[FP_COEF] * q[FP_SGN]; ph.sgn = 1.0; ph.m2 = (op.flags & PAOS_PWF_MUL2PI) ? 6.283185307179586 : 1.0; }
          else { ph.sx = ph.sy = 0.0; ph.coef = 0.0; ph.sgn = 1.0; ph.m2 = 1.0; }
        }
      }
      slots[l]->sign_on = sign_bits[l] == 3 ? 1.0 : (sign_bits[l] == 1 ? 2.0 : (sign_bits[l] == 2 ? 3.0 : 0.0));
    }
    fi.active = active ? 1.0 : 0.0;
    fi.line_lo = 0.0; fi.line_hi = (double)d.n; fi.line_fill = 0.0; fi.pos_lo = 0.0; fi.pos_hi = (double)d.n;
    fi.spos_lo = 0.0; fi.spos_hi = (double)d.n;
  }
  if (kpre == 0)
    for (const FrugalItem& fi : items)
      if (fi.active != 0.0 && (fi.pre.sign_on != 0.0 || fi.pre.scale != 1.0 || fi.pre.mask_on != 0.0)) { kpre = 1; break; }
  return true;
}


inline bool mask_live_range(const PlanDims& d, const double* q, const double* q2, int axis, int* lo, int* hi) {
  if (q[0] == 0.0 || q2[0] != 0.0 || q2[1] != 0.0) return false;
  const double centre = axis == 0 ? q[2] : q[1];
  double ext = axis == 0 ? q[4] : q[3];
  if (q2[3] != PAOS_SHAPE_ELLIPSE) ext = ext / 2.0;
  if (!std::isfinite(centre) || !std::isfinite(ext) || !(ext > 0.0)) return false;
  const double a = std::floor(centre - ext + 0.5) - 1.0, b = std::ceil(centre + ext + 0.5) + 1.0;
  const int n = d.n;
  int l = a < 0.0 ? 0 : (a > n ? n : (int)a), h = b < 0.0 ? 0 : (b > n ? n : (int)b);
  const int br = d.br;
  l = (l / br) * br;
  h = ((h + br - 1) / br) * br;
  if (h > n) h = n;
  if (l >= h) { l = 0; h = br; }
  *lo = l; *hi = h;
  return true;
}

struct LineRange { int lo, hi; };

inline void plan_pruning(const PlanDims& d, const paos_pass* passes, int n_passes, const double* blocks,
                         std::vector<LoweredPass>& low, const double* entry_rows, bool entry_stale, const double* entry_cols) {
  const int n = d.n, br = d.br;
  auto meet = [br](LineRange a, LineRange b) {
    LineRange r{a.lo > b.lo ? a.lo : b.lo, a.hi < b.hi ? a.hi : b.hi};
    if (r.lo >= r.hi) { r.lo = a.lo; r.hi = a.lo + br < a.hi ? a.lo + br : a.hi; }
    return r;
  };
  std::vector<int> act;
  std::vector<LineRange> lines, loads;
  for (int it = 0; it < d.batch; ++it) {
    act.clear();
    for (int q = 0; q < n_passes; ++q)
      if (low[q].items[it].active != 0.0) act.push_back(q);
    if (act.empty()) continue;
    LineRange box[2] = {{0, n}, {0, n}};
    bool clean = false;
    LineRange rows0{0, n};
    if (entry_rows) {
      int l = (int)entry_rows[2 * it], h = (int)entry_rows[2 * it + 1];
      l = l < 0 ? 0 : (l / br) * br;
      h = h > n ? n : ((h + br - 1) / br) * br;
      if (h > n) h = n;
      if (l < h && (l > 0 || h < n)) { box[0] = {l, h}; clean = !entry_stale; }
      rows0 = box[0];
    }
    if (entry_cols && entry_stale) {
      int l = (int)entry_cols[2 * it], h = (int)entry_cols[2 * it + 1];
      l = l < 0 ? 0 : (l / br) * br;
      h = h > n ? n : ((h + br - 1) / br) * br;
      if (h > n) h = n;
      if (l < h && (l > 0 || h < n)) box[1] = {l, h};
    }
    lines.assign(act.size(), LineRange{0, n});
    loads.assign(act.size(), LineRange{0, n});
    for (size_t k = 0; k < act.size(); ++k) {
      const int q = act[k], ax = passes[q].axis;
      const FrugalItem& fi = low[q].items[it];
      LineRange& L = box[ax];
      LineRange& P = box[1 - ax];
      LineRange ml{0, n}, mp{0, n};
      bool masked = false;
      if (low[q].mask_block >= 0) {
        const double* mq = blocks + ((size_t)low[q].mask_block * d.batch + it) * FP_STRIDE;
        const double* mq2 = blocks + ((size_t)(low[q].mask_block + 1) * d.batch + it) * FP_STRIDE;
        masked = mask_live_range(d, mq, mq2, ax, &ml.lo, &ml.hi) && mask_live_range(d, mq, mq2, 1 - ax, &mp.lo, &mp.hi);
      }
      if (masked) L = meet(L, ml);
      lines[k] = L;
      LineRange pos = P;
      if (masked && low[q].mask_slot == 0) pos = meet(pos, mp);
      loads[k] = pos;
      if (fi.fft1_on != 0.0) pos = {0, n};
      if (masked && low[q].mask_slot == 1) pos = meet(pos, mp);
      if (low[q].nfft >= 2 && fi.fft2_on != 0.0) pos = {0, n};
      P = pos;
    }
    LineRange want[2] = {{0, n}, {0, n}};
    for (size_t k = act.size(); k-- > 0;) {
      const int q = act[k], ax = passes[q].axis;
      FrugalItem& fi = low[q].items[it];
      const LineRange proc = meet(lines[k], want[ax]);
      fi.line_lo = proc.lo; fi.line_hi = proc.hi;
      fi.pos_lo = loads[k].lo; fi.pos_hi = loads[k].hi;
      fi.spos_lo = want[1 - ax].lo; fi.spos_hi = want[1 - ax].hi;
      want[ax] = proc;
      want[1 - ax] = loads[k];
    }
    for (size_t k = 0; k < act.size(); ++k) {
      const FrugalItem& fi = low[act[k]].items[it];
      if (passes[act[k]].axis != 0 || (int)fi.line_lo != rows0.lo || (int)fi.line_hi != rows0.hi || fi.spos_lo > 0.0 ||
          fi.spos_hi < (double)n)
        clean = false;
    }
    FrugalItem& last = low[act.back()].items[it];
    if ((last.line_lo > 0.0 || last.line_hi < (double)n) && !clean) last.line_fill = 1.0;
  }
}

inline void record_window(const PlanDims& d, LoweredPass& lp) {
  double lo = (double)d.n, hi = 0.0;
  for (const FrugalItem& fi : lp.items) {
    if (fi.active == 0.0) continue;
    lo = fi.line_lo < lo ? fi.line_lo : lo;
    hi = fi.line_hi > hi ? fi.line_hi : hi;
  }
  const bool window = hi > lo;
  lp.mask_lo = window ? (int)lo : 0;
  lp.mask_hi = window ? (int)hi : d.n;
}

inline bool entry_zero_first(const PlanDims& d, bool pruned, const std::vector<LoweredPass>& low, const double* entry_rows,
                             const double* entry_cols) {
  bool need = !pruned;
  for (int it = 0; it < d.batch && !need; ++it) {
    bool active = false;
    for (const LoweredPass& lp : low) active = active || lp.items[it].active != 0.0;
    need = !active;
  }
  const double* windows[2] = {entry_rows, entry_cols};
  for (int w = 0; w < 2 && !need; ++w)
    for (int it = 0; windows[w] && it < d.batch && !need; ++it) {
      const int br = d.br, l = ((int)windows[w][2 * it] / br) * br;
      int h = (((int)windows[w][2 * it + 1] + br - 1) / br) * br;
      if (h > d.n) h = d.n;
      need = l >= h;
    }
  return need;
}

inline int last_pass_store(const std::vector<LoweredPass>& low, int final_mode) {
  if (final_mode == 0 || low.empty()) return 0;
  const LoweredPass& last = low.back();
  bool ok = last.ok && last.kpre <= 1 && (final_mode == 2 || last.kmid <= 1);
  if (ok)
    for (const FrugalItem& fi : last.items) ok = ok && fi.active != 0.0;
  return ok ? final_mode : 0;
}

inline void psf_zero_fill(const PlanDims& d, const PlanSwitches& sw, int axis, std::vector<FrugalItem>& last, int known_axis,
                          std::vector<double>& zero_lo, std::vector<double>& zero_hi) {
  const bool known = sw.psf_zero_reuse && known_axis == axis && (int)zero_lo.size() == d.batch;
  zero_lo.resize(d.batch); zero_hi.resize(d.batch);
  for (int it = 0; it < d.batch; ++it) {
    const double old_lo = known ? zero_lo[it] : 0.0, old_hi = known ? zero_hi[it] : (double)d.n;
    const bool covered = old_lo >= last[it].line_lo && old_hi <= last[it].line_hi;
    last[it].line_fill = covered ? 0.0 : 1.0;
    last[it].spos_lo = covered ? 0.0 : old_lo;
    last[it].spos_hi = covered ? (double)d.n : old_hi;
    zero_lo[it] = last[it].line_lo; zero_hi[it] = last[it].line_hi;
  }
}

inline std::vector<int> batched_renderings(const PlanSwitches& sw, bool all_frugal, const std::vector<LoweredPass>& low) {
  std::vector<int> todo;
  bool safe = sw.batched_records && all_frugal;
  for (int q = 0; q < (int)low.size() && safe; ++q) {
    if (low[q].mask_block < 0) continue;
    if (low[q].mask_render) {
      for (int r = 0; r < q; ++r) safe = safe && !(low[r].mask_block >= 0 && low[r].mask_set == low[q].mask_set);
      todo.push_back(q);
    }
  }
  if (!safe || todo.size() <= 1) todo.clear();
  return todo;
}

inline bool phases_along_lines(const PlanSwitches& sw, int axis, const LoweredPass& lp, bool or_none = false) {
  if (!sw.line_tables || (lp.kpre + lp.kmid == 0 && !or_none)) return false;
  const int counts[2] = {lp.kpre, lp.kmid};
  for (int l = 0; l < 2; ++l)
    for (const FrugalItem& fi : lp.items) {
      if (fi.active == 0.0) continue;
      const FrugalPhase* ph = l == 0 ? fi.pre_ph : fi.mid_ph;
      for (int j = 0; j < counts[l]; ++j)
        if ((axis == 0 ? ph[j].sy : ph[j].sx) != 0.0) return false;
    }
  return true;
}

inline bool can_fuse_pair(const PlanDims& d, const PlanSwitches& sw, int axis, const LoweredPass& lp, int axis2, const LoweredPass& lp2) {
  if (!sw.fuse_pairs) return false;
  if (!lp.ok || !lp2.ok || axis != axis2 || lp.nfft != 2) return false;
  if (lp.mask_block >= 0 && lp2.mask_block >= 0 && lp.mask_set == lp2.mask_set) return false;
  if (!phases_along_lines(sw, axis, lp, true) || !phases_along_lines(sw, axis2, lp2, true)) return false;
  for (int it = 0; it < d.batch; ++it) {
    const FrugalItem &f1 = lp.items[it], &f2 = lp2.items[it];
    if ((f1.active != 0.0) != (f2.active != 0.0)) return false;
    if (f1.active != 0.0 && (f1.line_lo != f2.line_lo || f1.line_hi != f2.line_hi || f1.line_fill != 0.0)) return false;
  }
  return true;
}

struct Launch {
  LoweredPass* lp[3] = {nullptr, nullptr, nullptr};
  int q = 0, count = 1, axis = 0;
  bool tables = false;
  size_t item_base = 0;
  int store = 0;
  FrugalBuild build{};
  unsigned live_lo = 0, live_hi = 0;
  int tag = 0;
  double bytes = 0.0, lines = 0.0;
  const LoweredPass& last() const { return *lp[count - 1]; }
};

inline std::vector<Launch> form_launches(const PlanDims& d, const PlanSwitches& sw, const paos_pass* passes, int n_passes,
                                         std::vector<LoweredPass>& low, bool fusable, std::vector<int>& launch_of) {
  std::vector<Launch> launches;
  launch_of.assign(n_passes, -1);
  for (int q = 0; q < n_passes;) {
    Launch g;
    g.q = q; g.axis = passes[q].axis; g.lp[0] = &low[q];
    if (low[q].ok && fusable) {
      const bool pair = q + 1 < n_passes && can_fuse_pair(d, sw, passes[q].axis, low[q], passes[q + 1].axis, low[q + 1]);
      const bool triple = pair && q + 2 < n_passes && can_fuse_pair(d, sw, passes[q + 1].axis, low[q + 1], passes[q + 2].axis, low[q + 2]) &&
                          !(low[q].mask_block >= 0 && low[q + 2].mask_block >= 0 && low[q].mask_set == low[q + 2].mask_set);
      g.count = triple ? 3 : (pair ? 2 : 1);
      for (int k = 1; k < g.count; ++k) g.lp[k] = &low[q + k];
    }
    launch_of[q] = (int)launches.size();
    launches.push_back(g);
    q += g.count;
  }
  return launches;
}

inline bool stage_whole_program(const PlanDims& d, const PlanSwitches& sw, bool all_frugal, int n_passes) {
  const size_t table_bytes = (size_t)2 * n_passes * d.batch * d.n * 2 * sizeof(double);
  return all_frugal && sw.stage_program && table_bytes <= (size_t(1) << 30);
}

inline void decide_tables(const PlanDims& d, const PlanSwitches& sw, Launch& g) {
  g.tables = g.count > 1 || (d.precision == PAOS_F64 && phases_along_lines(sw, g.axis, *g.lp[0]));
  if (g.tables && g.count == 1) {
    double lines = 0.0, active = 0.0;
    for (const FrugalItem& fi : g.lp[0]->items)
      if (fi.active != 0.0) { lines += fi.line_hi - fi.line_lo; active += 1.0; }
    if (active > 0.0 && lines > 0.5 * active * d.n) g.tables = false;
  }
}

inline bool build_exists(const PlanDims& d, const FrugalBuild& b) {
  return dispatch_family(d.precision, d.n, false, [&](auto t, auto n) { return frugal_built<decltype(t), decltype(n)::value>(b); });
}

inline FrugalBuild pick_build(const PlanDims& d, const Launch& g) {
  const LoweredPass& lp = *g.lp[0];
  const LoweredPass *next = g.lp[1], *next2 = g.lp[2];
  FrugalBuild b{};
  b.axis = g.axis;
  b.kpre = next ? 1 : (g.tables && lp.kpre > 1 ? 1 : lp.kpre);
  b.kmid = next ? 1 : (g.tables && lp.kmid > 1 ? 1 : lp.kmid);
  b.nfft = lp.nfft >= 2 ? 2 : 1;
  b.store = g.store;
  b.tab = g.tables ? 1 : 0;
  b.fuse = next2 ? 2 + next2->nfft : (next ? next->nfft : 0);
  if (!g.tables || g.store != 0) return b;
  bool light = !next, central = d.central_half, any = false;
  for (const FrugalItem& fi : lp.items) {
    if (fi.active == 0.0) continue;
    any = true;
    light = light && 2.0 * (fi.pos_hi - fi.pos_lo) <= (double)d.n && 2.0 * (fi.spos_hi - fi.spos_lo) <= (double)d.n;
    central = central && 4.0 * fi.pos_lo >= (double)d.n && 4.0 * fi.pos_hi <= 3.0 * (double)d.n;
  }
  b.one_line = light ? 1 : 0;
  if (!build_exists(d, b)) b.one_line = 0;
  b.central = central && any ? 1 : 0;
  if (!build_exists(d, b)) b.central = 0;
  return b;
}

inline void finish_launch(const PlanDims& d, const PlanSwitches& sw, Launch& g, int store) {
  g.store = store;
  g.build = pick_build(d, g);
  const bool store_psf = store == 1;
  const LoweredPass& lp = *g.lp[0];
  {
    double lo = (double)d.n, hi = 0.0;
    bool fill = false;
    for (const FrugalItem& fi : g.last().items) {
      if (fi.active == 0.0) continue;
      lo = fi.line_lo < lo ? fi.line_lo : lo;
      hi = fi.line_hi > hi ? fi.line_hi : hi;
      if (fi.line_fill != 0.0 && store_psf) {
        lo = fi.spos_lo < lo ? fi.spos_lo : lo;
        hi = fi.spos_hi > hi ? fi.spos_hi : hi;
      } else {
        fill = fill || fi.line_fill != 0.0;
      }
    }
    g.live_lo = g.live_hi = 0;
    if (sw.compact_grid && !fill && hi > lo && (lo > 0.0 || hi < (double)d.n)) {
      g.live_lo = (unsigned)lo;
      g.live_hi = (unsigned)hi;
    }
  }
  const double elem = d.precision == PAOS_F64 ? 16.0 : 8.0;
  g.tag = store_psf ? 8 : 0;
  g.bytes = 0.0;
  g.lines = 0.0;
  if (g.count > 1) g.tag |= g.count > 2 ? 32 : 16;
  for (int it = 0; it < d.batch; ++it) {
    const FrugalItem& fi = lp.items[it];
    const FrugalItem& fo = g.last().items[it];
    if (fi.active == 0.0) continue;
    if (fi.line_lo > 0.0 || fi.line_hi < (double)d.n) g.tag |= 1;
    if (fi.pos_lo > 0.0 || fi.pos_hi < (double)d.n) g.tag |= 2;
    if (!store_psf && (fo.spos_lo > 0.0 || fo.spos_hi < (double)d.n)) g.tag |= 4;
    g.bytes += (fi.line_hi - fi.line_lo) * ((fi.pos_hi - fi.pos_lo) * elem + (store_psf ? (double)d.n * 8.0 : (fo.spos_hi - fo.spos_lo) * elem));
    for (int k = 0; k < g.count; ++k) {
      const FrugalItem& fk = g.lp[k]->items[it];
      g.lines += (fi.line_hi - fi.line_lo) * ((fk.fft1_on != 0.0 ? 1.0 : 0.0) + (g.lp[k]->nfft >= 2 && fk.fft2_on != 0.0 ? 1.0 : 0.0));
    }
  }
}

#pragma GCC visibility pop
```

paos_amd/csrc/passes.hip:

```cpp
#include "frugal_launch.h"

#include <algorithm>
#include <cmath>
#include <cstdio>
#include <cstring>

#include "pass_program.h"
#include "phase_tables.h"

namespace {

int check_ops(paos_ctx* c, const paos_pw_op* ops, int count, int n_blocks) {
  if (count < 0 || count > PAOS_MAX_PW) return fail(c, PAOS_EINVAL, "too many pointwise operators in a pass");
  for (int o = 0; o < count; ++o) {
    if (ops[o].kind < PAOS_PW_SIGN || ops[o].kind > PAOS_PW_MASK) return fail(c, PAOS_EINVAL, "unknown pointwise operator");
    if (ops[o].block < 0 || ops[o].block >= n_blocks) return fail(c, PAOS_EINVAL, "operator block index out of range");
    if (ops[o].kind == PAOS_PW_MASK && ops[o].block + 1 >= n_blocks) return fail(c, PAOS_EINVAL, "an aperture operator needs two parameter blocks");
  }
  return PAOS_OK;
}

bool use_tables() {
  static const bool on = env_is("PAOS_PHASE_TABLES", '1');
  return on;
}

bool use_frugal() {
  static const bool on = !env_is("PAOS_NO_FRUGAL", '1');
  return on;
}

bool frugal_sizes(const paos_ctx* c) {
  return use_frugal() && c->n >= (c->precision == PAOS_F64 ? 1024 : 2048);
}

int ensure_mask_store(paos_ctx* c) {
  if (!c->mask_overflow) {
    HIPCHK(c, hipMalloc(&c->mask_overflow, sizeof(int)));
    HIPCHK(c, hipMemsetAsync(c->mask_overflow, 0, sizeof(int), c->stream));
  }
  return PAOS_OK;
}

int assign_mask_set(paos_ctx* c, const paos_pass& p, LoweredPass& lp, const double* blocks) {
  std::vector<double> key;
  key.reserve((size_t)2 * c->batch * FP_STRIDE + c->batch + 3);
  key.push_back((double)p.axis);
  key.push_back((double)(mask_render_mode() + (mask_rect_blocks() ? 0 : 8)));
  const double* ap = blocks + (size_t)lp.mask_block * c->batch * FP_STRIDE;
  key.insert(key.end(), ap, ap + (size_t)2 * c->batch * FP_STRIDE);
  key.insert(key.end(), lp.mask_shared.begin(), lp.mask_shared.end());
  int hit = -1, victim = 0;
  for (int k = 0; k < paos_ctx::kMaskSets; ++k) {
    const paos_ctx::MaskSet& ms = c->mask_sets[k];
    if (!ms.key.empty() && ms.key.size() == key.size() && !std::memcmp(ms.key.data(), key.data(), key.size() * sizeof(double))) hit = k;
    if (ms.used < c->mask_sets[victim].used) victim = k;
  }
  const int k = hit >= 0 ? hit : victim;
  paos_ctx::MaskSet& ms = c->mask_sets[k];
  if (!ms.lines) {
    for (paos_ctx::MaskSet& m2 : c->mask_sets) {
      if (m2.lines) continue;
      HIPCHK(c, hipMalloc(&m2.lines, (size_t)c->batch * c->n * sizeof(MaskLine)));
      HIPCHK(c, hipMalloc(&m2.vals, (size_t)c->batch * c->n * 2 * kMaskW * sizeof(double)));
    }
  }
  ms.used = ++c->mask_clock;
  lp.mask_set = k;
  lp.mask_render = hit < 0;
  lp.mask_shapes = 0;
  for (int it = 0; it < c->batch; ++it) {
    const double* a1 = ap + (size_t)it * FP_STRIDE;
    const double* a2 = a1 + (size_t)c->batch * FP_STRIDE;
    if (a1[0] != 0.0 && (it >= (int)lp.mask_shared.size() || lp.mask_shared[it] == 0.0)) lp.mask_shapes |= (int)a2[3] == 0 ? 1 : 2;
  }
  if (hit < 0) { ms.key = std::move(key); ++c->mask_rendered; } else ++c->mask_hits;
  for (int it = 0; it < c->batch; ++it) {
    if (lp.mask_rep[it] < 0) continue;
    FrugalSlot& sl = lp.mask_slot == 0 ? lp.items[it].pre : lp.items[it].mid;
    sl.lines = ms.lines + (size_t)lp.mask_rep[it] * c->n;
    sl.vals = ms.vals + (size_t)lp.mask_rep[it] * c->n * 2 * kMaskW;
  }
  return PAOS_OK;
}

void forget_mask_sets(paos_ctx* c) {
  for (auto& ms : c->mask_sets) ms.key.clear();
}

MaskRender mask_job(paos_ctx* c, int axis, const LoweredPass& lp, const double* ap, const double* dshared) {
  const int line0 = lp.mask_lo, line_end = lp.mask_hi > lp.mask_lo ? lp.mask_hi : c->n;
  return MaskRender{ap, dshared, lp.mask_set, axis, line0, line_end, lp.mask_shapes};
}

PlanDims plan_dims(const paos_ctx* c) { return PlanDims{c->n, c->batch, c->br, c->precision, c->central_half ? 1 : 0}; }
PlanSwitches plan_switches(const paos_ctx* c) {
  static const bool line_tables = !env_is("PAOS_LINE_TABLES", '0'), compact_grid = !env_is("PAOS_COMPACT_GRID", '0'),
                    env_prune = !env_is("PAOS_NO_PRUNE", '1'), batched_records = !env_is("PAOS_BATCHED_RECORDS", '0'),
                    psf_zero_reuse = !env_is("PAOS_PSF_ZERO_REUSE", '0');
  PlanSwitches sw;
  sw.line_tables = line_tables;
  sw.fuse_pairs = !env_is("PAOS_FUSE_PAIRS", '0');
  sw.compact_grid = compact_grid;
  sw.env_prune = env_prune;
  sw.stage_program = !env_is("PAOS_STAGE_PROGRAM", '0');
  sw.batched_records = batched_records;
  sw.psf_zero_reuse = psf_zero_reuse;
  sw.ctx_prune = c->prune;
  return sw;
}

struct StagedTables {
  const FrugalItem* items = nullptr;
  const PhaseSlotDesc* descs = nullptr;
  unsigned count = 0;
};
int stage_groups(paos_ctx* c, ArenaBatch& ab, std::vector<Launch>& groups, StagedTables* st) {
  std::vector<FrugalItem> blob;
  std::vector<PhaseSlotDesc> descs;
  int slots = 0;
  for (const Launch& g : groups)
    if (g.tables) slots += 2 * g.count;
  if (slots > c->ptab_slots) {
    if (c->ptab) { HIPCHK(c, hipStreamSynchronize(c->stream)); (void)hipFree(c->ptab); c->ptab = nullptr; c->ptab_slots = 0; }
    HIPCHK(c, hipMalloc(&c->ptab, (size_t)slots * c->batch * c->n * sizeof(cx<double>)));
    c->ptab_slots = slots;
  }
  int slot = 0;
  for (Launch& g : groups) {
    g.item_base = blob.size();
    for (int k = 0; k < g.count; ++k) {
      LoweredPass& l = *g.lp[k];
      const int counts[2] = {l.kpre, l.kmid};
      for (int s = 0; s < 2; ++s) {
        const bool has = g.tables && (counts[s] > 0 || g.count > 1);
        for (int it = 0; it < c->batch; ++it)
          (s == 0 ? l.items[it].pre : l.items[it].mid).table = has ? c->ptab + ((size_t)slot * c->batch + it) * c->n : nullptr;
        if (has) descs.push_back(PhaseSlotDesc{(int)blob.size(), s, counts[s], g.axis});
        if (g.tables) ++slot;
      }
      blob.insert(blob.end(), l.items.begin(), l.items.end());
    }
  }
  static_assert(sizeof(FrugalItem) % sizeof(double) == 0 && sizeof(PhaseSlotDesc) == 2 * sizeof(double), "records of doubles");
  const size_t item_doubles = blob.size() * sizeof(FrugalItem) / sizeof(double);
  std::vector<double> flat(item_doubles + 2 * descs.size());
  std::memcpy(flat.data(), blob.data(), item_doubles * sizeof(double));
  if (!descs.empty()) std::memcpy(flat.data() + item_doubles, descs.data(), descs.size() * sizeof(PhaseSlotDesc));
  const double* dflat = nullptr;
  int rc = ab.add(flat.data(), flat.size(), &dflat);
  if (rc) return rc;
  st->items = reinterpret_cast<const FrugalItem*>(dflat);
  st->descs = reinterpret_cast<const PhaseSlotDesc*>(dflat + item_doubles);
  st->count = (unsigned)descs.size();
  return PAOS_OK;
}
int launch_staged_tables(paos_ctx* c, const StagedTables& st) {
  if (st.count == 0) return PAOS_OK;
  const PhaseTableArgs ta{st.items, reinterpret_cast<const cx<double>*>(c->tw), st.descs, c->n, c->precision == PAOS_F64 ? 0 : 1};
  hipLaunchKernelGGL(phase_table_kernel<0>, dim3(c->n / 256, c->batch, st.count), dim3(256), 0, c->stream, ta);
  HIPCHK(c, hipGetLastError());
  return PAOS_OK;
}

int launch_lowered(paos_ctx* c, const Launch& g, const double* dblocks, const FrugalItem* staged) {
  for (int k = 0; k < g.count; ++k) {
    LoweredPass* l = g.lp[k];
    if (l->mask_block < 0 || !l->mask_render) continue;
    const double* ap = dblocks + (size_t)l->mask_block * c->batch * FP_STRIDE;
    const double* dshared = nullptr;
    int rcs = arena_push(c, l->mask_shared.data(), l->mask_shared.size(), &dshared);
    if (rcs) return rcs;
    const MaskRender job = mask_job(c, g.axis, *l, ap, dshared);
    if ((rcs = render_mask_records(c, &job, 1))) return rcs;
    l->mask_render = false;
  }
  if (!staged) {
    std::vector<Launch> one{g};
    ArenaBatch ab(c);
    StagedTables st;
    int rcg = stage_groups(c, ab, one, &st);
    if (rcg || (rcg = ab.commit()) || (rcg = launch_staged_tables(c, st))) return rcg;
    staged = st.items + one[0].item_base;
  }
  FrugalArgs a{c->field, c->tw, staged, c->pitch, c->item_stride, nullptr, nullptr, nullptr};
  if (g.store == 1) { a.psf = c->psf; a.psf_partial = c->psf_partial; }
  if (g.store == 2) a.pow_partial = c->pow_partial;
  a.dyn_scale = c->dyn_scale;
  a.live_lo = g.live_lo; a.live_hi = g.live_hi; a.wg0 = 0;
  c->prof_next_tag = g.tag;
  c->prof_next_bytes = g.bytes;
  c->prof_next_lines = g.lines;
  const FrugalBuild& b = g.build;
  {
    int rec[kBuildFields];
    build_to_ints(b, rec);
    c->pass_builds.insert(c->pass_builds.end(), rec, rec + kBuildFields);
  }
  static const bool dump = env_is("PAOS_DUMP_PASSES", '1');
  if (dump) {
    std::fprintf(stderr, "build axis %d kpre %d kmid %d nfft %d store %d tab %d fuse %d one_line %d central %d n %d %s\n", b.axis, b.kpre, b.kmid,
                 b.nfft, b.store, b.tab, b.fuse, b.one_line, b.central, c->n, c->precision == PAOS_F64 ? "fp64" : "fp32");
    for (int k = 0; k < g.count; ++k) {
      const LoweredPass* l = g.lp[k];
      if (l->items.empty()) continue;
      const FrugalItem& f = l->items[0];
      std::fprintf(stderr, "%spass axis %d kpre %d kmid %d nfft %d | pre: sign %g scale %g mask %g | fft1 on %g inv %g | mid: sign %g scale %g mask %g | "
                   "fft2 on %g inv %g | lines [%g, %g) fill %g loads [%g, %g) stores [%g, %g)\n", k == 0 ? "" : "+", g.axis, l->kpre, l->kmid, l->nfft,
                   f.pre.sign_on, f.pre.scale, f.pre.mask_on, f.fft1_on, f.fft1_inv, f.mid.sign_on, f.mid.scale, f.mid.mask_on, f.fft2_on, f.fft2_inv,
                   f.line_lo, f.line_hi, f.line_fill, f.pos_lo, f.pos_hi, f.spos_lo, f.spos_hi);
    }
  }
  return dispatch_family(c->precision, c->n, (int)PAOS_EUNSUPPORTED,
                         [&](auto t, auto n) { return frugal_family<decltype(t), decltype(n)::value>(c, b, a); });
}

int launch_one_pass(paos_ctx* c, const paos_pass& p, const double* dblocks, int n_blocks,
                    const int* table_of_op ) {
  int rc;
  for (int l = 0; l < 3; ++l)
    if ((rc = check_ops(c, op_list(p, l).ops, op_list(p, l).count, n_blocks))) return rc;
  if (p.fft1 >= n_blocks || p.fft2 >= n_blocks) return fail(c, PAOS_EINVAL, "transform control block out of range");
  int nmask = 0;
  for (int l = 0; l < 3; ++l) {
    const OpList ol = op_list(p, l);
    for (int o = 0; o < ol.count; ++o)
      if (ol.ops[o].kind == PAOS_PW_MASK) {
        if (++nmask > 1) return fail(c, PAOS_EINVAL, "one aperture operator per pass");
        int rcm = render_mask_weights(c, dblocks + (size_t)ol.ops[o].block * c->batch * FP_STRIDE);
        if (rcm) return rcm;
      }
  }
  PassArgs a{};
  a.field = c->field; a.tw = c->tw; a.blocks = dblocks; a.tables = c->tables; a.mask = c->mask; a.batch = c->batch;
  a.fft1 = p.fft1; a.fft2 = p.fft2; a.n_pre = p.n_pre; a.n_mid = p.n_mid; a.n_post = p.n_post;
  static_assert(sizeof(PwOp) == sizeof(paos_pw_op), "ABI op layout");
  std::memcpy(a.pre, p.pre, sizeof(a.pre));
  std::memcpy(a.mid, p.mid, sizeof(a.mid));
  std::memcpy(a.post, p.post, sizeof(a.post));
  PwOp* lists[3] = {a.pre, a.mid, a.post};
  int feat = 0;
  for (int l = 0; l < 3; ++l)
    for (int o = 0; o < PAOS_MAX_PW; ++o) {
      lists[l][o].flags &= (1 << kTableShift) - 1;
      const int t = table_of_op[l * PAOS_MAX_PW + o];
      if (t >= 0) { lists[l][o].flags |= (t + 1) << kTableShift; feat = 3; }
      if (o < op_list(p, l).count && lists[l][o].kind == PWK_MASK) feat = 3;
    }
  a.pitch = c->pitch; a.item_stride = c->item_stride;
  if (p.axis == 0 || p.axis == 1) return generic_pass(c, p.axis, a, feat);
  if (p.axis != -1) return fail(c, PAOS_EINVAL, "pass axis must be 0, 1 or -1");
  if (p.fft1 >= 0 || p.fft2 >= 0 || p.n_mid || p.n_post)
    return fail(c, PAOS_EINVAL, "a transform-free pass carries its operators in the pre list");
  return pointwise_pass(c, a);
}

struct ProgramRun {
  paos_ctx* c;
  const paos_pass* passes;
  int n_passes;
  const double* blocks;
  int n_blocks;
  PlanDims d;
  PlanSwitches sw;
  ArenaBatch ab;
  const double* dblocks = nullptr;
  std::vector<LoweredPass> low;
  bool all_frugal = false, pruned = false;
  int store = 0;
  int power_groups = 0;
  std::vector<MaskRender> renderings;
  std::vector<Launch> launches;
  std::vector<int> launch_of;
  StagedTables staged;
  ProgramRun(paos_ctx* c_, const paos_pass* passes_, int n_passes_, const double* blocks_, int n_blocks_)
      : c(c_), passes(passes_), n_passes(n_passes_), blocks(blocks_), n_blocks(n_blocks_), d(plan_dims(c_)), sw(plan_switches(c_)), ab(c_) {}
};

int validate_program(paos_ctx* c, const paos_pass* passes, int n_passes, const double* blocks, int n_blocks, const int* final_ticket) {
  if (c) c->pass_builds.clear();
  if (!c || !passes || !blocks || n_passes < 0 || n_blocks < 1) return fail(c, PAOS_EINVAL, "bad pass program");
  c->norm2_of_field = false;
  if (int rcr = final_ticket ? power_ring_full(c) : PAOS_OK) return rcr;
  switch (check_phase_args(plan_dims(c), passes, n_passes, blocks, n_blocks)) {
    case PHASE_BLOCK_OUT_OF_RANGE: return fail(c, PAOS_EINVAL, "operator block index out of range");
    case PHASE_TOO_LARGE: return fail(c, PAOS_EUNSUPPORTED, "quadratic phase exceeds 1e12 rad at the grid corner (or is not finite)");
    default: return PAOS_OK;
  }
}

int open_batch(ProgramRun& r) {
  paos_ctx* c = r.c;
  const size_t per_pass = (((size_t)c->batch * sizeof(FrugalItem) / sizeof(double) + 15) & ~size_t(15)) +
                          (((size_t)c->batch + 15) & ~size_t(15)) + 16;
  int rc = r.ab.begin((size_t)r.n_blocks * c->batch * FP_STRIDE + 16 + (size_t)r.n_passes * per_pass + 2 * arena_rounded((size_t)2 * c->batch));
  if (rc) return rc;
  return r.ab.add(r.blocks, (size_t)r.n_blocks * c->batch * FP_STRIDE, &r.dblocks);
}

int lower_and_assign_sets(ProgramRun& r) {
  paos_ctx* c = r.c;
  r.low.resize(r.n_passes);
  r.all_frugal = !use_tables() && frugal_sizes(c) && r.n_passes > 0;
  if (use_tables() || !frugal_sizes(c)) return PAOS_OK;
  int rc = ensure_mask_store(c);
  if (rc) return rc;
  for (int q = 0; q < r.n_passes; ++q) {
    LoweredPass& lp = r.low[q];
    lp.ok = lower_frugal(r.d, r.passes[q], r.blocks, lp);
    if (lp.ok && lp.mask_block >= 0 && (rc = assign_mask_set(c, r.passes[q], lp, r.blocks))) return rc;
    r.all_frugal = r.all_frugal && lp.ok;
  }
  return PAOS_OK;
}

int settle_stop(ProgramRun& r) {
  paos_ctx* c = r.c;
  if (!c->dyn_pending) return PAOS_OK;
  bool ride = r.n_passes > 0 && r.low[0].ok;
  if (ride)
    for (const FrugalItem& fi : r.low[0].items) ride = ride && fi.active != 0.0;
  if (ride) ++c->deferred_rode;
  return ride ? PAOS_OK : settle_scale(c);
}

void plan_lines(ProgramRun& r, const double* entry_rows, bool entry_stale, const double* entry_cols) {
  paos_ctx* c = r.c;
  r.pruned = r.all_frugal && r.sw.env_prune && r.sw.ctx_prune;
  if (r.pruned) plan_pruning(r.d, r.passes, r.n_passes, r.blocks, r.low, entry_rows, entry_stale, entry_cols);
  for (LoweredPass& lp : r.low) {
    if (!lp.ok || lp.mask_block < 0) continue;
    record_window(r.d, lp);
    paos_ctx::MaskSet& ms = c->mask_sets[lp.mask_set];
    if (!lp.mask_render && !(ms.line_lo <= lp.mask_lo && ms.line_hi >= lp.mask_hi)) {
      lp.mask_render = true;
      --c->mask_hits; ++c->mask_rendered;
    }
    if (lp.mask_render) { ms.line_lo = lp.mask_lo; ms.line_hi = lp.mask_hi; }
  }
}

int prepare_store(ProgramRun& r, int final_mode) {
  paos_ctx* c = r.c;
  r.store = last_pass_store(r.low, final_mode);
  if (final_mode == 2 && r.store == 2) {
    r.power_groups = c->n / frugal_tile_lines(c, r.passes[r.n_passes - 1].axis);
    if (c->pow_nparts < c->n / 2) {
      if (c->pow_partial) (void)hipFree(c->pow_partial);
      c->pow_partial = nullptr; c->pow_nparts = 0;
      HIPCHK(c, hipMalloc(&c->pow_partial, (size_t)c->batch * (c->n / 2) * sizeof(double)));
      c->pow_nparts = c->n / 2;
    }
    HIPCHK(c, hipMemsetAsync(c->pow_partial, 0, (size_t)c->batch * r.power_groups * sizeof(double), c->stream));
  }
  if (final_mode != 1) return PAOS_OK;
  if (!c->psf) HIPCHK(c, hipMalloc(&c->psf, (size_t)c->batch * c->item_stride * sizeof(double)));
  c->otf_valid = c->ee_valid = false;
  if (r.store != 1) return PAOS_OK;
  const int axis = r.passes[r.n_passes - 1].axis, groups = c->n / frugal_tile_lines(c, axis);
  if (c->psf_nparts < groups) {
    if (c->psf_partial) (void)hipFree(c->psf_partial);
    c->psf_partial = nullptr; c->psf_nparts = 0;
    c->psf_zero_axis = -1;
    HIPCHK(c, hipMalloc(&c->psf_partial, (size_t)c->batch * groups * sizeof(double)));
    c->psf_nparts = groups;
  }
  psf_zero_fill(r.d, r.sw, axis, r.low[r.n_passes - 1].items, c->psf_zero_axis, c->psf_zero_lo, c->psf_zero_hi);
  c->psf_zero_axis = -1;
  return PAOS_OK;
}

int batch_renderings(ProgramRun& r) {
  for (int q : batched_renderings(r.sw, r.all_frugal, r.low)) {
    LoweredPass& lp = r.low[q];
    const double* dshared = nullptr;
    int rc = r.ab.add(lp.mask_shared.data(), lp.mask_shared.size(), &dshared);
    if (rc) return rc;
    r.renderings.push_back(mask_job(r.c, r.passes[q].axis, lp, r.dblocks + (size_t)lp.mask_block * r.c->batch * FP_STRIDE, dshared));
    lp.mask_render = false;
  }
  return PAOS_OK;
}

int plan_and_stage_launches(ProgramRun& r) {
  r.launches = form_launches(r.d, r.sw, r.passes, r.n_passes, r.low, r.all_frugal && r.pruned, r.launch_of);
  for (Launch& g : r.launches) {
    if (!g.lp[0]->ok) continue;
    decide_tables(r.d, r.sw, g);
    finish_launch(r.d, r.sw, g, g.q + g.count == r.n_passes ? r.store : 0);
  }
  if (!stage_whole_program(r.d, r.sw, r.all_frugal, r.n_passes)) return PAOS_OK;
  return stage_groups(r.c, r.ab, r.launches, &r.staged);
}

int launch_chunks(ProgramRun& r) {
  paos_ctx* c = r.c;
  int rc;
  int i = 0;
  while (i < r.n_passes) {
    TableArgs ta{};
    ta.blocks = r.dblocks; ta.tables = c->tables; ta.batch = c->batch; ta.n = c->n; ta.count = 0;
    std::vector<int> assign;
    int j = i;
    for (; j < r.n_passes; ++j) {
      const paos_pass& p = r.passes[j];
      int need = 0;
      for (int l = 0; l < 3; ++l)
        for (int o = 0; o < op_list(p, l).count && o < PAOS_MAX_PW; ++o) need += is_phase(op_list(p, l).ops[o]);
      if (use_tables() && ta.count + need > kMaxTables) {
        if (j == i) return fail(c, PAOS_EINVAL, "one pass needs more phase tables than the store holds");
        break;
      }
      const size_t base = assign.size();
      assign.resize(base + 3 * PAOS_MAX_PW, -1);
      if (!use_tables()) continue;
      for (int l = 0; l < 3; ++l)
        for (int o = 0; o < op_list(p, l).count && o < PAOS_MAX_PW; ++o) {
          const paos_pw_op& op = op_list(p, l).ops[o];
          if (!is_phase(op)) continue;
          if (op.block < 0 || op.block >= r.n_blocks) return fail(c, PAOS_EINVAL, "operator block index out of range");
          ta.jobs[ta.count] = {op.block, op.kind, op.flags & PAOS_PWF_MUL2PI};
          assign[base + l * PAOS_MAX_PW + o] = ta.count++;
        }
    }
    if (ta.count > 0) {
      if (!c->tables) {
        HIPCHK(c, hipMalloc(&c->tables, (size_t)kMaxTables * c->batch * 2 * c->n * sizeof(cx<double>)));
        ta.tables = c->tables;
      }
      const dim3 grid((2 * c->n + 255) / 256, c->batch, ta.count);
      hipLaunchKernelGGL(phase_table_kernel, grid, dim3(256), 0, c->stream, ta);
      HIPCHK(c, hipGetLastError());
    }
    for (int q = i; q < j; ++q) {
      if (!r.low[q].ok) {
        if ((rc = launch_one_pass(c, r.passes[q], r.dblocks, r.n_blocks, &assign[(size_t)(q - i) * 3 * PAOS_MAX_PW]))) return rc;
        continue;
      }
      const Launch& g = r.launches[r.launch_of[q]];
      const int last = q + g.count - 1;
      if (last >= j) return fail(c, PAOS_EINVAL, "a fused group crosses a table chunk");
      if ((rc = launch_lowered(c, g, r.dblocks, r.staged.items ? r.staged.items + g.item_base : nullptr))) return rc;
      q = last;
      if (c->dyn_pending) {
        if ((rc = dyn_scale_reset(c))) return rc;
      }
    }
    i = j;
  }
  return PAOS_OK;
}

int hand_out_ticket(ProgramRun& r, int final_mode, int* final_ticket) {
  paos_ctx* c = r.c;
  if (final_mode == 2) {
    const int rcp = r.store == 2 ? take_power_ticket(c, c->pow_partial, r.power_groups, nullptr, final_ticket) : paos_norm2_enqueue(c, final_ticket);
    if (rcp == PAOS_OK) c->norm2_of_field = true;
    return rcp;
  }
  if (r.store != 1) return psf_keep_power_impl(c, final_ticket);
  c->psf_zero_axis = r.passes[r.n_passes - 1].axis;
  return take_power_ticket(c, c->psf_partial, c->n / frugal_tile_lines(c, r.passes[r.n_passes - 1].axis), nullptr, final_ticket);
}

int run_passes_impl(paos_ctx* c, const paos_pass* passes, int n_passes, const double* blocks, int n_blocks,
                    const double* entry_rows, bool entry_stale, int* final_ticket, int final_mode, const double* entry_cols) {
  int rc = validate_program(c, passes, n_passes, blocks, n_blocks, final_ticket);
  if (rc) return rc;
  final_mode = final_ticket ? (final_mode == 2 ? 2 : 1) : 0;
  ProgramRun r(c, passes, n_passes, blocks, n_blocks);
  if ((rc = open_batch(r)) || (rc = lower_and_assign_sets(r)) || (rc = settle_stop(r))) return rc;
  plan_lines(r, entry_rows, entry_stale, entry_cols);
  if (entry_stale && entry_rows && entry_zero_first(r.d, r.pruned, r.low, entry_rows, entry_cols)) {
    if ((rc = entry_cols ? zero_outside_box(c, entry_rows, entry_cols) : zero_outside_rows(c, entry_rows))) return rc;
  }
  if ((rc = prepare_store(r, final_mode)) || (rc = batch_renderings(r)) || (rc = plan_and_stage_launches(r))) return rc;
  if ((rc = r.ab.commit())) return rc;
  for (size_t at = 0; at < r.renderings.size(); at += kMaskRenders)
    if ((rc = render_mask_records(c, r.renderings.data() + at, (int)std::min<size_t>(kMaskRenders, r.renderings.size() - at)))) return rc;
  if ((rc = launch_staged_tables(c, r.staged)) || (rc = launch_chunks(r))) return rc;
  return final_mode ? hand_out_ticket(r, final_mode, final_ticket) : PAOS_OK;
}

}

int run_passes(paos_ctx* c, const paos_pass* passes, int n_passes, const double* blocks, int n_blocks, const double* entry_rows,
               bool entry_stale, int* final_ticket, int final_mode, const double* entry_cols) {
  const int rc = arena_settled(c, run_passes_impl(c, passes, n_passes, blocks, n_blocks, entry_rows, entry_stale, final_ticket, final_mode, entry_cols));
  if (rc != PAOS_OK && c) forget_mask_sets(c);
  return rc;
}

int mask_render_mode() {
  if (env_is("PAOS_MASK_SCAN", '1')) return 0;
  return env_is("PAOS_MASK_PAIRS", '0') ? 1 : (env_is("PAOS_MASK_PAIRS", '1') ? 2 : 3);
}
bool mask_rect_blocks() {
  return !env_is("PAOS_MASK_RECT_BLOCKS", '0');
}

namespace {

struct Program {
  std::vector<paos_pass> passes;
  std::vector<double> blocks;
  int batch;
  explicit Program(int b) : batch(b) {}
  int add_block(const double* src, double v1, double v2, double v3, double v4, bool copy) {
    const int id = (int)(blocks.size() / ((size_t)batch * FP_STRIDE));
    for (int i = 0; i < batch; ++i) {
      const double* s = src + (size_t)i * FP_STRIDE;
      if (copy) blocks.insert(blocks.end(), s, s + FP_STRIDE);
      else blocks.insert(blocks.end(), {s[FP_ENABLE], v1, v2, v3, v4});
    }
    return id;
  }
  paos_pass& add_pass(int axis, int fft1, int fft2) {
// ... 114 lines not shown
```

Measured before the change: 2401 wavefronts/s.

## Add narrow-window central-half pass variant that loads and stores only the middle 3/8

Adds a CH=2 kernel variant, chosen at plan time, for passes where every active item's load and store windows fall within [5n/16, 11n/16). That variant loads, computes slots for and stores only the middle six of sixteen elements per thread. It also prunes the first 16-point butterfly for the now-zero inputs, and pins the register tile with empty asm to keep the compiler from reordering. The aim is to cut HBM traffic and arithmetic on passes whose live region is narrower than the central half. The cost is another instantiated kernel variant and more plan-time checks that must classify windows correctly.

```diff
diff --git a/include/paos_hip.h b/include/paos_hip.h
--- a/include/paos_hip.h
+++ b/include/paos_hip.h
@@ -123,6 +123,7 @@
 int paos_copy_yardstick(paos_ctx* ctx, int reps, double* ms_per_launch, double* bytes_per_launch);
 int paos_record_set_stats(paos_ctx* ctx, unsigned long long* found, unsigned long long* rendered);
 int paos_central_half_stats(paos_ctx* ctx, unsigned long long* central, unsigned long long* plain);
+int paos_narrow_window_stats(paos_ctx* ctx, unsigned long long* narrow, unsigned long long* other);
 int paos_frugal_built(int precision, int n, const int* record);
 int paos_pass_builds(paos_ctx* ctx, int* records, int capacity, int* count);
 int paos_deferred_stop_stats(paos_ctx* ctx, unsigned long long* rode, unsigned long long* settled);
diff --git a/paos_amd/_lib.py b/paos_amd/_lib.py
--- a/paos_amd/_lib.py
+++ b/paos_amd/_lib.py
@@ -102,6 +102,7 @@
     "paos_copy_yardstick": (ctypes.c_int, [_c_ctx, ctypes.c_int, _dbl_p, _dbl_p]),
     "paos_record_set_stats": (ctypes.c_int, [_c_ctx, ctypes.POINTER(ctypes.c_ulonglong), ctypes.POINTER(ctypes.c_ulonglong)]),
     "paos_central_half_stats": (ctypes.c_int, [_c_ctx, ctypes.POINTER(ctypes.c_ulonglong), ctypes.POINTER(ctypes.c_ulonglong)]),
+    "paos_narrow_window_stats": (ctypes.c_int, [_c_ctx, ctypes.POINTER(ctypes.c_ulonglong), ctypes.POINTER(ctypes.c_ulonglong)]),
     "paos_frugal_built": (ctypes.c_int, [ctypes.c_int, ctypes.c_int, ctypes.POINTER(ctypes.c_int)]),
     "paos_pass_builds": (ctypes.c_int, [_c_ctx, ctypes.POINTER(ctypes.c_int), ctypes.c_int, ctypes.POINTER(ctypes.c_int)]),
     "paos_deferred_stop_stats": (ctypes.c_int, [_c_ctx, ctypes.POINTER(ctypes.c_ulonglong), ctypes.POINTER(ctypes.c_ulonglong)]),
diff --git a/paos_amd/csrc/context.hip b/paos_amd/csrc/context.hip
--- a/paos_amd/csrc/context.hip
+++ b/paos_amd/csrc/context.hip
@@ -302,6 +302,8 @@
   if (const char* pad = getenv("PAOS_LDS_PAD")) c->lds_pad = (size_t)std::max(0, std::atoi(pad));
   if (env_is("PAOS_CENTRAL_HALF", '0')) c->central_half = false;
   if (env_is("PAOS_CENTRAL_HALF", '1')) c->central_half = true;
+  if (env_is("PAOS_NARROW_WINDOWS", '0')) c->narrow_windows = false;
+  if (env_is("PAOS_NARROW_WINDOWS", '1')) c->narrow_windows = true;
   if ((e = hipMalloc(&c->dyn_scale, (size_t)batch * sizeof(double))) != hipSuccess) return bail(e, "hipMalloc(dyn_scale)");
   {
     std::vector<double> ones((size_t)batch, 1.0);
@@ -505,6 +507,13 @@
   return PAOS_OK;
 }
 
+int paos_narrow_window_stats(paos_ctx* c, unsigned long long* narrow, unsigned long long* other) {
+  if (!c || !narrow || !other) return fail(c, PAOS_EINVAL, "bad narrow-window request");
+  *narrow = c->narrow_launches;
+  *other = c->other_launches;
+  return PAOS_OK;
+}
+
 int paos_deferred_stop_stats(paos_ctx* c, unsigned long long* rode, unsigned long long* settled) {
   if (!c || !rode || !settled) return fail(c, PAOS_EINVAL, "bad deferred-stop request");
   *rode = c->deferred_rode;
diff --git a/paos_amd/csrc/fft_core.h b/paos_amd/csrc/fft_core.h
--- a/paos_amd/csrc/fft_core.h
+++ b/paos_amd/csrc/fft_core.h
@@ -217,7 +217,7 @@
   for (int k2 = 0; k2 < 4; ++k2) v[3 + 4 * k2] = o[k2];
 }
 
-template <int DIR, typename T>
+template <int DIR, bool NARROW = false, typename T>
 __device__ __forceinline__ void dft16_lf_central(cx<T>* v) {
   static_assert(DIR > 0, "the pass kernel runs forward transforms only");
   cx<T> y[16];
@@ -225,10 +225,22 @@
   for (int n2 = 0; n2 < 4; ++n2) {
     const cx<T> a = v[4 + n2], b = v[8 + n2];
     const cx<T> nb = {-b.x, -b.y};
-    y[0 * 4 + n2] = cadd(b, a);
-    y[1 * 4 + n2] = sub_ib(nb, a);
-    y[2 * 4 + n2] = csub(b, a);
-    y[3 * 4 + n2] = add_ib(nb, a);
+    if (NARROW && n2 == 0) {
+      y[0 * 4 + n2] = b;
+      y[1 * 4 + n2] = nb;
+      y[2 * 4 + n2] = b;
+      y[3 * 4 + n2] = nb;
+    } else if (NARROW && n2 == 3) {
+      y[0 * 4 + n2] = a;
+      y[1 * 4 + n2] = cx<T>{a.y, -a.x};
+      y[2 * 4 + n2] = cx<T>{-a.x, -a.y};
+      y[3 * 4 + n2] = cx<T>{-a.y, a.x};
+    } else {
+      y[0 * 4 + n2] = cadd(b, a);
+      y[1 * 4 + n2] = sub_ib(nb, a);
+      y[2 * 4 + n2] = csub(b, a);
+      y[3 * 4 + n2] = add_ib(nb, a);
+    }
   }
   cx<T> o[4];
   {
@@ -385,7 +397,7 @@
     }
     if constexpr (CH != 0 && NS == 1) {
       static_assert(R == 16 && TPT == 1, "central-half first stage: one 16-point butterfly per thread");
-      dft16_lf_central<DIR>(v);
+      dft16_lf_central<DIR, CH == 2>(v);
     } else {
       dft<R, DIR>(v + s * R);
     }
diff --git a/paos_amd/csrc/frugal_d1024.hip b/paos_amd/csrc/frugal_d1024.hip
--- a/paos_amd/csrc/frugal_d1024.hip
+++ b/paos_amd/csrc/frugal_d1024.hip
@@ -1,4 +1,4 @@
 #include "frugal_launch.h"
 
 template <>
-int frugal_family<double, 1024>(paos_ctx* c, const FrugalBuild& b, const FrugalArgs& a) { return frugal_dispatch<double, 1024>(c, b, a); }
+int frugal_family<double, 1024>(paos_ctx* c, const FrugalBuild& b, const FrugalArgs& a, bool narrow) { return frugal_dispatch<double, 1024>(c, b, a, narrow); }
diff --git a/paos_amd/csrc/frugal_d2048.hip b/paos_amd/csrc/frugal_d2048.hip
--- a/paos_amd/csrc/frugal_d2048.hip
+++ b/paos_amd/csrc/frugal_d2048.hip
@@ -1,4 +1,4 @@
 #include "frugal_launch.h"
 
 template <>
-int frugal_family<double, 2048>(paos_ctx* c, const FrugalBuild& b, const FrugalArgs& a) { return frugal_dispatch<double, 2048>(c, b, a); }
+int frugal_family<double, 2048>(paos_ctx* c, const FrugalBuild& b, const FrugalArgs& a, bool narrow) { return frugal_dispatch<double, 2048>(c, b, a, narrow); }
diff --git a/paos_amd/csrc/frugal_d4096.hip b/paos_amd/csrc/frugal_d4096.hip
--- a/paos_amd/csrc/frugal_d4096.hip
+++ b/paos_amd/csrc/frugal_d4096.hip
@@ -1,4 +1,4 @@
 #include "frugal_launch.h"
 
 template <>
-int frugal_family<double, 4096>(paos_ctx* c, const FrugalBuild& b, const FrugalArgs& a) { return frugal_dispatch<double, 4096>(c, b, a); }
+int frugal_family<double, 4096>(paos_ctx* c, const FrugalBuild& b, const FrugalArgs& a, bool narrow) { return frugal_dispatch<double, 4096>(c, b, a, narrow); }
diff --git a/paos_amd/csrc/frugal_f2048.hip b/paos_amd/csrc/frugal_f2048.hip
--- a/paos_amd/csrc/frugal_f2048.hip
+++ b/paos_amd/csrc/frugal_f2048.hip
@@ -1,4 +1,4 @@
 #include "frugal_launch.h"
 
 template <>
-int frugal_family<float, 2048>(paos_ctx* c, const FrugalBuild& b, const FrugalArgs& a) { return frugal_dispatch<float, 2048>(c, b, a); }
+int frugal_family<float, 2048>(paos_ctx* c, const FrugalBuild& b, const FrugalArgs& a, bool narrow) { return frugal_dispatch<float, 2048>(c, b, a, narrow); }
diff --git a/paos_amd/csrc/frugal_f4096.hip b/paos_amd/csrc/frugal_f4096.hip
--- a/paos_amd/csrc/frugal_f4096.hip
+++ b/paos_amd/csrc/frugal_f4096.hip
@@ -1,4 +1,4 @@
 #include "frugal_launch.h"
 
 template <>
-int frugal_family<float, 4096>(paos_ctx* c, const FrugalBuild& b, const FrugalArgs& a) { return frugal_dispatch<float, 4096>(c, b, a); }
+int frugal_family<float, 4096>(paos_ctx* c, const FrugalBuild& b, const FrugalArgs& a, bool narrow) { return frugal_dispatch<float, 4096>(c, b, a, narrow); }
diff --git a/paos_amd/csrc/frugal_launch.h b/paos_amd/csrc/frugal_launch.h
--- a/paos_amd/csrc/frugal_launch.h
+++ b/paos_amd/csrc/frugal_launch.h
@@ -32,7 +32,7 @@
 namespace {
 
 template <typename T, int N, int AXIS, int KPRE, int KMID, int NFFT, int STORE, int TAB, int LONG, int ONE, int CH>
-int frugal_launch(paos_ctx* c, const FrugalArgs& args) {
+int frugal_launch(paos_ctx* c, const FrugalArgs& args, bool narrow) {
   using C = FftCfg<T, N>;
   using G = FrugalGeometry<T, N, AXIS, KPRE, KMID, STORE, LONG, ONE>;
   FrugalArgs a = args;
@@ -50,32 +50,38 @@
   constexpr size_t kMaxPad = 8192;
   const size_t lds = G::LDS + (c->lds_pad < kMaxPad ? c->lds_pad : kMaxPad);
   auto kern = frugal_pass_kernel<T, N, C::E, G::LINES, G::TILES, AXIS, C::BR, C::BC, G::SPLIT, KPRE, KMID, NFFT, STORE, TAB, LONG, G::OCC, CH>;
+  if constexpr (CH == 1) {
+    if (narrow) kern = frugal_pass_kernel<T, N, C::E, G::LINES, G::TILES, AXIS, C::BR, C::BC, G::SPLIT, KPRE, KMID, NFFT, STORE, TAB, LONG, G::OCC, 2>;
+  } else {
+    narrow = false;
+  }
   ++(CH != 0 ? c->central_launches : c->plain_launches);
+  ++(narrow ? c->narrow_launches : c->other_launches);
   return TIMED_LAUNCH(c, kern, grid, block, lds, G::LDS + kMaxPad, AXIS == 0 ? PAOS_KERNEL_PASS_ROWS : PAOS_KERNEL_PASS_COLS,
                       c->prof_next_tag, PAOS_FRUGAL_PASS(a));
 }
 
 constexpr int kFrugalFieldMax[] = {1, kFrugalMaxPre, kFrugalMaxMid, 2, 2, 1, 4, 1, 1};
 template <typename T, int N, int X, int... V>
-int frugal_unfold(paos_ctx* c, const FrugalBuild& b, const FrugalArgs& a) {
+int frugal_unfold(paos_ctx* c, const FrugalBuild& b, const FrugalArgs& a, bool narrow) {
   constexpr int I = sizeof...(V), kFields = sizeof(kFrugalFieldMax) / sizeof(int);
   static_assert(kFields == kBuildFields, "one maximum per field");
   int field[kBuildFields];
   build_to_ints(b, field);
   if (field[I] != X) {
-    if constexpr (X < kFrugalFieldMax[I]) return frugal_unfold<T, N, X + 1, V...>(c, b, a);
+    if constexpr (X < kFrugalFieldMax[I]) return frugal_unfold<T, N, X + 1, V...>(c, b, a, narrow);
     else return frugal_not_built(c, b);
   } else if constexpr (I + 1 < kFields) {
-    return frugal_unfold<T, N, 0, V..., X>(c, b, a);
+    return frugal_unfold<T, N, 0, V..., X>(c, b, a, narrow);
   } else if constexpr (frugal_built<T, N>(FrugalBuild{V..., X})) {
-    return frugal_launch<T, N, V..., X>(c, a);
+    return frugal_launch<T, N, V..., X>(c, a, narrow);
   } else {
     return frugal_not_built(c, b);
   }
 }
 template <typename T, int N>
-int frugal_dispatch(paos_ctx* c, const FrugalBuild& b, const FrugalArgs& a) {
-  return frugal_unfold<T, N, 0>(c, b, a);
+int frugal_dispatch(paos_ctx* c, const FrugalBuild& b, const FrugalArgs& a, bool narrow = false) {
+  return frugal_unfold<T, N, 0>(c, b, a, narrow);
 }
 
 }
diff --git a/paos_amd/csrc/frugal_pass.h b/paos_amd/csrc/frugal_pass.h
--- a/paos_amd/csrc/frugal_pass.h
+++ b/paos_amd/csrc/frugal_pass.h
@@ -144,6 +144,11 @@
   return p;
 }
 
+template <int E, int CH>
+constexpr int ch_first() { return CH == 2 ? 5 * E / 16 : (CH != 0 ? E / 4 : 0); }
+template <int E, int CH>
+constexpr int ch_end() { return CH == 2 ? 11 * E / 16 : (CH != 0 ? 3 * E / 4 : E); }
+
 template <typename T, int N, int E, int K, typename Map, int PLAIN = 0, bool SHARE = false, int RECS = 0, int TAB = 0, int CH = 0>
 __device__ __forceinline__ void frugal_slot(cx<T>* v, const FrugalSlot& sl, const FrugalPhase* ph,
                                             const Map& m, const cx<double>* circle, bool conj_in, bool conj_out, int tpos,
@@ -170,8 +175,8 @@
   }
   constexpr int TL = N / E;
   static_assert(TL % 2 == 0, "the checkerboard sign is constant along a thread's elements");
-  static_assert(CH == 0 || (K > 0 && TAB != 0 && sizeof(T) == 8 && E % 4 == 0), "central-half slots: complex128 table slots");
-  constexpr int kFirst = CH != 0 ? E / 4 : 0, kEnd = CH != 0 ? 3 * E / 4 : E;
+  static_assert(CH == 0 || (K > 0 && TAB != 0 && sizeof(T) == 8 && E % 16 == 0), "central-half slots: complex128 table slots");
+  constexpr int kFirst = ch_first<E, CH>(), kEnd = ch_end<E, CH>();
   const double sc = __dmul_rn(sl.scale, extra_scale);
   const int line = Map::kAxis == 0 ? m.row(0) : m.col(0);
   if (sl.mask_on != 0.0) {
@@ -420,6 +425,12 @@
   else *p = v;
 }
 
+template <int E, typename T>
+__device__ __forceinline__ void pin_tile(cx<T>* v) {
+#pragma unroll
+  for (int k = 0; k < E; ++k) asm volatile("" : "+v"(v[k].x), "+v"(v[k].y));
+}
+
 template <typename T, int N, int E, bool SPLIT, bool FLIP = true, int CH = 0>
 __device__ __forceinline__ void frugal_fft(cx<T>* v, void* lds, int t, const cx<T>* tw, const cx<double>* circle,
                                            double inv, const cx<T>* w1_last = nullptr) {
@@ -496,6 +507,7 @@
     frugal_pass_kernel(PAOS_FRUGAL_PARAMS) {
   static_assert(LONG == 0 || (TAB != 0 && NFFT == 2 && KPRE == 1 && KMID == 1), "LONG builds: see above");
   static_assert(CH == 0 || (sizeof(T) == 8 && N == 4096 && E == 16 && TAB != 0 && KPRE == 1 && NFFT <= 2), "CH builds: see above");
+  static_assert(CH >= 0 && CH <= 2 && (CH != 2 || STORE == 0), "CH = 2: field-storing builds");
   FrugalArgs a;
   a.items = k_items; a.field = k_field; a.pitch = k_pitch; a.item_stride = k_item_stride; a.wg0 = k_wg0;
   a.tw = k_tw; a.psf = k_psf; a.psf_partial = k_psf_partial; a.pow_partial = k_pow_partial; a.dyn_scale = k_dyn_scale; a.live_lo = a.live_hi = 0;
@@ -595,7 +607,7 @@
 #pragma unroll
     for (int k = 0; k < E; ++k) v[k] = cx<T>{(T)0, (T)0};
 #pragma unroll
-    for (int k = E / 4; k < 3 * E / 4; ++k) {
+    for (int k = ch_first<E, CH>(); k < ch_end<E, CH>(); ++k) {
       const int pos = m.t + k * (N / E);
       if (pos >= plo && pos < phi) v[k] = stream_load<NT>(at(k));
     }
@@ -672,7 +684,8 @@
   if (ran1) frugal_fft<T, N, E, SPLIT, false, CH>(v, lds, m.t, tw, circle, it.fft1_inv, w1_last);
   PAOS_STAMP(3);
   constexpr bool kShareMid = kShare && KPRE == 0 && KMID < 3;
-  frugal_slot<T, N, E, KMID, decltype(m), 0, kShareMid, (kRecMode == 1 ? -1 : kRecs), TAB>(
+  constexpr int kNarrowMid = (CH == 2 && NFFT == 1 && LONG == 0 && KMID > 0) ? 2 : 0;
+  frugal_slot<T, N, E, KMID, decltype(m), 0, kShareMid, (kRecMode == 1 ? -1 : kRecs), TAB, kNarrowMid>(
       v, it.mid, it.mid_ph, m, circle, inv1, ran2 && it.fft2_inv != 0.0, m.t, lds, ran1, kRecMode == 1 ? rec_lds : mrec, lbase, h_dyn);
   PAOS_STAMP(4);
   if constexpr (NFFT == 2) {
@@ -689,13 +702,16 @@
     const bool ran4 = (kTwo) && (ix).fft2_on != 0.0;                                                                                 \
     const bool inv3 = ran3 && (ix).fft1_inv != 0.0;                                                                                  \
     frugal_slot<T, N, E, 1, decltype(m), 0, false, 0, TAB>(v, (ix).pre, (ix).pre_ph, m, circle, false, inv3, m.t, lds, false);       \
+    if constexpr (CH == 2 && !(kTwo)) pin_tile<E>(v);                                                                                \
     if (ran3) {                                                                                                                      \
       if (busy) __syncthreads();                                                                                                     \
       frugal_fft<T, N, E, SPLIT, false>(v, lds, m.t, tw, circle, (ix).fft1_inv, w1_last);                                            \
       busy = true;                                                                                                                   \
     }                                                                                                                                \
-    frugal_slot<T, N, E, 1, decltype(m), 0, false, 0, TAB>(v, (ix).mid, (ix).mid_ph, m, circle, inv3, ran4 && (ix).fft2_inv != 0.0,  \
-                                                           m.t, lds, ran3);                                                          \
+                \
+    frugal_slot<T, N, E, 1, decltype(m), 0, false, 0, TAB, (CH == 2 && !(kTwo)) ? 2 : 0>(                                            \
+        v, (ix).mid, (ix).mid_ph, m, circle, inv3, ran4 && (ix).fft2_inv != 0.0, m.t, lds, ran3);                                    \
+    if constexpr (CH == 2 && (kTwo)) pin_tile<E>(v);                                                                                 \
     if constexpr (kTwo) {                                                                                                            \
       if (ran4) {                                                                                                                    \
         if (busy) __syncthreads();                                                                                                   \
@@ -728,7 +744,13 @@
     return;
   }
   const int slo = (int)h_spos_lo, shi = (int)h_spos_hi;
-  if (slo <= 0 && shi >= N) {
+  if constexpr (CH == 2) {
+#pragma unroll
+    for (int k = ch_first<E, CH>(); k < ch_end<E, CH>(); ++k) {
+      const int pos = m.t + k * (N / E);
+      if (pos >= slo && pos < shi) stream_store<NT>(at(k), v[k]);
+    }
+  } else if (slo <= 0 && shi >= N) {
 #pragma unroll
     for (int k = 0; k < E; ++k) stream_store<NT>(at(k), v[k]);
   } else {
diff --git a/paos_amd/csrc/host.h b/paos_amd/csrc/host.h
--- a/paos_amd/csrc/host.h
+++ b/paos_amd/csrc/host.h
@@ -126,6 +126,8 @@
   size_t lds_pad = 0;
   bool central_half = true;
   unsigned long long central_launches = 0, plain_launches = 0;
+  bool narrow_windows = true;
+  unsigned long long narrow_launches = 0, other_launches = 0;
   std::vector<int> pass_builds;
   int* mask_overflow = nullptr;
   double* partial = nullptr;
@@ -267,7 +269,7 @@
 int generic_pass(paos_ctx* c, int axis, const PassArgs& a, int feat);
 
 template <typename T, int N>
-int frugal_family(paos_ctx* c, const FrugalBuild& b, const FrugalArgs& a);
+int frugal_family(paos_ctx* c, const FrugalBuild& b, const FrugalArgs& a, bool narrow);
 
 int settle_scale(paos_ctx* c, bool field_is_overwritten = false);
 int dyn_scale_reset(paos_ctx* c);
diff --git a/paos_amd/csrc/pass_program.h b/paos_amd/csrc/pass_program.h
--- a/paos_amd/csrc/pass_program.h
+++ b/paos_amd/csrc/pass_program.h
@@ -16,6 +16,7 @@
   int n, batch, br;
   int precision;
   int central_half;
+  int narrow_windows = 1;
 };
 struct PlanSwitches {
   bool line_tables = true;
@@ -366,6 +367,7 @@
   size_t item_base = 0;
   int store = 0;
   FrugalBuild build{};
+  int narrow = 0;
   unsigned live_lo = 0, live_hi = 0;
   int tag = 0;
   double bytes = 0.0, lines = 0.0;
@@ -438,9 +440,26 @@
   return b;
 }
 
+inline int pick_narrow(const PlanDims& d, const Launch& g, const FrugalBuild& b) {
+  if (b.central != 1 || !d.narrow_windows) return 0;
+  const double lo = 5.0 * (double)d.n, hi = 11.0 * (double)d.n;
+  bool any = false;
+  for (const FrugalItem& fi : g.lp[0]->items) {
+    if (fi.active == 0.0) continue;
+    any = true;
+    if (!(16.0 * fi.pos_lo >= lo && 16.0 * fi.pos_hi <= hi)) return 0;
+  }
+  for (const FrugalItem& fo : g.last().items) {
+    if (fo.active == 0.0) continue;
+    if (!(16.0 * fo.spos_lo >= lo && 16.0 * fo.spos_hi <= hi)) return 0;
+  }
+  return any ? 1 : 0;
+}
+
 inline void finish_launch(const PlanDims& d, const PlanSwitches& sw, Launch& g, int store) {
   g.store = store;
   g.build = pick_build(d, g);
+  g.narrow = pick_narrow(d, g, g.build);
   const bool store_psf = store == 1;
   const LoweredPass& lp = *g.lp[0];
   {
diff --git a/paos_amd/csrc/passes.hip b/paos_amd/csrc/passes.hip
--- a/paos_amd/csrc/passes.hip
+++ b/paos_amd/csrc/passes.hip
@@ -93,7 +93,9 @@
   return MaskRender{ap, dshared, lp.mask_set, axis, line0, line_end, lp.mask_shapes};
 }
 
-PlanDims plan_dims(const paos_ctx* c) { return PlanDims{c->n, c->batch, c->br, c->precision, c->central_half ? 1 : 0}; }
+PlanDims plan_dims(const paos_ctx* c) {
+  return PlanDims{c->n, c->batch, c->br, c->precision, c->central_half ? 1 : 0, c->narrow_windows ? 1 : 0};
+}
 PlanSwitches plan_switches(const paos_ctx* c) {
   static const bool line_tables = !env_is("PAOS_LINE_TABLES", '0'), compact_grid = !env_is("PAOS_COMPACT_GRID", '0'),
                     env_prune = !env_is("PAOS_NO_PRUNE", '1'), batched_records = !env_is("PAOS_BATCHED_RECORDS", '0'),
@@ -212,7 +214,7 @@
     }
   }
   return dispatch_family(c->precision, c->n, (int)PAOS_EUNSUPPORTED,
-                         [&](auto t, auto n) { return frugal_family<decltype(t), decltype(n)::value>(c, b, a); });
+                         [&](auto t, auto n) { return frugal_family<decltype(t), decltype(n)::value>(c, b, a, g.narrow != 0); });
 }
 
 int launch_one_pass(paos_ctx* c, const paos_pass& p, const double* dblocks, int n_blocks,
```

Measured after the change: 2439 wavefronts/s, median of 6. 1.6% higher.
